# MDIL-SNU/SevenNet

Hardware: AMD Instinct MI355X
Metric: atom-steps/sec (energy+forces), SevenNet-0 100k-atom cell, 1/2/4/8 MI355X (higher is better)
Workload: dtype f32 (storage / accumulate / tensor product; in-kernel W2 products f16x3 = two fp16 terms per operand, three matrix-core products: fp32-rounding class; node linears bf16x6); 1 GPU; sevennet_0 shape (5 interaction layers), 97336-atom periodic diamond-Si cell (a=5.431 A x 23^3, sigma=0.05 A), cutoff 5.0 A, 2725408 directed edges, seeded synthetic weights; atoms=97336, edges=2725408, parallelism=single GPU, fused=auto, terms=4

## Files before the change

include/snet_hip.h:

```cpp
#ifndef SNET_HIP_H
#define SNET_HIP_H

#include <stdint.h>

#ifdef __cplusplus
extern "C" {
#endif

#define SNET_ABI_VERSION 3

int snet_abi_version(void);
const char *snet_last_error(void);
int snet_conv_num_shapes(void);
const char *snet_conv_shape_tag(int i);

typedef struct snet_edge_params {
  float cutoff;
  int32_t n_basis;
  int32_t cutoff_kind;
  int32_t poly_p;
  float cutoff_on;
  int32_t lmax;
  int32_t normalize;
} snet_edge_params;
// ... 54 lines not shown
void snet_fused_plan_destroy(snet_fused_plan *plan);
int snet_edge_tiles(const int32_t *row_ptr, int64_t n_dst, int32_t *tile_ptr, int32_t *tile_node, int64_t tile_capacity,
                    int64_t *n_tiles, void *stream);
int snet_edge_tiles_packed(const int32_t *row_ptr, int64_t node_begin, int64_t node_end, int32_t *tile_e0,
                           int32_t *tile_nodes, int64_t tile_capacity, int64_t *n_tiles, void *stream);
int snet_fused_plan_tile_mode(const snet_fused_plan *plan);
int snet_conv_plan_transposed(const snet_conv_plan *plan, char *tag, float *col_scale, int32_t *dead, int32_t dead_capacity,
                              int32_t *n_dead);
int snet_edges_by_source(const int32_t *row_ptr, int64_t n_dst, const int32_t *eperm, const int32_t *w_row, int64_t n_edges,
                         int32_t *center_t, int32_t *w_row_t, void *stream);
int snet_conv_fwd_fused(const snet_fused_plan *plan, const float *x, const float *sh, const float *h2,
                        const int32_t *w_row, const int32_t *row_ptr, const int32_t *src, int64_t n_dst, float scale,
                        float *out, void *stream);
int snet_conv_bwd_fused(const snet_fused_plan *plan, const float *x, const float *sh, const float *dsh,
                        const float *h2, const int32_t *w_row, const int32_t *row_ptr, const int32_t *src,
                        const int32_t *tile_ptr, const int32_t *tile_node, int64_t n_tiles, float scale,
                        const float *g_out, float *g_xe, float *g_h2, const float *emb, float *g_emb, float *g_vec,
                        const float *x_rowmax, const float *g_rowmax, void *stream);
int snet_conv_bwd_fused_sh(const snet_fused_plan *plan, const float *x, const float *sh, const float *h2, const int32_t *w_row,
                           const int32_t *row_ptr, const int32_t *src, const int32_t *tile_ptr, const int32_t *tile_node,
                           int64_t n_tiles, float scale, const float *g_out, float *g_xe, float *g_h2, const float *emb,
                           float *g_emb, float *g_sh, const float *x_rowmax, const float *g_rowmax, void *stream);
int snet_fused_plan_has_mlp_tail(const snet_fused_plan *plan);
int snet_fused_plan_prefers_tangent(const snet_fused_plan *plan);
int snet_edge_embed_tangent(const snet_edge_params *p_host, const float *coeffs_host, const float *edge_vec,
                            const int32_t *edge_of_row, int64_t n_rows, float *demb, void *stream);
int snet_radial_mlp_hidden_fwd_layers_tangent(const snet_mlp_plan *const *plans, int32_t n_layers, const float *emb, const float *demb,
                                              int64_t n_rows, float *const *h2, float *const *h2d, void *stream);
int snet_conv_bwd_fused_tangent(const snet_fused_plan *plan, const float *x, const float *sh, const float *dsh, const float *h2,
                                const float *h2d, const int32_t *w_row, const int32_t *row_ptr, const int32_t *src,
                                const int32_t *tile_ptr, const int32_t *tile_node, int64_t n_tiles, float scale, const float *g_out,
                                float *g_xe, const float *edge_vec, float *g_vec, const float *x_rowmax, const float *g_rowmax,
                                void *stream);
int snet_fused_plan_gxe_chunks(const snet_fused_plan *plan, int32_t *chunk_pos, int32_t capacity);
int snet_segment_sum_rows_chunked(const float *x, const int32_t *seg_ptr, const int32_t *perm, int64_t n_seg, int32_t dim,
                                  const int32_t *chunk_pos, float *out, void *stream);
int snet_row_absmax(const float *x, int64_t n_rows, int32_t dim, float *out, void *stream);
int snet_row_absmax_multi(const float *const *x, const int64_t *n_rows, const int32_t *dims, float *const *out, int32_t n,
                          void *stream);
int snet_row_norm2(const float *x, int64_t n_rows, int32_t dim, float mult, float *out, void *stream);
int snet_conv_bwd_edge(const snet_conv_plan *plan, const float *x, const float *sh, const float *w,
                       const int32_t *w_row, const int32_t *row_ptr, const int32_t *src, int64_t n_dst, float scale,
                       const float *g_out, float *g_w, float *g_xe, float *g_sh, void *stream);
int snet_conv_bwd_edge_vec(const snet_conv_plan *plan, const float *x, const float *sh, const float *dsh,
                           const float *w, const int32_t *w_row, const int32_t *row_ptr, const int32_t *src,
                           int64_t n_dst, float scale, const float *g_out, float *g_w, float *g_xe, float *g_vec,
                           void *stream);
int snet_conv_bwd_node(const snet_conv_plan *plan, const float *sh, const float *w, const int32_t *w_row,
                       const int32_t *col_ptr,
                       const int32_t *eperm, const int32_t *dst, int64_t n_src, float scale,
                       const float *g_out, float *g_x, void *stream);

int snet_segment_sum_rows(const float *x, const int32_t *seg_ptr, const int32_t *perm, int64_t n_seg, int32_t dim,
                          float *out, void *stream);

typedef struct snet_gate_seg {
  int32_t kind;
  int32_t in_off;
  int32_t out_off;
  int32_t mul;
  int32_t l;
  int32_t gate_off;
  int32_t act;
  float cst;
} snet_gate_seg;
#define SNET_MAX_GATE_SEGS 16
// ... 153 lines not shown
```

sevennet_amd/_lib.py:

```python
from __future__ import annotations

import ctypes as C
import os

_HERE = os.path.dirname(os.path.abspath(__file__))
ABI_VERSION = 3
LIB_PATH = os.environ.get('SNET_HIP_LIB') or os.path.join(_HERE, 'libsnet_hip.so')

c_f32p = C.c_void_p
c_i32p = C.c_void_p
c_f64p = C.c_void_p
c_stream = C.c_void_p


class EdgeParams(C.Structure):
    _fields_ = [('cutoff', C.c_float), ('n_basis', C.c_int32), ('cutoff_kind', C.c_int32),
                ('poly_p', C.c_int32), ('cutoff_on', C.c_float), ('lmax', C.c_int32),
                ('normalize', C.c_int32)]


class GemmDesc(C.Structure):
    _fields_ = [('B', C.c_void_p), ('B_split', C.c_void_p), ('a_off', C.c_int64), ('c_off', C.c_int64), ('d', C.c_int32), ('K', C.c_int32),
                ('N', C.c_int32), ('accumulate', C.c_int32)]

# ... 30 lines not shown
    'snet_act_bwd': (C.c_int, [c_f32p, c_f32p, c_f32p, C.c_int64, C.c_int32, C.c_float, c_stream]),
    'snet_conv_plan_create': (C.c_int, [C.c_char_p, C.POINTER(C.c_void_p)]),
    'snet_conv_plan_destroy': (None, [C.c_void_p]),
    'snet_conv_register_library': (C.c_int, [C.c_char_p]),
    'snet_conv_plan_dims': (C.c_int, [C.c_void_p, C.POINTER(C.c_int32), C.POINTER(C.c_int32),
                                      C.POINTER(C.c_int32), C.POINTER(C.c_int32)]),
    'snet_conv_fwd': (C.c_int, [C.c_void_p, c_f32p, c_f32p, c_f32p, c_i32p, c_i32p, c_i32p, C.c_int64, C.c_float,
                                c_f32p, c_stream]),
    'snet_radial_mlp_hidden_fwd': (C.c_int, [C.c_void_p, c_f32p, C.c_int64, c_f32p, c_stream]),
    'snet_radial_mlp_hidden_fwd_layers': (C.c_int, [C.POINTER(C.c_void_p), C.c_int32, c_f32p, C.c_int64, C.POINTER(C.c_void_p), c_stream]),
    'snet_radial_mlp_hidden_bwd': (C.c_int, [C.c_void_p, c_f32p, c_f32p, C.c_int64, c_f32p, c_stream]),
    'snet_conv_fused_available': (C.c_int, [C.c_void_p]),
    'snet_conv_plan_transposed': (C.c_int, [C.c_void_p, C.c_char_p, c_f32p, c_i32p, C.c_int32, C.POINTER(C.c_int32)]),
    'snet_edges_by_source': (C.c_int, [c_i32p, C.c_int64, c_i32p, c_i32p, C.c_int64, c_i32p, c_i32p, c_stream]),
    'snet_fused_plan_create': (C.c_int, [C.c_void_p, C.c_void_p, C.c_int32, C.POINTER(C.c_void_p)]),
    'snet_fused_plan_destroy': (None, [C.c_void_p]),
    'snet_edge_tiles': (C.c_int, [c_i32p, C.c_int64, c_i32p, c_i32p, C.c_int64, C.POINTER(C.c_int64), c_stream]),
    'snet_conv_fwd_fused': (C.c_int, [C.c_void_p, c_f32p, c_f32p, c_f32p, c_i32p, c_i32p, c_i32p, C.c_int64, C.c_float,
                                      c_f32p, c_stream]),
    'snet_conv_bwd_fused': (C.c_int, [C.c_void_p, c_f32p, c_f32p, c_f32p, c_f32p, c_i32p, c_i32p, c_i32p, c_i32p,
                                      c_i32p, C.c_int64, C.c_float, c_f32p, c_f32p, c_f32p, c_f32p, c_f32p, c_f32p, c_f32p, c_f32p,
                                      c_stream]),
    'snet_conv_bwd_fused_sh': (C.c_int, [C.c_void_p, c_f32p, c_f32p, c_f32p, c_i32p, c_i32p, c_i32p, c_i32p,
                                         c_i32p, C.c_int64, C.c_float, c_f32p, c_f32p, c_f32p, c_f32p, c_f32p, c_f32p, c_f32p, c_f32p,
                                         c_stream]),
    'snet_fused_plan_has_mlp_tail': (C.c_int, [C.c_void_p]),
    'snet_fused_plan_prefers_tangent': (C.c_int, [C.c_void_p]),
    'snet_edge_embed_tangent': (C.c_int, [C.POINTER(EdgeParams), C.POINTER(C.c_float), c_f32p, c_i32p, C.c_int64, c_f32p, c_stream]),
    'snet_radial_mlp_hidden_fwd_layers_tangent': (C.c_int, [C.POINTER(C.c_void_p), C.c_int32, c_f32p, c_f32p, C.c_int64,
                                                            C.POINTER(C.c_void_p), C.POINTER(C.c_void_p), c_stream]),
    'snet_conv_bwd_fused_tangent': (C.c_int, [C.c_void_p, c_f32p, c_f32p, c_f32p, c_f32p, c_f32p, c_i32p, c_i32p, c_i32p, c_i32p,
                                              c_i32p, C.c_int64, C.c_float, c_f32p, c_f32p, c_f32p, c_f32p, c_f32p, c_f32p,
                                              c_stream]),
    'snet_fused_plan_gxe_chunks': (C.c_int, [C.c_void_p, C.POINTER(C.c_int32), C.c_int32]),
    'snet_segment_sum_rows_chunked': (C.c_int, [c_f32p, c_i32p, c_i32p, C.c_int64, C.c_int32, c_i32p, c_f32p, c_stream]),
    'snet_edge_vectors': (C.c_int, [c_f64p, c_i32p, c_i32p, c_f64p, C.c_int64, c_f32p, c_stream]),
    'snet_row_absmax': (C.c_int, [c_f32p, C.c_int64, C.c_int32, c_f32p, c_stream]),
    'snet_row_absmax_multi': (C.c_int, [C.POINTER(C.c_void_p), C.POINTER(C.c_int64), C.POINTER(C.c_int32), C.POINTER(C.c_void_p), C.c_int32, c_stream]),
    'snet_row_norm2': (C.c_int, [c_f32p, C.c_int64, C.c_int32, C.c_float, c_f32p, c_stream]),
    'snet_conv_bwd_edge': (C.c_int, [C.c_void_p, c_f32p, c_f32p, c_f32p, c_i32p, c_i32p, c_i32p, C.c_int64, C.c_float,
                                     c_f32p, c_f32p, c_f32p, c_f32p, c_stream]),
    'snet_segment_sum_rows': (C.c_int, [c_f32p, c_i32p, c_i32p, C.c_int64, C.c_int32, c_f32p, c_stream]),
    'snet_conv_bwd_node': (C.c_int, [C.c_void_p, c_f32p, c_f32p, c_i32p, c_i32p, c_i32p, c_i32p, C.c_int64, C.c_float,
                                     c_f32p, c_f32p, c_stream]),
    'snet_gate_fwd': (C.c_int, [c_f32p, c_f32p, c_f32p, C.c_int64, C.c_int32, C.c_int32, C.POINTER(GateSeg), C.c_int32,
                                c_stream]),
    'snet_gate_bwd': (C.c_int, [c_f32p, c_f32p, c_f32p, C.c_int64, C.c_int32, C.c_int32, C.POINTER(GateSeg),
                                C.c_int32, c_stream]),
    'snet_gate_bwd_norm': (C.c_int, [c_f32p, c_f32p, c_f32p, C.c_int64, C.c_int32, C.c_int32, C.POINTER(GateSeg),
                                     C.c_int32, C.c_float, c_f32p, c_stream]),
    'snet_embed_rows': (C.c_int, [c_f32p, c_i32p, c_f32p, C.c_int64, C.c_int32, c_stream]),
    'snet_add_row_bias': (C.c_int, [c_f32p, c_f32p, C.c_int64, C.c_int32, c_stream]),
    'snet_add_inplace': (C.c_int, [c_f32p, c_f32p, C.c_int64, c_stream]),
    'snet_permute_cols': (C.c_int, [c_f32p, c_i32p, c_f32p, C.c_int64, C.c_int32, c_stream]),
    'snet_rescale_reduce': (C.c_int, [c_f32p, c_i32p, c_f32p, c_f32p, C.c_int32, C.c_int64, c_f32p, c_f64p,
                                      c_stream]),
    'snet_readout_energy': (C.c_int, [c_f32p, C.c_int64, C.c_int32, c_f64p, C.c_double, c_i32p, c_f32p, c_f32p, C.c_int32,
                                      c_f32p, c_f64p, c_stream]),
    'snet_readout_grad': (C.c_int, [c_f64p, C.c_int32, c_i32p, c_f32p, C.c_int32, C.c_int64, c_f32p, c_stream]),
    'snet_edge_force': (C.c_int, [c_f32p, c_f32p, c_i32p, c_i32p, c_i32p, C.c_int64, C.c_int64, c_f32p, c_f32p,
                                  c_f64p, c_stream]),
    'snet_readout_energy_seg': (C.c_int, [c_f32p, C.c_int64, C.c_int32, c_f64p, C.c_double, c_i32p, c_f32p, c_f32p, C.c_int32,
                                          c_i32p, C.c_int32, c_f32p, c_f64p, c_f64p, c_stream]),
    'snet_rescale_reduce_seg': (C.c_int, [c_f32p, c_i32p, c_f32p, c_f32p, C.c_int32, C.c_int64, c_i32p, C.c_int32, c_f32p, c_f64p,
                                          c_f64p, c_stream]),
    'snet_edge_force_seg': (C.c_int, [c_f32p, c_f32p, c_i32p, c_i32p, c_i32p, C.c_int64, C.c_int64, c_i32p, C.c_int32, c_f32p,
# ... 132 lines not shown
```

sevennet_amd/build.py:

```python
from __future__ import annotations

import argparse
import concurrent.futures as cf
import hashlib
import os
import shutil
import subprocess
import sys
from typing import List

from . import codegen, codegen_fused
from .shapes import aot_conv_specs

HERE = os.path.dirname(os.path.abspath(__file__))
CSRC = os.path.join(HERE, 'csrc')
INCLUDE = os.path.join(os.path.dirname(HERE), 'include')
LIB = os.environ.get('SNET_BUILD_LIB') or os.path.join(HERE, 'libsnet_hip.so')
_sfx = ('_' + os.path.basename(LIB).replace('.so', '')) if os.environ.get('SNET_BUILD_LIB') else ''
GEN = os.path.join(CSRC, 'generated' + _sfx)
OBJ = os.path.join(CSRC, 'build' + _sfx)
ARCH = 'gfx950'
STATIC_SOURCES = ['snet_api.cpp', 'snet_model.cpp', 'snet_halo.cpp', 'snet_gemm.hip', 'snet_mlp.hip', 'snet_edge.hip', 'snet_node.hip', 'snet_force.hip', 'snet_neighbor.hip', 'snet_batch.hip', 'snet_relax.hip', 'snet_mdstep.hip', 'snet_md.hip', 'snet_d3.hip', 'snet_d3_ref.cpp']


# ... 90 lines not shown
        ['-o', out, f'-L{os.path.dirname(LIB)}', '-l:' + os.path.basename(LIB), f'-L{rocm}/lib', '-lamdhip64',
         '-Wl,-rpath,$ORIGIN/../../sevennet_amd', f'-Wl,-rpath,{rocm}/lib']
    r = subprocess.run(cmd, capture_output=True, text=True)
    if r.returncode != 0:
        raise RuntimeError(f'g++ failed on the LAMMPS mock harness:\n{r.stderr[-4000:]}')
    if verbose:
        print(f'[sevennet_amd.build] built {out}', flush=True)
    return out


def build(jobs: int = 0, force: bool = False, extra_configs=(), verbose: bool = True) -> str:
    write_d3_blob()
    os.makedirs(GEN, exist_ok=True)
    os.makedirs(OBJ, exist_ok=True)
    os.makedirs(os.path.join(CSRC, 'generated'), exist_ok=True)
    codegen.write_if_changed(os.path.join(CSRC, 'generated', 'sh_generated.h'), codegen.gen_sh_header(3))
    specs = aot_conv_specs(extra_configs)
    sources = [os.path.join(CSRC, s) for s in STATIC_SOURCES]
    keep = set()
    for tag, spec in specs.items():
        path = os.path.join(GEN, f'conv_{tag}.hip')
        codegen.write_if_changed(path, codegen.gen_conv(spec))
        sources.append(path)
        keep.add(os.path.basename(path))
        if codegen_fused.fusable(spec):
            fpath = os.path.join(GEN, f'convf_{tag}.hip')
            codegen.write_if_changed(fpath, codegen_fused.gen_conv_fused(spec))
            sources.append(fpath)
            keep.add(os.path.basename(fpath))
            tpath = os.path.join(GEN, f'convft_{tag}.hip')
            codegen.write_if_changed(tpath, codegen_fused.gen_conv_fused_tangent(spec))
            sources.append(tpath)
            keep.add(os.path.basename(tpath))
    for f in os.listdir(GEN):
        if (f.startswith('conv_') or f.startswith('convf_') or f.startswith('convft_') or f.startswith('_conv')) and f not in keep:
            os.remove(os.path.join(GEN, f))
    jobs = jobs or min(16, os.cpu_count() or 4)
    if verbose:
        print(f'[sevennet_amd.build] {len(sources)} translation units ({len(specs)} conv shapes), -j{jobs}',
              flush=True)
    with cf.ThreadPoolExecutor(jobs) as ex:
        objs = list(ex.map(lambda s: _compile(s, force), sources))
    newest = max(os.path.getmtime(o) for o in objs)
    if force or not os.path.exists(LIB) or os.path.getmtime(LIB) < newest:
        cmd = [_hipcc(), f'--offload-arch={ARCH}', '-shared', '-fPIC', '-o', LIB] + objs
        r = subprocess.run(cmd, capture_output=True, text=True)
        if r.returncode != 0:
            raise RuntimeError(f'link failed:\n{r.stderr[-4000:]}')
    if verbose:
        print(f'[sevennet_amd.build] built {LIB}', flush=True)
    if not os.environ.get('SNET_BUILD_LIB'):
        try:
            build_lammps_harness(verbose)
        except Exception as exc:
            print(f'[sevennet_amd.build] LAMMPS mock harness NOT built: {exc}', file=sys.stderr, flush=True)
    return LIB


def main(argv=None):
    ap = argparse.ArgumentParser()
    ap.add_argument('-j', type=int, default=0)
    ap.add_argument('--force', action='store_true')
    a = ap.parse_args(argv)
    build(a.j, a.force)


if __name__ == '__main__':
    main()
# ... 1 lines not shown
```

sevennet_amd/codegen_fused.py:

```python
from __future__ import annotations

import struct
from typing import Dict, List

from .codegen import OPTS, _Cat, _f, _path_terms, _sum_expr
from .model_spec import ConvSpec


def fusable(spec: ConvSpec) -> bool:
    return all(mul % 16 == 0 for mul, _, _ in spec.irreps_x) and spec.irreps_sh.dim <= 16 and len(spec.paths) > 0


def schedule(spec: ConvSpec):
    cats = []
    for i in range(len(spec.irreps_x)):
        cat = _Cat(spec, i, 0)
        if cat.paths:
            cats.append(cat)
    pairs_of, cols = [], []
    for cat in cats:
        ps = [pi for pi, _ in cat.paths]
        pairs = [(ps[k], ps[k + 1] if k + 1 < len(ps) else None) for k in range(0, len(ps), 2)]
        pairs_of.append(pairs)
        for ct in range(cat.mul // 16):
            for pa, pb in pairs:
                cols.append((spec.paths[pa].w_off + 16 * ct, spec.paths[pb].w_off + 16 * ct if pb is not None else -1))
    return cats, pairs_of, cols


def schedule_bwd(spec: ConvSpec):
    out, cols = [], []
    n_cats = sum(1 for i in range(len(spec.irreps_x)) if _Cat(spec, i, 0).paths)
    for i in range(len(spec.irreps_x)):
        cat = _Cat(spec, i, 0)
        if not cat.paths:
            continue
        ps = [pi for pi, _ in cat.paths]
        nct = cat.mul // 16
        entries = sum(2 * p.l3 + 1 for _, p in cat.paths)
        if len(ps) % 2 == 1 and nct % 2 == 0 and 2 * entries <= 32 and n_cats > 1 and not OPTS.get('nopairct'):
            full = [(ps[k], ps[k + 1]) for k in range(0, len(ps) - 1, 2)]
            steps = [((a, 0), (b, 0)) for a, b in full] + [((a, 1), (b, 1)) for a, b in full] + [((ps[-1], 0), (ps[-1], 1))]
            U = 2
# ... 97 lines not shown
    for a, cl in reverse_plan(p):
        A(f'  {{  // x component {a}')
        A(f'    const f32x2 xl = lo2(xr[{a}]), xh = hi2(xr[{a}]);')
        A('    const f32x2 wxl = wl * xl, wxh = wh * xh;')
        A('    f32x2 Pl, Ph;')
        for k, (c, bl) in enumerate(cl):
            tl = [f'{_f(v)} * ys[{p.sh_off + b}]' for b, v in bl]
            A(f'    {{ const float V = {_sum_expr(tl)};')
            A('      const f32x2 V2 = f32x2{V, V};')
            A(f'      const f32x2 Gl = lo2(G[{c}]), Gh = hi2(G[{c}]);')
            if k == 0:
                A('      Pl = V2 * Gl; Ph = V2 * Gh;')
            else:
                A('      Pl = __builtin_elementwise_fma(V2, Gl, Pl); Ph = __builtin_elementwise_fma(V2, Gh, Ph);')
            A('      const f32x2 s2 = __builtin_elementwise_fma(wxh, Gh, wxl * Gl);')
            for b, v in bl:
                if pkgy:
                    A(f'      gy[{p.sh_off + b}] = __builtin_elementwise_fma(f32x2{{{_f(v)}, {_f(v)}}}, s2, gy[{p.sh_off + b}]);')
                else:
                    A(f'      gy[{p.sh_off + b}] = fmaf({_f(v)}, s2[0] + s2[1], gy[{p.sh_off + b}]);')
            A('    }')
        A('    gwl = __builtin_elementwise_fma(xl, Pl, gwl); gwh = __builtin_elementwise_fma(xh, Ph, gwh);')
        A('    if constexpr (GX) {')
        A(f'      const f32x2 gl_ = __builtin_elementwise_fma(wl, Pl, lo2(gx[{a}])), gh_ = __builtin_elementwise_fma(wh, Ph, hi2(gx[{a}]));')
        A(f'      gx[{a}] = f32x4{{gl_[0], gl_[1], gh_[0], gh_[1]}};')
        A('    }')
        A('  }')
    A('  gw = f32x4{gwl[0], gwl[1], gwh[0], gwh[1]};')
    A('}')


class _Gen:

    def __init__(self, spec: ConvSpec, tangent: bool = False):
        self.spec = spec
        self.TG = bool(tangent)
        tag = self.tag = spec.tag
        self.def_b = (int(OPTS.get('fnwv', 8)), int(OPTS.get('fglds', 0)), int(OPTS.get('focc', 2)))
        self.def_f = (int(OPTS.get('fnwvf', 8)), int(OPTS.get('fgldsf', 0)), int(OPTS.get('foccf', 2)))
        self.exp = OPTS.get('fexp') == tag
        self.DX, self.DOUT, self.NSH, self.WN = spec.irreps_x.dim, spec.irreps_out.dim, spec.irreps_sh.dim, spec.weight_numel
        NSH = self.NSH
        cats, self.pairs_of, self.cols = schedule(spec)
        self.cats = cats
        self.NS = len(self.cols)
        self.offs_x = spec.irreps_x.offsets()
        self.dead_x = [i for i in range(len(spec.irreps_x)) if not any(p.i_x == i for p in spec.paths)]
        self.L: List[str] = []
        self.A = self.L.append
        self.NSHP = NSH + 1 if (4 * NSH) % 32 == 0 else NSH
        self.gxe_std = bool(OPTS.get('gxestd'))
        self.stamped = tag in (OPTS.get('stamp'), OPTS.get('stampl'), OPTS.get('stampf'), OPTS.get('stampfl'))
        self.FROW = bool(int(OPTS.get('frow', 1)))
        self.FRSB = int(OPTS.get('frsb', 0))
        self._reverse_decisions()
        self._forward_decisions()
        if self.TG:
            self.stamped = self.ST = self.STL = False

    def _reverse_decisions(self):
        spec, cats, NSH = self.spec, self.cats, self.NSH
        bsched, cols_b = schedule_bwd(spec)
        self.bsched, self.cols_b = bsched, cols_b
        glists = [[(pi, m3, u) for u in range(bs['U']) for pi, p in bs['cat'].paths for m3 in range(2 * p.l3 + 1)] for bs in bsched]
        self.glists = glists
        NGP = max((len(gl) + 15) // 16 * 16 for gl in glists)
        NK = NGP // 16
        self.NGP, self.NK = NGP, NK
        maxd1 = max(2 * c_.l1 + 1 for c_ in cats)
        maxd3 = max(2 * p_.l3 + 1 for p_ in spec.paths)

        def live_regs(gs):
            return 12 * maxd1 + 32 + NSH + 4 * gs * NK + 16 + 4 * maxd3 + 35
        packed_class = live_regs(2) <= 200 and live_regs(1) > 168 and len(cats) > 1
        XT = self.XT = bool(int(OPTS['xtile'])) if 'xtile' in OPTS else packed_class
        GS = self.GS = 2 if XT else 1
        self.PK = bool(int(OPTS['pk'])) if 'pk' in OPTS else XT
        self.PKGY = self.PK and bool(int(OPTS.get('pkgy', 1)))
        VMORD = self.VMORD = not OPTS.get('novmord')
        self.GRAW = VMORD and not OPTS.get('nograw')
        GUNC = VMORD and not OPTS.get('nogunc')
        live = self.live = live_regs(GS)
        self.three_waves = 2 * 8 * 2 * 1024 + 4 * (2 * NGP * 64 + NSH * 64) <= 53 * 1024 and live <= (160 if XT else 168)
        if self.three_waves:
            GUNC = GUNC and bool(OPTS.get('gunc3'))
        self.GUNC = GUNC
        budget = (168 if self.three_waves else 256) - 24
        xp_regs = max([4 * b_['U'] * (2 * b_['cat'].l1 + 1) for b_ in bsched[1:]] or [0])
        self.XPF = VMORD and len(bsched) > 1 and live + xp_regs + 8 <= budget and not OPTS.get('noxpf')
        self.HOIST = VMORD and live + 16 + 8 <= budget and not OPTS.get('nohoist')
        self.noxn = int(OPTS.get('noxn', 7 if live > 200 else 0))
        self.STL = OPTS.get('stampl') == self.tag
        self.ST = OPTS.get('stamp') == self.tag or self.STL
        self.TGPREF = bool(int(OPTS['tgpref'])) if 'tgpref' in OPTS else live <= 200

    def block_info(self, ci):
        bs = self.bsched[ci]
        d1 = 2 * bs['cat'].l1 + 1
        return bs['cat'], bs['U'], bs['ncb'], d1, (self.noxn > 0 and d1 >= self.noxn)

    def bwd_lds(self, nt, nwv):
        return 2 * 8 * nt * 1024 + nwv * (2 * self.NGP * 64 + (128 if self.XT else 0) + self.NSH * 64)

    def bwd_cfg(self, nt):
        if 'fnwv' in OPTS:
            return self.def_b
        if len(self.cats) == 1 and self.bwd_lds(nt, 8) <= 80 * 1024:
            return (8, 0, 2)
        if self.bwd_lds(nt, 4) <= 53 * 1024 and self.live <= (160 if self.XT else 168):
            return (4, 0, 3)
        if self.bwd_lds(nt, 4) <= 80 * 1024:
            return (4, 0, 2)
        return (2, 0, 2)

    def _forward_decisions(self):
        spec, cats = self.spec, self.cats
        FG = int(OPTS.get('ffg', 3))
        fgroups = []
        for ci, cat in enumerate(cats):
            prs = list(enumerate(self.pairs_of[ci]))
            fgroups.append([prs[i:i + FG] for i in range(0, len(prs), FG)])
        self.fgroups = fgroups
        self.LPB = max(len(grp) for gl in fgroups for grp in gl)
        NOE = max(sum(2 * spec.paths[pi].l3 + 1 for _, pr in grp for pi in pr if pi is not None) for gl in fgroups for grp in gl)
        self.NOEP = (NOE + 15) // 16 * 16
        self.MAXD1 = max(2 * cat.l1 + 1 for cat in cats)
        self.N_OOFF = sum((sum(2 * spec.paths[pi].l3 + 1 for _, pr in grp for pi in pr if pi is not None) + 15) // 16 for gl in fgroups for grp in gl)
        self.OOLDS = self.N_OOFF > 8 if 'oolds' not in OPTS else bool(int(OPTS['oolds']))
        self.STFL = OPTS.get('stampfl') == self.tag
        self.STF = OPTS.get('stampf') == self.tag or self.STFL
        self.olists, self.oo_index = {}, {}

    def fwd_lds(self, nt, nwv):
        return 2 * self.LPB * 4 * nt * 1024 + nwv * (32 * self.NSHP * 4 + self.MAXD1 * 1024 + self.NOEP * 64) + 4 * nwv + (64 * self.N_OOFF if self.OOLDS else 0)

    def fwd_cfg(self, nt):
        if 'fnwvf' in OPTS:
            return self.def_f
        if len(self.cats) == 1 and self.fwd_lds(nt, 8) <= 80 * 1024:
            return (8, 0, 2)
        if nt <= 2 and self.fwd_lds(nt, 12) <= 160 * 1024:
            return (12, 0 if OPTS.get('f12reg') else 1, 3)
        for w in (8, 4, 2, 1):
            if self.fwd_lds(nt, w) <= 160 * 1024:
                return (w, 1, 2)
        raise NotImplementedError(f'conv shape {self.spec.key}: the fused forward kernel does not fit the LDS')

    @staticmethod
    def out_index(p, m3):
        return p.out_off + m3 * p.out_mul + p.out_ch

    def S(self, i, ind='      '):
        if self.ST and (not self.STL or i in (0, 1, 10, 11, 12, 13)):
            self.A(f'{ind}stamp({i});')

    def SF(self, i, ind, light=True):
        if self.STF and (light or not self.STFL):
            self.A(f'{ind}stamp({i});')

    def g_row(self, ci, pi, m3, u):
        return self.glists[ci].index((pi, m3, u))

    def emit_g_loads(self, ind, ci, cb_expr):
        A, glists, bsched, exp, GRAW, GUNC, XT = self.A, self.glists, self.bsched, self.exp, self.GRAW, self.GUNC, self.XT
        gl = glists[ci]
        U_ = bsched[ci]['U']
        for k in range((len(gl) + 15) // 16):
            dg = '(diag & 8) ? f32x4{1.f, 1.f, 1.f, 1.f} : ' if exp else ''
            sc_ = ' * scale' if not GRAW else ''
            pred = '' if GUNC else f'(goff{ci}_{k} < 0) ? f32x4{{0.f, 0.f, 0.f, 0.f}} : '
            A(f'{ind}gpre[{k}] = {dg}{pred}*reinterpret_cast<const f32x4 *>(gnode + goff{ci}_{k} + {16 * U_} * ({cb_expr})){sc_};')
        if XT:
            A(f'{ind}if (two) {{')
            for k in range((len(gl) + 15) // 16):
                A(f'{ind}  gpre_b[{k}] = {dg}{pred}*reinterpret_cast<const f32x4 *>(gnode_b + goff{ci}_{k} + {16 * U_} * ({cb_expr})){sc_};')
            A(f'{ind}}}')

    def emit_g_park(self, ind, ci, buf_expr):
        A, glists, GRAW, XT = self.A, self.glists, self.GRAW, self.XT
        gl = glists[ci]
        for k in range((len(gl) + 15) // 16):
            sc_ = ' * g_park'
            A(f'{ind}*reinterpret_cast<f32x4 *>(&s_g[wave][{"0" if XT else buf_expr}][(16 * {k} + (lane >> 2)) * 16 + 4 * (lane & 3)]) = gpre[{k}]{sc_};')
        if XT:
            A(f'{ind}if (two) {{')
            for k in range((len(gl) + 15) // 16):
                A(f'{ind}  *reinterpret_cast<f32x4 *>(&s_g[wave][1][(16 * {k} + (lane >> 2)) * 16 + 4 * (lane & 3)]) = gpre_b[{k}]{sc_};')
            A(f'{ind}}}')

    def emit_x_loads(self, ind, ci_, ct_expr, tl_):
        A, cats = self.A, self.cats
        cat_ = cats[ci_]
        A(f'{ind}{{ const float *xs_ = x + {cat_.x_off} + 16 * ({ct_expr}) + 4 * (lane & 3) + (size_t)srs[{tl_}] * DX;')
        for m in range(2 * cat_.l1 + 1):
            A(f'{ind}  xq[{m}] = *reinterpret_cast<const f32x4 *>(xs_ + {m * cat_.mul});')
        A(f'{ind}}}')


def _emit_header(cx: _Gen):
    A, spec, tag, cats = cx.A, cx.spec, cx.tag, cx.cats
    DX, DOUT, NSH, NSHP, WN, NS, cols, cols_rev = cx.DX, cx.DOUT, cx.NSH, cx.NSHP, cx.WN, cx.NS, cx.cols, cx.cols_b
    A('// GENERATED by sevennet_amd/codegen_fused.py -- do not edit.')
    A(f'// fused conv shape {tag}: x = {spec.irreps_x}, sh = {spec.irreps_sh}, out = {spec.irreps_out}')
    A(f'// {len(spec.paths)} paths, weight_numel = {WN}, {NS} sub-steps of two 16-column tiles')
    A('#include <cstdio>')
    A('#include <cstdlib>')
    A('#include "snet_common.h"')
    A('#include "snet_split.h"')
    A('namespace {')
    A('using namespace snet;')
    A('__device__ __forceinline__ f32x2 lo2(const f32x4 v) { return __builtin_shufflevector(v, v, 0, 1); }')
    A('__device__ __forceinline__ f32x2 hi2(const f32x4 v) { return __builtin_shufflevector(v, v, 2, 3); }')
    A(f'constexpr int DX = {DX}, DOUT = {DOUT}, NSH = {NSH}, NSHP = {NSHP}, WN = {WN}, NS = {NS};')
    A('const int32_t SUB_COLS[NS * 2] = {' + ', '.join(f'{a}, {b}' for a, b in cols) + '};')
    A(f'const int32_t SUB_COLS_B[{2 * len(cols_rev)}] = {{' + ', '.join(f'{a}, {b}' for a, b in cols_rev) + '};')
    gxe_chunk = list(range(DX // 16))
    for cat in ([] if cx.gxe_std else cats):
        d1c = 2 * cat.l1 + 1
        for ct in range(cat.mul // 16):
            for m in range(d1c):
                gxe_chunk[(cat.x_off + m * cat.mul) // 16 + ct] = cat.x_off // 16 + ct * d1c + m
    assert sorted(gxe_chunk) == list(range(DX // 16))
    A(f'const int32_t GXE_CHUNK[{DX // 16}] = {{' + ', '.join(str(v) for v in gxe_chunk) + '};')
    A('')


def _emit_path_functions(cx: _Gen):
    A, spec, PK, FROW, FRSB = cx.A, cx.spec, cx.PK, cx.FROW, cx.FRSB
    for pi, p in enumerate(spec.paths):
# ... 51 lines not shown
                    A(f'    const float y{b_} = ysl[{r} * NSHP + {p.sh_off + b_}];')
            if w_first:
                for a_ in sorted({a_ for (a_, _) in byab}):
                    A(f'    const float xw{a_} = w[{r}] * xr[{r}][{a_}];')
            for (a_, b_), cl in sorted(byab.items()):
                A(f'    {{ const float xy = ' + (f'xw{a_}' if w_first else f'xr[{r}][{a_}]') + f' * y{b_};')
                for cc, v in cl:
                    A(f'      acc[{cc}] = fmaf({_f(v)}, xy, acc[{cc}]);' if w_first else f'      s{cc} = fmaf({_f(v)}, xy, s{cc});')
                A('    }')
            for i in range(0 if w_first else d3):
                A(f'    acc[{i}] = fmaf(w[{r}], s{i}, acc[{i}]);')
            A('  }')
            if r < 3 and FRSB and len(terms) >= FRSB:
                A('  __builtin_amdgcn_sched_barrier(0);   // one row at a time: the rows\' temporaries are not interleaved (register pressure of the large paths)')
        A('}')
    A('')


def _rev_prologue(cx: _Gen):
    A, spec, tag, cats, exp = cx.A, cx.spec, cx.tag, cx.cats, cx.exp
    NSH, XT, ST, GUNC, HOIST = cx.NSH, cx.XT, cx.ST, cx.GUNC, cx.HOIST
    bsched, glists, NGP, NK, NSB = cx.bsched, cx.glists, cx.NGP, cx.NK, len(cx.cols_b)
    S, emit_g_loads, emit_g_park, out_index = cx.S, cx.emit_g_loads, cx.emit_g_park, cx.out_index
    NPH = 16
    if cx.stamped:
        A('constexpr int SNET_STAMP_TILES = 1 << 18;')
        A('__device__ unsigned snet_stamps[16 * SNET_STAMP_TILES];   // one row per tile: no atomics (2.7 M atomics on 16 hot words stalled the whole chip)')
    TG = cx.TG
    if TG:
        A('// TANGENT MODE of the reverse kernel: the radial gradient dE/d|r_e| = sum_k g_w[e, k] w\'_e[k] with w\'_e = h2\' W2, h2\' = d h2 / d|r| of')
        A('// the edge\'s radial row (tail.h2d).  w\' is a second product on the A fragments of w, its contraction with the fresh g_w tiles one')
        A('// multiply-add per register.  No operand split of g_w, no g_h2 products, no second W2 image in the slab, no hidden-layer tail, no')
        A('// g_emb: the sum goes, along r_e / |r_e|, straight into the g_vec row the kernel writes anyway.')
    A('template <int NT, bool F16, int NWV, bool GLDS, int OCC, bool GX>')
    A(f'__global__ __launch_bounds__(64 * NWV, OCC) void conv_bwdf{"t" if TG else ""}_{tag}(const float *__restrict__ x, const float *__restrict__ sh,')
    A('    const float *__restrict__ dsh, const float *__restrict__ h2, const int32_t *__restrict__ w_row,')
    A('    const int32_t *__restrict__ row_ptr, const int32_t *__restrict__ src, const int32_t *__restrict__ tile_ptr,')
    A('    const int32_t *__restrict__ tile_node, int n_tiles, const u32x4 *__restrict__ slabs, float scale,')
    A('    const float *__restrict__ g_out, float *__restrict__ g_xe, float *__restrict__ g_h2, float *__restrict__ g_vec,')
    A('    const snet::FusedTail tail, int diag) {')
    A('  // diag: always 0 in production (bit 0 also serves as the opaque branch condition around the tensor-product bodies);')
    A('  // kernel-tuning builds: 1 skip the tensor product, 2 skip the g_h2 products, 4 skip the w products, 8 skip the')
    A('  // g_out loads, 16 skip the g_xe stores -- timing decomposition, results are then garbage')
    if TG:
        A('  constexpr int LPS = 8 * NT, LW = 4 * NT, NTH = 64 * NWV, NST = (LW * 64 + NTH - 1) / NTH, GLN = 1;  // 1-KB fragment lines per sub-step in the stream / staged; sub-steps per slab')
        A('  __shared__ u32x4 slab[2][GLN * LW * 64];')
    else:
        A('  constexpr int LPS = 8 * NT, NTH = 64 * NWV, NST = (LPS * 64 + NTH - 1) / NTH, GLN = 1;  // 1-KB fragment lines per sub-step; sub-steps per slab')
        A('  __shared__ u32x4 slab[2][GLN * LPS * 64];')
    A('  const int tid = threadIdx.x, lane = tid & 63, wave = __builtin_amdgcn_readfirstlane(tid >> 6);   // (wave-uniform: scalar address arithmetic)')
    A('  const int j = lane & 15, g = lane >> 4;')
    if ST:
        A(f'  unsigned ph[{NPH}];')
        A('#pragma unroll')
        A(f'  for (int i = 0; i < {NPH}; ++i) ph[i] = 0u;')
        A('  unsigned t_prev;')
        A('  { unsigned long long t0_; asm volatile("s_memtime %0\\n\\ts_waitcnt lgkmcnt(0)" : "=s"(t0_) :: "memory"); t_prev = (unsigned)t0_; }')
        A('  auto stamp = [&](int i) {')
        A('    __builtin_amdgcn_sched_barrier(0);')
        A('    unsigned long long t_; asm volatile("s_memtime %0\\n\\ts_waitcnt lgkmcnt(0)" : "=s"(t_) :: "memory");')
        A('    const unsigned tn = (unsigned)t_;')
        A('    ph[i] += tn - t_prev;')
        A('    t_prev = tn;')
        A('    __builtin_amdgcn_sched_barrier(0);')
        A('  };')
    _emit_staging(A, 'LW' if TG else 'LPS')
    A('  stage_load(0, 0);')
    A('  const int t_raw = snet::xcd_node(blockIdx.x, gridDim.x) * NWV + wave;')
    A('  const bool live = t_raw < n_tiles;')
    A('  const int t = __builtin_amdgcn_readfirstlane(live ? t_raw : n_tiles - 1);  // idle waves shadow the last tile, stores masked')
    if XT:
        A('  const int node = __builtin_amdgcn_readfirstlane(tile_node[2 * t]);       // A: the node of the tile\'s first edge')
        A('  const int node_b = __builtin_amdgcn_readfirstlane(tile_node[2 * t + 1]);  // B: the node of its last edge (= A for most tiles of a long segment)')
        A('  const bool two = node_b != node;')
    else:
        A('  const int node = __builtin_amdgcn_readfirstlane(tile_node[t]);')
    A(f'  constexpr int NGP = {NGP}, NK = {NK}, NSUB = {NSB};   // NSUB: sub-steps of the reverse kernel\'s weight stream')
    if XT:
        A(f'  __shared__ __attribute__((aligned(16))) float s_g[NWV][2][NGP * 16 + {int(OPTS.get("gpad", 16))}];   // (+ 16: the two sets of a (row, group) read on disjoint banks)')
        A('  f32x4 gpre[NK], gpre_b[NK];')
        A('  const float *gnode = g_out + (size_t)node * DOUT + 4 * (lane & 3);')
        A('  const float *gnode_b = g_out + (size_t)node_b * DOUT + 4 * (lane & 3);')
    else:
        A('  __shared__ __attribute__((aligned(16))) float s_g[NWV][2][NGP * 16];')
        A('  f32x4 gpre[NK];')
        A('  const float *gnode = g_out + (size_t)((diag & 256) ? (node & 63) : node) * DOUT + 4 * (lane & 3);')
    for ci, gl in enumerate(glists):
        for k in range((len(gl) + 15) // 16):
            offs = [out_index(spec.paths[gl[q][0]], gl[q][1]) + 16 * gl[q][2] if q < len(gl) else (0 if GUNC else -1) for q in range(16 * k, 16 * k + 16)]
            A(f'  static const int32_t GOFF{ci}_{k}[16] = {{' + ', '.join(str(o) for o in offs) + '};')
            A(f'  const int goff{ci}_{k} = GOFF{ci}_{k}[lane >> 2];')
    emit_g_loads('  ', 0, '0')
    if XT:
        A('  const int e0 = tile_ptr[t];')
        A('  const int cnt = tile_ptr[t + 1] - e0;')
        A('  const int e_b = two ? row_ptr[node + 1] : 0x7fffffff;   // first edge of node B')
    else:
        A('  const int e0 = row_ptr[node] + 16 * (t - tile_ptr[node]);')
        A('  const int cnt = min(16, row_ptr[node + 1] - e0);')
    A('  const bool valid = live && j < cnt;')
    A('  const int e = e0 + min(j, cnt - 1);')
    if XT:
        A('  const int in_b = e >= e_b ? 1 : 0;')
    A('  const int s_src = src[e];')
    A('  const int wr = w_row ? w_row[e] : e;')
    A('  float x_bound = 0.f;')
    A('  if constexpr (F16) x_bound = tail.x_max[s_src] * tail.g_max[' + ('in_b ? node_b : node' if XT else 'node') + '];')
    _c0, _U0 = cats[0], bsched[0]['U']
    _d0 = 2 * _c0.l1 + 1
    A(f'  const float *xs0 = x + (size_t)s_src * DX + {_c0.x_off} + 4 * g;')
    A(f'  f32x4 xr0[{_U0}][{_d0}], xn0[{_U0}][{_d0}];')
    for u in range(_U0):
        for m in range(_d0):
            A(f'  xr0[{u}][{m}] = *reinterpret_cast<const f32x4 *>(xs0 + {16 * u + m * _c0.mul});')

    A('  // the edge\'s spherical harmonics wait in wave-private LDS ([component][edge]: conflict-free, the four channel')
    A('  // groups of an edge read the same word) and are re-read per path: 9 .. 16 fewer live registers per lane')
    A('  __shared__ float s_y[NWV][NSH * 16];')
    A('  if (g == 0) {')
    A('#pragma unroll')
    A('    for (int k = 0; k < NSH; ++k) s_y[wave][k * 16 + j] = sh[(size_t)e * NSH + k];')
    A('  }')
    A('  const float *yl = &s_y[wave][j];')
    A('  SplitN<NT> hb[2];  // h2^T as B operand: column = edge, k slots (g, 0..7) <-> hidden unit 32 q + 8 g + slot')
    A('  float w_unscale = 1.f;  // fp16 terms: h2 is scaled per tile (wave-uniform power of two), W2 per matrix on the host')
    A('  {')
    A('    float hv[2][8];')
    A('#pragma unroll')
    A('    for (int q = 0; q < 2; ++q) {')
    A('      const f32x4 lo4 = *reinterpret_cast<const f32x4 *>(h2 + (size_t)wr * 64 + 32 * q + 8 * g);')
    A('      const f32x4 hi4 = *reinterpret_cast<const f32x4 *>(h2 + (size_t)wr * 64 + 32 * q + 8 * g + 4);')
    A('#pragma unroll')
    A('      for (int i = 0; i < 4; ++i) { hv[q][i] = lo4[i]; hv[q][4 + i] = hi4[i]; }')
    A('    }')
    A('    if constexpr (F16) {')
    A('      const int kh = snet::F16_TOP - snet::bound_exp(snet::wave_max(fmaxf(snet::max8(hv[0]), snet::max8(hv[1]))));')
    A('      const float sc = snet::pow2f(kh);')
    A('#pragma unroll')
    A('      for (int q = 0; q < 2; ++q)')
    A('#pragma unroll')
    A('        for (int i = 0; i < 8; ++i) hv[q][i] *= sc;')
    A('      w_unscale = snet::pow2f(-(kh + tail.w2_exp));')
    A('    }')
    A('    hb[0] = splitn8<NT, F16>(hv[0]);')
    A('    hb[1] = splitn8<NT, F16>(hv[1]);')
    A('  }')
    if TG:
# ... 16 lines not shown
        A('      for (int q = 0; q < 2; ++q)')
        A('#pragma unroll')
        A('        for (int i = 0; i < 8; ++i) hv[q][i] *= sc;')
        A('      hd_unsc = snet::pow2f(-kd);')
        A('    }')
        A('    hdb[0] = splitn8<NT, F16>(hv[0]);')
        A('    hdb[1] = splitn8<NT, F16>(hv[1]);')
        A('  }')
    else:
        A('  f32x4 ga[4];  // g_h2^T[k = 16 m + 4 g + r][edge]')
        A('#pragma unroll')
        A('  for (int m = 0; m < 4; ++m) ga[m] = f32x4{0.f, 0.f, 0.f, 0.f};')
    if cx.PKGY:
        A('  f32x2 gy[NSH];')
        A('#pragma unroll')
        A('  for (int k = 0; k < NSH; ++k) gy[k] = f32x2{0.f, 0.f};')
    else:
        A('  float gy[NSH];')
        A('#pragma unroll')
        A('  for (int k = 0; k < NSH; ++k) gy[k] = 0.f;')
    KC = max(sum(abs(v) for _, _, _, v in _path_terms(p)) for p in spec.paths)
    A('  float g_sc = 1.f, g_unsc = 1.f, gx_fix = 1.f;')
    A('  if constexpr (F16) {')
    A('    float ym = 0.f;')
    A('#pragma unroll')
    A('    for (int k = 0; k < NSH; ++k) ym = fmaxf(ym, fabsf(yl[k * 16]));')
    A(f'    const int kg = min(60, snet::F16_TOP - snet::bound_exp({_f(KC)} * fabsf(scale) * snet::wave_max(x_bound * ym)));')
    A('    g_sc = snet::pow2f(kg);')
    A('    g_unsc = snet::pow2f(-(kg + tail.w2_exp));')
    A('    gx_fix = w_unscale * snet::pow2f(-kg);')
    A('  }')
    A('  const float g_park = ' + ('scale * g_sc' if cx.GRAW else 'g_sc') + ';   // factor of the g_out entries when they are parked in LDS')
    emit_g_park('  ', 0, '0')
    A('  stage_store(0);')
    A('  __syncthreads();')
    if HOIST:
        A('  if (1 < NSUB' + (' && !(diag & 32)' if exp else '') + ') stage_load(1, 1);   // the first block\'s first sub-step does not request its slab itself')
    A('  int sidx = 0, buf = 0, gbuf = 0;')
    S(0, '  ')


def _rev_block_top(cx: _Gen, ci: int):
    A, exp, XT, XPF, bsched = cx.A, cx.exp, cx.XT, cx.XPF, cx.bsched
    S, emit_g_loads = cx.S, cx.emit_g_loads
    bs = bsched[ci]
    cat, U, ncb, d1, NOXN = cx.block_info(ci)
    A(f'  // ---- x block {cat.i_x}: {cat.mul}x l={cat.l1}, {len(cat.paths)} paths, {U} channel tile(s) per block, {len(bs["steps"])} sub-steps per block')
    if ci > 0:
        A(f'  const float *xs{ci} = x + (size_t)s_src * DX + {cat.x_off} + 4 * g;')
        A(f'  f32x4 xr{ci}[{U}][{d1}], xn{ci}[{U}][{d1}];')
        for u in range(U):
            for m in range(d1):
                A(f'  xr{ci}[{u}][{m}] = ' + (f'xp{ci}[{u}][{m}];' if XPF else f'*reinterpret_cast<const f32x4 *>(xs{ci} + {16 * u + m * cat.mul});'))
    if XPF and ci + 1 < len(bsched):
        cat_n, U_n = bsched[ci + 1]['cat'], bsched[ci + 1]['U']
        d1_n = 2 * cat_n.l1 + 1
        A(f'  const float *xs{ci + 1}p = x + (size_t)s_src * DX + {cat_n.x_off} + 4 * g;')
        A(f'  f32x4 xp{ci + 1}[{U_n}][{d1_n}];')
    A(f'  for (int cb = 0; cb < {ncb}; ++cb) {{')
    A(f'    f32x4 (&xr)[{U}][{d1}] = xr{ci};')
    A(f'    f32x4 gx[{U}][{d1}];')
    for u in range(U):
        for m in range(d1):
            A(f'    gx[{u}][{m}] = f32x4{{0.f, 0.f, 0.f, 0.f}};')
    def emit_next_xblock_rows(ind):
        for u in range(U_n):
            for m in range(d1_n):
                A(f'{ind}xp{ci + 1}[{u}][{m}] = *reinterpret_cast<const f32x4 *>(xs{ci + 1}p + {16 * u + m * cat_n.mul});')
    if ncb > 1:
        A(f'    if (cb + 1 < {ncb}' + (' && !(diag & 64)' if exp else '') + ') {')
        for u in range(U):
            for m in range(d1):
                if not NOXN:
                    A(f'      xn{ci}[{u}][{m}] = *reinterpret_cast<const f32x4 *>(xs{ci} + {16 * U} * (cb + 1) + {16 * u + m * cat.mul});')
        if XPF and ci + 1 < len(bsched):
            A('    } else {')
            emit_next_xblock_rows('      ')
        A('    }')
    elif XPF and ci + 1 < len(bsched):
        emit_next_xblock_rows('    ')
    A('    const float *gl_ = &s_g[wave][' + ('in_b' if XT else 'gbuf') + '][4 * g];')
    if ncb > 1:
        A(f'    if (cb + 1 < {ncb}) {{')
        emit_g_loads('      ', ci, 'cb + 1')
        A('    }' + (' else {' if ci + 1 < len(bsched) else ''))
        if ci + 1 < len(bsched):
            emit_g_loads('      ', ci + 1, '0')
            A('    }')
    elif ci + 1 < len(bsched):
        emit_g_loads('    ', ci + 1, '0')
    S(1, '    ')


def _rev_substep(cx: _Gen, ci: int, si_: int, ta, tb):
    A, spec, exp, ST, STL, HOIST = cx.A, cx.spec, cx.exp, cx.ST, cx.STL, cx.HOIST
    S, g_row = cx.S, cx.g_row
    U, TG = cx.bsched[ci]['U'], cx.TG
    A('    {')
    if not (HOIST and si_ == 0):
        A('      if (sidx + 1 < NSUB' + (' && !(diag & 32)' if exp else '') + ') stage_load(sidx + 1, (buf ^ 1));')
    A('      __builtin_amdgcn_sched_barrier(0);')
    S(2)
    A('      const u32x4 *sl = slab[buf];')
    A('      f32x4 gw0 = f32x4{0.f, 0.f, 0.f, 0.f}, gw1 = gw0;')
    for tp, tl_ in enumerate((ta, tb)):
        if tl_ is None:
# ... 322 lines not shown
        A('      gr = gr * g_unsc * hd_unsc;   // g_w carried 2^kg, w\' 2^(kd + w2_exp) (fp16 terms; 1 otherwise)')
        A('      const float *v_ = tail.edge_vec + (size_t)e * 3;')
        A('      const float vx = v_[0], vy = v_[1], vz = v_[2];')
        A('      const float ir = 1.f / sqrtf(vx * vx + vy * vy + vz * vz);')
        A('      float *o = g_vec + (size_t)e * 3;')
        A('      o[0] += gr * vx * ir; o[1] += gr * vy * ir; o[2] += gr * vz * ir;')
        A('    }')
        A('  }')
    if ST:
        S(13, '  ')
        A('  if (lane == 0 && live && t_raw < SNET_STAMP_TILES) {')
        A(f'    for (int i = 0; i < {NPH}; ++i) snet_stamps[t_raw * 16 + i] = ph[i];')
        A('  }')
    A('}')
    A('')


def _emit_reverse_kernel(cx: _Gen):
    _rev_prologue(cx)
    for ci, bs in enumerate(cx.bsched):
        _rev_block_top(cx, ci)
        for si_, (ta, tb) in enumerate(bs['steps']):
            _rev_substep(cx, ci, si_, ta, tb)
        _rev_block_end(cx, ci)
    _rev_tail(cx)
    _rev_epilogue(cx)


def _fwd_prologue(cx: _Gen):
    A, L, spec, tag, NSHP = cx.A, cx.L, cx.spec, cx.tag, cx.NSHP
    fgroups, LPB, NOEP, MAXD1, N_OOFF, OOLDS, STF = cx.fgroups, cx.LPB, cx.NOEP, cx.MAXD1, cx.N_OOFF, cx.OOLDS, cx.STF
    SF, out_index, olists, oo_index = cx.SF, cx.out_index, cx.olists, cx.oo_index
    oo_rows = []
    A('template <int NT, bool F16, int NWV, bool GLDS, int OCC>')
    A(f'__global__ __launch_bounds__(64 * NWV, OCC) void conv_fwdf_{tag}(const float *__restrict__ x, const float *__restrict__ sh,')
    A('    const float *__restrict__ h2, const int32_t *__restrict__ w_row, const int32_t *__restrict__ row_ptr,')
    A('    const int32_t *__restrict__ src, int n_nodes, const u32x4 *__restrict__ slabs, float scale, float *__restrict__ out, int w2_exp, int diag) {')
    A(f'  constexpr int LPS = 8 * NT, LPF = 4 * NT, LPB = {LPB}, NTH = 64 * NWV;  // lines per sub-step (all / w part), sub-steps per block')
    A('  constexpr int NSTB = (LPB * LPF * 64 + NTH - 1) / NTH;')
    A('  __shared__ u32x4 slab[2][LPB * LPF * 64];')
    A('  __shared__ int s_pass[NWV];')
    if OOLDS:
        A(f'  __shared__ int32_t s_ooff[{16 * N_OOFF}];')
    A('  __shared__ __attribute__((aligned(16))) float s_ys[NWV][32 * NSHP];  // spherical harmonics of the pass\'s edges (rows padded: NSHP)')
    A(f'  __shared__ __attribute__((aligned(16))) float s_x[NWV][{MAXD1} * 256];  // source-row slice of one tile: [m][r][g][channel]')
    A(f'  __shared__ __attribute__((aligned(16))) float s_o[NWV][{NOEP} * 16];      // output rows of one block: [entry][channel]')
    A('  const int tid = threadIdx.x, lane = tid & 63, wave = __builtin_amdgcn_readfirstlane(tid >> 6);   // (wave-uniform: scalar address arithmetic)')
    A('  const int c = lane & 15, g = lane >> 4;')
    A('  const int n_raw = snet::xcd_node(blockIdx.x, gridDim.x) * NWV + wave;')
    if STF:
        A('  unsigned ph[16];')
        A('#pragma unroll')
        A('  for (int i = 0; i < 16; ++i) ph[i] = 0u;')
        A('  unsigned t_prev;')
        A('  { unsigned long long t0_; asm volatile("s_memtime %0\\n\\ts_waitcnt lgkmcnt(0)" : "=s"(t0_) :: "memory"); t_prev = (unsigned)t0_; }')
        A('  auto stamp = [&](int i) {')
        A('    __builtin_amdgcn_sched_barrier(0);')
        A('    unsigned long long t_; asm volatile("s_memtime %0\\n\\ts_waitcnt lgkmcnt(0)" : "=s"(t_) :: "memory");')
        A('    const unsigned tn = (unsigned)t_;')
        A('    ph[i] += tn - t_prev;')
        A('    t_prev = tn;')
        A('    __builtin_amdgcn_sched_barrier(0);')
        A('  };')
    A('  const bool live = n_raw < n_nodes;')
    A('  const int node = __builtin_amdgcn_readfirstlane(live ? n_raw : n_nodes - 1);')
    A('  const int e_beg = row_ptr[node], e_end = row_ptr[node + 1];')
    A('  const int my_pass = live ? (e_end - e_beg + 31) >> 5 : 0;')
    oo_fill_at = len(L)
    A('  if (lane == 0) s_pass[wave] = my_pass;')
    A('  __syncthreads();')
    A('  int n_pass = 1;  // every wave of the block walks the weight stream the same number of times')
    A('#pragma unroll')
    A('  for (int i = 0; i < NWV; ++i) n_pass = max(n_pass, s_pass[i]);')
    SF(0, '  ')
    A('  u32x4 st[GLDS ? 1 : NSTB];')
    A('  auto stage_load = [&](int s0, int n, int b) {  // the w parts of sub-steps s0 .. s0 + n - 1 -> slab[b]')
    A('    if constexpr (GLDS) {')
    A('      for (int l = wave; l < n * LPF; l += NWV)')
    A('        __builtin_amdgcn_global_load_lds((const __attribute__((address_space(1))) void *)(slabs + (size_t)(s0 + l / LPF) * (LPS * 64) + (l % LPF) * 64 + lane),')
    A('                                         (__attribute__((address_space(3))) void *)(&slab[b][l * 64]), 16, 0, 0);')
    A('    } else {')
    A('#pragma unroll')
    A('      for (int i = 0; i < NSTB; ++i) {')
    A('        const int f = tid + NTH * i, l = f >> 6;')
    A('        if (l < n * LPF) st[i] = slabs[(size_t)(s0 + l / LPF) * (LPS * 64) + (l % LPF) * 64 + (f & 63)];')
    A('      }')
    A('    }')
    A('  };')
    A('  auto stage_store = [&](int n, int b) {')
    A('    if constexpr (!GLDS) {')
    A('#pragma unroll')
    A('      for (int i = 0; i < NSTB; ++i) if (((tid + NTH * i) >> 6) < n * LPF) slab[b][tid + NTH * i] = st[i];')
    A('    }')
    A('  };')
    A('  float *onode = out + (size_t)node * DOUT + 4 * (lane & 3);')
    A('  const bool has_e = e_end > e_beg;')
    A('  const int e_last = max(e_beg, e_end - 1);  // clamp target for padded rows (their weight is zeroed)')
    for ci, gl in enumerate(fgroups):
        for gi, grp in enumerate(gl):
            ol = [(pi, m3) for _, pr in grp for pi in pr if pi is not None for m3 in range(2 * spec.paths[pi].l3 + 1)]
# ... 16 lines not shown
    A, FROW, fgroups, MAXD1, SF = cx.A, cx.FROW, cx.fgroups, cx.MAXD1, cx.SF
    A('  for (int pass = 0; pass < n_pass; ++pass) {')
    A('    const int eb = e_beg + 32 * pass;')
    A('    const int n_e = live ? max(0, min(32, e_end - eb)) : 0;  // edges of this pass: tile 0 = [0,16), tile 1 = [16,32)')
    A('    const bool two = n_e > 16;')
    if FROW:
        A('    const int m_t[2] = {min(n_e, 16), max(n_e - 16, 0)};')
        A('    const int rows_t[2] = {(m_t[0] + 3) >> 2, (m_t[1] + 3) >> 2};')
        A('    auto edge_of_row = [&](int tl, int row) { return 16 * tl + (row >> 2) * rows_t[tl] + (row & 3); };  // (rows r >= R alias a neighbour\'s edge: never used)')
    else:
        A('    auto edge_of_row = [&](int tl, int row) { return 16 * tl + row; };')
    A('    // per tile: A fragments of h2 (row = edge lane & 15; rows without an edge are zero) and the source row this lane stages (edge lane >> 2)')
    A('    SplitN<NT> ha[2][2];')
    A('    int srs[2];')
    A('    float hv[2][2][8];')
    A('#pragma unroll')
    A('    for (int tl = 0; tl < 2; ++tl) {')
    A('      const int ea = min(eb + edge_of_row(tl, c), e_last);')
    if FROW:
        A('      const bool rv = (c & 3) < rows_t[tl] && (c >> 2) * rows_t[tl] + (c & 3) < m_t[tl];   // this lane\'s A row holds an edge')
    else:
        A('      const bool rv = 16 * tl + c < n_e;')
    A('      const int wra = rv ? (w_row ? w_row[ea] : ea) : 0;')
    A('#pragma unroll')
    A('      for (int q = 0; q < 2; ++q) {')
    A('        f32x4 lo4 = f32x4{0.f, 0.f, 0.f, 0.f}, hi4 = lo4;')
    A('        if (rv) {')
    A('          lo4 = *reinterpret_cast<const f32x4 *>(h2 + (size_t)wra * 64 + 32 * q + 8 * g);')
    A('          hi4 = *reinterpret_cast<const f32x4 *>(h2 + (size_t)wra * 64 + 32 * q + 8 * g + 4);')
    A('        }')
    A('#pragma unroll')
    A('        for (int i = 0; i < 4; ++i) { hv[tl][q][i] = lo4[i]; hv[tl][q][4 + i] = hi4[i]; }')
    A('      }')
    A('      srs[tl] = has_e ? src[min(eb + edge_of_row(tl, lane >> 2), e_last)] : 0;')
    A('    }')
    A('    float o_scale = scale;  // fp16 terms: h2 is scaled per pass (wave-uniform power of two), W2 per matrix on the host; both are undone on the output rows')
    A('    if constexpr (F16) {')
    A('      const int kh = snet::F16_TOP - snet::bound_exp(snet::wave_max(fmaxf(fmaxf(snet::max8(hv[0][0]), snet::max8(hv[0][1])), fmaxf(snet::max8(hv[1][0]), snet::max8(hv[1][1])))));')
    A('      const float sc = snet::pow2f(kh);')
    A('#pragma unroll')
    A('      for (int tl = 0; tl < 2; ++tl)')
    A('#pragma unroll')
    A('        for (int q = 0; q < 2; ++q)')
    A('#pragma unroll')
    A('          for (int i = 0; i < 8; ++i) hv[tl][q][i] *= sc;')
    A('      o_scale = scale * snet::pow2f(-(kh + w2_exp));')
    A('    }')
    A('#pragma unroll')
    A('    for (int tl = 0; tl < 2; ++tl) {')
    A('      ha[tl][0] = splitn8<NT, F16>(hv[tl][0]);')
    A('      ha[tl][1] = splitn8<NT, F16>(hv[tl][1]);')
    A('    }')
    A('    for (int i = lane; i < 32 * NSH; i += 64) {')
    A('      const int el = i / NSH;')
    A('      s_ys[wave][el * NSHP + (i - el * NSH)] = has_e ? sh[(size_t)min(eb + edge_of_row(el >> 4, el & 15), e_last) * NSH + (i - el * NSH)] : 0.f;')
    A('    }')
    first_n = len(fgroups[0][0])
    A(f'    stage_load(0, {first_n}, 0);')
    A(f'    stage_store({first_n}, 0);')
    A('    __syncthreads();  // also orders the wave\'s s_ys stores before its reads')
    SF(1, '    ')
    A('    int sidx = 0, buf = 0;')
    A(f'    f32x4 xq[{MAXD1}];  // the next stage\'s slice, in flight: lane L holds channels 4 (L & 3) .. + 3 of edge L >> 2')
    cx.emit_x_loads('    ', 0, '0', 0)


def _fwd_block(cx: _Gen, ci: int, gi: int):
# ... 110 lines not shown


def _emit_forward_kernel(cx: _Gen):
    A = cx.A
    _fwd_prologue(cx)
    _fwd_pass_top(cx)
    for ci, cat in enumerate(cx.cats):
        A(f'    // ---- x block {cat.i_x}: {cat.mul}x l={cat.l1}, {len(cat.paths)} paths')
        A(f'    for (int ct = 0; ct < {cat.mul // 16}; ++ct) {{')
        for gi in range(len(cx.fgroups[ci])):
            _fwd_block(cx, ci, gi)
        A('    }')
    A('  }')
    if cx.STF:
        A('  if (lane == 0 && live && n_raw < SNET_STAMP_TILES) {')
        A('    for (int i = 0; i < 16; ++i) snet_stamps[n_raw * 16 + i] = ph[i];')
        A('  }')
    A('}')
    A('')


def _variants(exp, default, fwd=False):
    combos = [default]
    if exp:
        cand = ((4, 0, 2), (8, 0, 2), (8, 1, 2), (4, 0, 3), (12, 0, 3), (12, 1, 3)) if fwd else \
            ((4, 0, 2), (8, 0, 2), (8, 1, 2), (4, 0, 3), (4, 1, 3), (12, 0, 3), (12, 1, 3), (8, 1, 4), (8, 0, 4), (8, 0, 3))
        combos += [v for v in cand if v != default]
    return combos


def _emit_launch_bwd(cx: _Gen):
    A, exp, def_b, bwd_cfg = cx.A, cx.exp, cx.def_b, cx.bwd_cfg
    tag = ('t_' if cx.TG else '_') + cx.tag
    A('template <int NT, bool F16, int NWV, bool GLDS, int OCC>')
    A('void launch_bwd_t(const float *x, const float *sh, const float *dsh, const float *h2, const int32_t *w_row,')
    A('                  const int32_t *row_ptr, const int32_t *src, const int32_t *tile_ptr, const int32_t *tile_node, int64_t n_tiles,')
    A('                  const void *slabs, float scale, const float *g_out, float *g_xe, float *g_h2, float *g_vec, snet::FusedTail tail, hipStream_t st) {')
    A('  const unsigned grid = (unsigned)((n_tiles + NWV - 1) / NWV);')
    A('  int diag = 0;')
    if exp:
        A('  if (const char *e = getenv("SNET_FV_DIAG")) diag = atoi(e);')
    A('  // launches without a g_xe output (first layer, last layer with the transposed convolution) take the instantiation that does not form')
    A('  // the source-row gradient: its multiply-adds and its 4 U d1 registers per lane are gone, not just its stores')
    A('  if (g_xe != nullptr)')
    A(f'    conv_bwdf{tag}<NT, F16, NWV, GLDS, OCC, true><<<dim3(grid), dim3(64 * NWV), 0, st>>>(x, sh, dsh, h2, w_row, row_ptr, src, tile_ptr, tile_node,')
    A('        (int)n_tiles, static_cast<const u32x4 *>(slabs), scale, g_out, g_xe, g_h2, g_vec, tail, diag);')
    A('  else')
    A(f'    conv_bwdf{tag}<NT, F16, NWV, GLDS, OCC, false><<<dim3(grid), dim3(64 * NWV), 0, st>>>(x, sh, dsh, h2, w_row, row_ptr, src, tile_ptr, tile_node,')
    A('        (int)n_tiles, static_cast<const u32x4 *>(slabs), scale, g_out, g_xe, g_h2, g_vec, tail, diag);')
    A('}')
    A(f'void launch_bwd{"_tangent" if cx.TG else ""}(int nt, const float *x, const float *sh, const float *dsh, const float *h2, const int32_t *w_row,')
    A('                const int32_t *row_ptr, const int32_t *src, const int32_t *tile_ptr, const int32_t *tile_node, int64_t n_tiles,')
    A('                const void *slabs, float scale, const float *g_out, float *g_xe, float *g_h2, float *g_vec, snet::FusedTail tail, hipStream_t st) {')
    args_b = 'x, sh, dsh, h2, w_row, row_ptr, src, tile_ptr, tile_node, n_tiles, slabs, scale, g_out, g_xe, g_h2, g_vec, tail, st'
    if exp:
        A('  int vw = %d, vg = %d, vo = %d;' % def_b)
        A('  if (const char *e = getenv("SNET_FV_BWD")) sscanf(e, "%d,%d,%d", &vw, &vg, &vo);')
        for (w, gl, oc) in _variants(exp, def_b):
            for nt_ in (3, 2):
                A(f'  if (nt == {nt_} && vw == {w} && vg == {gl} && vo == {oc}) return launch_bwd_t<{nt_}, false, {w}, {"true" if gl else "false"}, {oc}>({args_b});')
            A(f'  if (nt == 4 && vw == {w} && vg == {gl} && vo == {oc}) return launch_bwd_t<2, true, {w}, {"true" if gl else "false"}, {oc}>({args_b});')
    w, gl, oc = bwd_cfg(2)
    A(f'  if (nt == 4) launch_bwd_t<2, true, {w}, {"true" if gl else "false"}, {oc}>({args_b});')
    for nt_, kw in ((3, 'else if'), (2, 'else if'), (1, 'else')):
        w, gl, oc = bwd_cfg(nt_)
        cond = f' (nt == {nt_})' if kw != 'else' else ''
        A(f'  {kw}{cond} launch_bwd_t<{nt_}, false, {w}, {"true" if gl else "false"}, {oc}>({args_b});')
    A('}')


def _emit_launch_fwd(cx: _Gen):
    A, tag, exp, def_f, fwd_cfg = cx.A, cx.tag, cx.exp, cx.def_f, cx.fwd_cfg
    A('template <int NT, bool F16, int NWV, bool GLDS, int OCC>')
    A('void launch_fwd_t(const float *x, const float *sh, const float *h2, const int32_t *w_row, const int32_t *row_ptr,')
    A('                  const int32_t *src, int64_t n_dst, const void *slabs, float scale, float *out, int w2_exp, hipStream_t st) {')
    A('  unsigned grid = (unsigned)((n_dst + NWV - 1) / NWV);')
    A('  int diag = 0;')
    if exp:
        A('  if (const char *e = getenv("SNET_FV_DIAG")) diag = atoi(e);')
    A(f'  conv_fwdf_{tag}<NT, F16, NWV, GLDS, OCC><<<dim3(grid), dim3(64 * NWV), 0, st>>>(x, sh, h2, w_row, row_ptr, src, (int)n_dst,')
    A('      static_cast<const u32x4 *>(slabs), scale, out, w2_exp, diag);')
    A('}')
    A('void launch_fwd(int nt, const float *x, const float *sh, const float *h2, const int32_t *w_row, const int32_t *row_ptr,')
    A('                const int32_t *src, int64_t n_dst, const void *slabs, float scale, float *out, int w2_exp, hipStream_t st) {')
    args_f = 'x, sh, h2, w_row, row_ptr, src, n_dst, slabs, scale, out, w2_exp, st'
    if exp:
        A('  int vw = %d, vg = %d, vo = %d;' % def_f)
        A('  if (const char *e = getenv("SNET_FV_FWD")) sscanf(e, "%d,%d,%d", &vw, &vg, &vo);')
        for (w, gl, oc) in _variants(exp, def_f, True):
            for nt_ in (3, 2):
                if nt_ == 3 and w > 8:
                    continue
                A(f'  if (nt == {nt_} && vw == {w} && vg == {gl} && vo == {oc}) return launch_fwd_t<{nt_}, false, {w}, {"true" if gl else "false"}, {oc}>({args_f});')
            A(f'  if (nt == 4 && vw == {w} && vg == {gl} && vo == {oc}) return launch_fwd_t<2, true, {w}, {"true" if gl else "false"}, {oc}>({args_f});')
    w, gl, oc = fwd_cfg(2)
    A(f'  if (nt == 4) launch_fwd_t<2, true, {w}, {"true" if gl else "false"}, {oc}>({args_f});')
    for nt_, kw in ((3, 'else if'), (2, 'else if'), (1, 'else')):
        w, gl, oc = fwd_cfg(nt_)
        cond = f' (nt == {nt_})' if kw != 'else' else ''
        A(f'  {kw}{cond} launch_fwd_t<{nt_}, false, {w}, {"true" if gl else "false"}, {oc}>({args_f});')
    A('}')


def _emit_registration(cx: _Gen):
    A, tag, XT, cols_rev = cx.A, cx.tag, cx.XT, cx.cols_b
    if cx.TG:
        A(f'const snet::FusedTangentKernels kernels = {{"{tag}", {1 if cx.TGPREF else 0}, launch_bwd_tangent}};')
        A('const snet::FusedTangentRegistrar registrar(&kernels);')
        A('}  // namespace')
        return
    A(f'const snet::FusedKernels kernels = {{"{tag}", DX, DOUT, NSH, WN, NS, SUB_COLS, {len(cols_rev)}, SUB_COLS_B, GXE_CHUNK, launch_bwd, launch_fwd, {1 if XT else 0}}};')
    A('const snet::FusedRegistrar registrar(&kernels);')
    A('}  // namespace')
    if cx.stamped:
        A('// out[0 .. 15] = per-phase cycle sums over the tiles of the LAST launch, out[31] = number of tiles that reported')
        A('extern "C" int snet_debug_stamps(unsigned long long *out, int reset) {')
        A('  static unsigned *host = nullptr;')
        A('  const size_t bytes = sizeof(unsigned) * 16 * SNET_STAMP_TILES;')
        A('  if (!host) host = static_cast<unsigned *>(malloc(bytes));')
        A('  if (out) {')
        A('    if (hipMemcpyFromSymbol(host, HIP_SYMBOL(snet_stamps), bytes) != hipSuccess) return 1;')
        A('    for (int i = 0; i < 32; ++i) out[i] = 0;')
        A('    for (int t = 0; t < SNET_STAMP_TILES; ++t) {')
        A('      unsigned long long tot = 0;')
        A('      for (int i = 0; i < 16; ++i) tot += host[t * 16 + i];')
        A('      if (!tot) continue;')
        A('      for (int i = 0; i < 16; ++i) out[i] += host[t * 16 + i];')
        A('      ++out[31];')
        A('    }')
        A('  }')
        A('  if (reset) { void *dev = nullptr; if (hipGetSymbolAddress(&dev, HIP_SYMBOL(snet_stamps)) != hipSuccess || hipMemset(dev, 0, bytes) != hipSuccess) return 1; }')
        A('  return 0;')
        A('}')


def gen_conv_fused_tangent(spec: ConvSpec) -> str:
    cx = _Gen(spec, tangent=True)
    _emit_header(cx)
    _emit_path_functions(cx)
    _emit_reverse_kernel(cx)
    _emit_launch_bwd(cx)
    _emit_registration(cx)
    return '\n'.join(cx.L) + '\n'


def gen_conv_fused(spec: ConvSpec) -> str:
    cx = _Gen(spec)
    _emit_header(cx)
    _emit_path_functions(cx)
    _emit_reverse_kernel(cx)
    _emit_forward_kernel(cx)
    _emit_launch_bwd(cx)
    _emit_launch_fwd(cx)
    _emit_registration(cx)
    return '\n'.join(cx.L) + '\n'
```

sevennet_amd/csrc/snet_api.cpp:

```cpp
#include <cstdio>
#include <cstring>
#include <map>
#include <vector>

#include <dlfcn.h>

#include "snet_common.h"

namespace snet {

static thread_local std::string g_err;
void set_error(const std::string &msg) { g_err = msg; }

static std::vector<const ConvKernels *> &registry() {
  static std::vector<const ConvKernels *> r;
  return r;
}
void register_conv(const ConvKernels *k) { registry().push_back(k); }

static std::vector<const FusedKernels *> &fused_registry() {
  static std::vector<const FusedKernels *> r;
  return r;
}
void register_fused(const FusedKernels *k) { fused_registry().push_back(k); }
const FusedKernels *find_fused(const char *tag) {
  for (const FusedKernels *k : fused_registry())
    if (std::string(k->tag) == tag) return k;
  return nullptr;
}
static std::vector<const FusedTangentKernels *> &fused_tangent_registry() {
  static std::vector<const FusedTangentKernels *> r;
  return r;
}
void register_fused_tangent(const FusedTangentKernels *k) { fused_tangent_registry().push_back(k); }
const FusedTangentKernels *find_fused_tangent(const char *tag) {
  for (const FusedTangentKernels *k : fused_tangent_registry())
    if (std::string(k->tag) == tag) return k;
  return nullptr;
}

double *reduce_scratch(int64_t n_doubles, hipStream_t st) {
  (void)st;
  static thread_local std::map<int, std::pair<double *, int64_t>> bufs;
  int dev = 0;
  if (hipGetDevice(&dev) != hipSuccess) return nullptr;
  auto &b = bufs[dev];
  if (b.second < n_doubles) {
    if (b.first) (void)hipFree(b.first);
    const int64_t n = n_doubles < 4096 ? 4096 : n_doubles;
    if (hipMalloc(&b.first, sizeof(double) * n) != hipSuccess) {
      b = {nullptr, 0};
      return nullptr;
    }
    b.second = n;
  }
  return b.first;
}

}

struct snet_conv_plan {
  const snet::ConvKernels *k;
};
struct snet_fused_plan {
  const snet::FusedKernels *k;
  const snet::FusedTangentKernels *kt;
  int terms;
  void *slabs;
  void *slabs_b;
  snet::MlpHidden hidden;
  int32_t exps[3];
};

extern "C" {

int snet_abi_version(void) { return SNET_ABI_VERSION; }
const char *snet_last_error(void) { return snet::g_err.c_str(); }
int snet_conv_num_shapes(void) { return (int)snet::registry().size(); }
const char *snet_conv_shape_tag(int i) {
  auto &r = snet::registry();
  return (i >= 0 && i < (int)r.size()) ? r[i]->tag : nullptr;
}

int snet_conv_plan_create(const char *tag, snet_conv_plan **plan) {
  SNET_REQUIRE(tag != nullptr && plan != nullptr, "snet_conv_plan_create: null argument");
  for (const snet::ConvKernels *k : snet::registry()) {
    if (std::string(k->tag) == tag) {
      *plan = new snet_conv_plan{k};
      return 0;
    }
  }
  snet::set_error(std::string("snet_conv_plan_create: tensor-product shape '") + tag +
                  "' is not compiled into libsnet_hip.so (rebuild with the model's config: "
                  "sevennet_amd.build.build(extra_configs=[config]), or register it in sevennet_amd/shapes.py)");
  return 3;
}
void snet_conv_plan_destroy(snet_conv_plan *plan) { delete plan; }
int snet_conv_register_library(const char *path) {
  SNET_REQUIRE(path != nullptr, "snet_conv_register_library: null path");
  const size_t before = snet::registry().size() + snet::fused_registry().size();
  void *h = dlopen(path, RTLD_NOW | RTLD_LOCAL);
  if (h == nullptr) {
    const char *why = dlerror();
    snet::set_error(std::string("snet_conv_register_library: dlopen(") + path + ") failed: " + (why ? why : "?"));
// ... 34 lines not shown
  snprintf(tag, 13, "%s", k->t_tag);
  if (col_scale) memcpy(col_scale, k->t_col_scale, (size_t)k->wn * 4);
  if (dead) memcpy(dead, k->t_dead, (size_t)k->t_ndead * 8);
  if (n_dead) *n_dead = k->t_ndead;
  return 0;
}

int snet_conv_fused_available(const snet_conv_plan *plan) {
  return plan != nullptr && snet::find_fused(plan->k->tag) != nullptr;
}


int snet_fused_plan_create(const snet_conv_plan *plan, const snet_mlp_plan *mlp, int32_t terms, snet_fused_plan **out) {
  SNET_REQUIRE(plan != nullptr && mlp != nullptr && out != nullptr, "snet_fused_plan_create: null argument");
  SNET_REQUIRE(terms >= 1 && terms <= 4,
               "snet_fused_plan_create: terms must be 1 (bf16), 2 (bf16x3), 3 (bf16x6) or 4 (f16x3: two fp16 terms)");
  const snet::FusedKernels *k = snet::find_fused(plan->k->tag);
  SNET_REQUIRE(k != nullptr, "snet_fused_plan_create: this tensor-product shape has no fused kernels (channel "
                             "multiplicities must be multiples of 16)");
  SNET_REQUIRE(snet::mlp_plan_wn(mlp) == k->wn && snet::mlp_plan_w2_host(mlp) != nullptr,
               "snet_fused_plan_create: the radial-MLP plan does not match the shape's weight_numel");
  void *dev = nullptr;
  snet::MlpHidden hid = snet::mlp_plan_hidden(mlp);
  if (hid.w0 != nullptr && !(hid.nb <= 16 && hid.nb % 4 == 0 && (hid.act == 0 || hid.act == 1))) hid.w0 = nullptr;
  int32_t exps[3] = {0, 0, 0}, exps_f[3];
  void *dev_b = nullptr;
  if (snet::pack_fused_slabs(snet::mlp_plan_w2_host(mlp), k->wn, k->n_sub, k->sub_cols, terms, nullptr, &dev, exps_f) != 0 ||
      snet::pack_fused_slabs(snet::mlp_plan_w2_host(mlp), k->wn, k->n_sub_b, k->sub_cols_b, terms,
                             hid.w0 ? &hid : nullptr, &dev_b, exps) != 0) {
    if (dev) (void)hipFree(dev);
    snet::set_error("snet_fused_plan_create: device allocation / upload of the W2 fragment stream failed");
    return 1;
  }
  *out = new snet_fused_plan{k, snet::find_fused_tangent(plan->k->tag), terms, dev, dev_b, hid, {exps[0], exps[1], exps[2]}};
  return 0;
}
int snet_fused_plan_tile_mode(const snet_fused_plan *p) { return p ? p->k->tile_mode : 0; }
void snet_fused_plan_destroy(snet_fused_plan *p) {
  if (!p) return;
  if (p->slabs) (void)hipFree(p->slabs);
  if (p->slabs_b) (void)hipFree(p->slabs_b);
  delete p;
}

int snet_conv_fwd_fused(const snet_fused_plan *fp, const float *x, const float *sh, const float *h2,
                        const int32_t *w_row, const int32_t *row_ptr, const int32_t *src, int64_t n_dst, float scale,
                        float *out, void *stream) {
  SNET_REQUIRE(fp != nullptr, "snet_conv_fwd_fused: null plan");
  SNET_REQUIRE(n_dst < (1ll << 31) / 4, "snet_conv_fwd_fused: too many nodes");
  if (n_dst <= 0) return 0;
  fp->k->fwd(fp->terms, x, sh, h2, w_row, row_ptr, src, n_dst, fp->slabs, scale, out, fp->exps[0],
             static_cast<hipStream_t>(stream));
  SNET_CHECK_LAUNCH("snet_conv_fwd_fused");
  return 0;
}
int snet_fused_plan_gxe_chunks(const snet_fused_plan *fp, int32_t *chunk_pos, int32_t capacity) {
  SNET_REQUIRE(fp != nullptr && chunk_pos != nullptr, "snet_fused_plan_gxe_chunks: null argument");
  const int n = fp->k->dx / 16;
  SNET_REQUIRE(capacity >= n, "snet_fused_plan_gxe_chunks: capacity below dx / 16");
  for (int i = 0; i < n; ++i) chunk_pos[i] = fp->k->gxe_chunk[i];
  return 0;
}
int snet_fused_plan_has_mlp_tail(const snet_fused_plan *fp) { return fp != nullptr && fp->hidden.w0 != nullptr; }

static int conv_bwd_fused_impl(const char *who, const snet_fused_plan *fp, const float *x, const float *sh, const float *dsh,
                               const float *h2, const int32_t *w_row, const int32_t *row_ptr, const int32_t *src,
                               const int32_t *tile_ptr, const int32_t *tile_node, int64_t n_tiles, float scale, const float *g_out,
// ... 21 lines not shown
                        const int32_t *w_row, const int32_t *row_ptr, const int32_t *src, const int32_t *tile_ptr,
                        const int32_t *tile_node, int64_t n_tiles, float scale, const float *g_out, float *g_xe,
                        float *g_h2, const float *emb, float *g_emb, float *g_vec, const float *x_rowmax,
                        const float *g_rowmax, void *stream) {
  return conv_bwd_fused_impl("snet_conv_bwd_fused", fp, x, sh, dsh, h2, w_row, row_ptr, src, tile_ptr, tile_node, n_tiles, scale, g_out,
                             g_xe, g_h2, emb, g_emb, g_vec, nullptr, x_rowmax, g_rowmax, stream);
}
int snet_fused_plan_prefers_tangent(const snet_fused_plan *fp) {
  return fp != nullptr && fp->kt != nullptr && fp->kt->tangent_pref != 0;
}
int snet_conv_bwd_fused_tangent(const snet_fused_plan *fp, const float *x, const float *sh, const float *dsh, const float *h2,
                                const float *h2d, const int32_t *w_row, const int32_t *row_ptr, const int32_t *src,
                                const int32_t *tile_ptr, const int32_t *tile_node, int64_t n_tiles, float scale, const float *g_out,
                                float *g_xe, const float *edge_vec, float *g_vec, const float *x_rowmax, const float *g_rowmax,
                                void *stream) {
  SNET_REQUIRE(fp != nullptr, "snet_conv_bwd_fused_tangent: null plan");
  SNET_REQUIRE(fp->kt != nullptr, "snet_conv_bwd_fused_tangent: this shape's tangent-mode kernel is not compiled in");
  SNET_REQUIRE(fp->terms != 4 || (x_rowmax != nullptr && g_rowmax != nullptr),
               "snet_conv_bwd_fused_tangent: terms = 4 (fp16 operands) needs x_rowmax and g_rowmax (snet_row_absmax of x and g_out)");
  SNET_REQUIRE(n_tiles < (1ll << 31), "snet_conv_bwd_fused_tangent: too many tiles");
  if (n_tiles <= 0) return 0;
  SNET_REQUIRE(tile_ptr != nullptr && tile_node != nullptr, "snet_conv_bwd_fused_tangent: null tile list");
  SNET_REQUIRE(h2d != nullptr && edge_vec != nullptr && dsh != nullptr && g_vec != nullptr,
               "snet_conv_bwd_fused_tangent: h2d, edge_vec, dsh and g_vec are required");
  snet::FusedTail tail{nullptr, nullptr, fp->hidden.nb, fp->hidden.act, fp->hidden.cst, fp->exps[0], fp->exps[1], fp->exps[2],
                       x_rowmax, g_rowmax, nullptr};
  tail.h2d = h2d;
  tail.edge_vec = edge_vec;
  fp->kt->bwd(fp->terms, x, sh, dsh, h2, w_row, row_ptr, src, tile_ptr, tile_node, n_tiles, fp->slabs_b, scale, g_out, g_xe, nullptr,
              g_vec, tail, static_cast<hipStream_t>(stream));
  SNET_CHECK_LAUNCH("snet_conv_bwd_fused_tangent");
  return 0;
}
int snet_conv_bwd_fused_sh(const snet_fused_plan *fp, const float *x, const float *sh, const float *h2, const int32_t *w_row,
                           const int32_t *row_ptr, const int32_t *src, const int32_t *tile_ptr, const int32_t *tile_node,
                           int64_t n_tiles, float scale, const float *g_out, float *g_xe, float *g_h2, const float *emb,
                           float *g_emb, float *g_sh, const float *x_rowmax, const float *g_rowmax, void *stream) {
  SNET_REQUIRE(g_sh != nullptr, "snet_conv_bwd_fused_sh: null g_sh");
  return conv_bwd_fused_impl("snet_conv_bwd_fused_sh", fp, x, sh, nullptr, h2, w_row, row_ptr, src, tile_ptr, tile_node, n_tiles, scale,
                             g_out, g_xe, g_h2, emb, g_emb, nullptr, g_sh, x_rowmax, g_rowmax, stream);
}
int snet_conv_bwd_edge(const snet_conv_plan *plan, const float *x, const float *sh, const float *w,
                       const int32_t *w_row, const int32_t *row_ptr, const int32_t *src, int64_t n_dst, float scale, const float *g_out,
                       float *g_w, float *g_xe, float *g_sh, void *stream) {
  SNET_REQUIRE(plan != nullptr, "snet_conv_bwd_edge: null plan");
  SNET_REQUIRE(n_dst < (1ll << 31), "snet_conv_bwd_edge: too many nodes");
  if (n_dst <= 0) return 0;
  plan->k->bwd_edge(x, sh, w, w_row, row_ptr, src, n_dst, scale, g_out, g_w, g_xe, g_sh, static_cast<hipStream_t>(stream));
  SNET_CHECK_LAUNCH("snet_conv_bwd_edge");
  return 0;
}
int snet_conv_bwd_edge_vec(const snet_conv_plan *plan, const float *x, const float *sh, const float *dsh,
                           const float *w, const int32_t *w_row, const int32_t *row_ptr, const int32_t *src, int64_t n_dst, float scale,
                           const float *g_out, float *g_w, float *g_xe, float *g_vec, void *stream) {
  SNET_REQUIRE(plan != nullptr, "snet_conv_bwd_edge_vec: null plan");
  SNET_REQUIRE(n_dst < (1ll << 31), "snet_conv_bwd_edge_vec: too many nodes");
  if (n_dst <= 0) return 0;
  plan->k->bwd_edge_vec(x, sh, dsh, w, w_row, row_ptr, src, n_dst, scale, g_out, g_w, g_xe, g_vec,
                        static_cast<hipStream_t>(stream));
  SNET_CHECK_LAUNCH("snet_conv_bwd_edge_vec");
  return 0;
}
int snet_conv_bwd_node(const snet_conv_plan *plan, const float *sh, const float *w, const int32_t *w_row,
                       const int32_t *col_ptr,
                       const int32_t *eperm, const int32_t *dst, int64_t n_src, float scale, const float *g_out,
                       float *g_x, void *stream) {
// ... 10 lines not shown
```

sevennet_amd/csrc/snet_common.h:

```cpp
#pragma once
#include <hip/hip_runtime.h>
#include <stdint.h>

#include <string>

#include "snet_hip.h"

namespace snet {

void set_error(const std::string &msg);

#define SNET_CHECK_LAUNCH(what)                                                    \
  do {                                                                             \
    hipError_t _e = hipGetLastError();                                             \
    if (_e != hipSuccess) {                                                        \
      snet::set_error(std::string(what) + ": " + hipGetErrorString(_e));           \
      return 1;                                                                    \
    }                                                                              \
  } while (0)

#define SNET_REQUIRE(cond, msg)                                                    \
  do {                                                                             \
    if (!(cond)) {                                                                 \
      snet::set_error(std::string(msg));                                           \
// ... 38 lines not shown
struct FusedKernels {
  const char *tag;
  int dx, dout, nsh, wn;
  int n_sub;
  const int32_t *sub_cols;
  int n_sub_b;
  const int32_t *sub_cols_b;
  const int32_t *gxe_chunk;
  void (*bwd)(int nt, const float *x, const float *sh, const float *dsh, const float *h2, const int32_t *w_row,
              const int32_t *row_ptr, const int32_t *src, const int32_t *tile_ptr, const int32_t *tile_node,
              int64_t n_tiles, const void *slabs, float scale, const float *g_out, float *g_xe, float *g_h2,
              float *g_vec, FusedTail tail, hipStream_t st);
  void (*fwd)(int nt, const float *x, const float *sh, const float *h2, const int32_t *w_row, const int32_t *row_ptr,
              const int32_t *src, int64_t n_dst, const void *slabs, float scale, float *out, int w2_exp, hipStream_t st);
  int tile_mode;
};
void register_fused(const FusedKernels *k);
const FusedKernels *find_fused(const char *tag);
struct FusedRegistrar {
  explicit FusedRegistrar(const FusedKernels *k) { register_fused(k); }
};
struct FusedTangentKernels {
  const char *tag;
  int tangent_pref;
  void (*bwd)(int nt, const float *x, const float *sh, const float *dsh, const float *h2, const int32_t *w_row,
              const int32_t *row_ptr, const int32_t *src, const int32_t *tile_ptr, const int32_t *tile_node,
              int64_t n_tiles, const void *slabs, float scale, const float *g_out, float *g_xe, float *g_h2,
              float *g_vec, FusedTail tail, hipStream_t st);
};
void register_fused_tangent(const FusedTangentKernels *k);
const FusedTangentKernels *find_fused_tangent(const char *tag);
struct FusedTangentRegistrar {
  explicit FusedTangentRegistrar(const FusedTangentKernels *k) { register_fused_tangent(k); }
};
const float *mlp_plan_w2_host(const snet_mlp_plan *plan);
struct MlpHidden {
  const float *w0, *w1;
  int nb, act;
  float cst;
};
MlpHidden mlp_plan_hidden(const snet_mlp_plan *plan);
constexpr int FUSED_TAIL_FRAGS = 22;
int pack_fused_slabs(const float *w2, int wn, int n_sub, const int32_t *sub_cols, int mode, const MlpHidden *tail,
                     void **dev_out, int32_t (&exps)[3]);

uint16_t f16_rne(float f);
float f16_f(uint16_t h);
int f16_scale_exp(const float *v, size_t n);

struct ConvRegistrar {
  explicit ConvRegistrar(const ConvKernels *k) { register_conv(k); }
};

__device__ __forceinline__ int xcd_node(unsigned b, unsigned n) {
  const unsigned k = b & 7u, j = b >> 3, q = n >> 3, r = n & 7u;
  return (int)(k * q + (k < r ? k : r) + j);
}

__device__ __forceinline__ float wave_sum(float v) {
  v += __shfl_xor(v, 32, 64);
  v += __shfl_xor(v, 16, 64);
  v += __shfl_xor(v, 8, 64);
  v += __shfl_xor(v, 4, 64);
  v += __shfl_xor(v, 2, 64);
  v += __shfl_xor(v, 1, 64);
  return v;
// ... 144 lines not shown
```

sevennet_amd/csrc/snet_model.cpp:

```cpp
#include <algorithm>
#include <cmath>
#include <cstdio>
#include <cstdlib>
#include <cstring>
#include <exception>
#include <map>
#include <string>
#include <vector>

#include "snet_common.h"

namespace {

struct Reader {
  const unsigned char *p, *end;
  bool ok = true;
  void get(void *dst, size_t n) {
    if (!ok || (size_t)(end - p) < n) {
      ok = false;
      return;
    }
    memcpy(dst, p, n);
    p += n;
  }
// ... 162 lines not shown
    if (!r.ok || !dev_upload(b, &L.bias)) return false;
  }
  plan_groups(L, false);
  plan_groups(L, true);
  return r.ok;
}

struct Arena {
  char *base = nullptr;
  size_t cap = 0, off = 0;
  float *f(size_t n) {
    const size_t bytes = ((n * 4 + 255) / 256) * 256;
    float *p = reinterpret_cast<float *>(base + off);
    off += bytes;
    return p;
  }
};

}

struct snet_model {
  int n_species, n_layers, lmax, normalize, n_basis, cutoff_kind, poly_p, act_radial, n_scale, d0;
  float cutoff, cutoff_on, act_cst;
  std::vector<float> coeffs;
  float *embed = nullptr, *scale = nullptr, *shift = nullptr;
  double *ro_v = nullptr, ro_c = 0.0;
  std::vector<int> fcn_dims;
  std::vector<float *> fcn_w, fcn_wt;
  int fcn_act = 0;
  float fcn_cst = 1.f;
  double *one_d = nullptr;
  float *h0_table = nullptr, *sc0_table = nullptr;
  float scale0 = 1.f;
  std::vector<Layer> layers;
  Linear ro1, ro2;
  std::string meta;
  Arena arena;
  snet_halo_fn halo_fwd = nullptr, halo_rev = nullptr;
  void *halo_user = nullptr;
  bool fold_forces = true;
  std::vector<std::vector<int32_t>> species_rows_host;
  int32_t *species_rows = nullptr;
  size_t species_rows_cap = 0;
  std::vector<int64_t> species_off, species_cnt;
  bool topo_cache = false, topo_valid = false;
  struct TopoKey { int64_t NT, N, E; const void *row_ptr, *src, *eperm, *w_row; } topo_key{0, 0, 0, nullptr, nullptr, nullptr, nullptr};
  int32_t *c_tile_ptr = nullptr, *c_tile_node = nullptr, *c_center_t = nullptr, *c_w_row_t = nullptr;
  size_t c_tile_cap = 0, c_edge_cap = 0, c_node_cap = 0;
  int64_t c_n_tiles = 0;
  int64_t n_interior = 0;
  hipStream_t halo_stream = nullptr;
  hipEvent_t ev_h0 = nullptr, ev_h1 = nullptr;
  int32_t *c_tile_ptr_b = nullptr;
  size_t c_tile_ptr_b_cap = 0;
  int64_t c_tile_k = 0;
  bool c_split_valid = false;
  int32_t *c_ptile_e0 = nullptr, *c_ptile_nodes = nullptr;
  size_t c_ptile_cap = 0;
  int64_t c_pn_tiles = 0, c_ptile_k = 0;
  std::vector<int32_t> types_prev;
  int64_t eval_syncs = 0;
  hipStream_t side = nullptr;
  hipEvent_t ev_main = nullptr, ev_bwd[2] = {nullptr, nullptr};
  std::vector<hipEvent_t> ev_w;
  bool overlap = getenv("SNET_NO_OVERLAP") == nullptr;
  int fused_terms = [] {
// ... 105 lines not shown
          for (int c = 0; c < L.wn; ++c) w2t[(size_t)k * L.wn + c] *= cs[c];
        good = snet_radial_mlp_plan_create(L.mlp[0], L.mlp[1], L.mlp[2], L.mlp[3], w0.data(), w1.data(), w2t.data(),
                                           m->act_radial, m->act_cst, 1, &L.tmlp) == 0 &&
               snet_fused_plan_create(L.tconv, L.tmlp, m->fused_terms, &L.tfused) == 0;
        L.t_dead.assign(dead, dead + 2 * nd);
      } else if (L.tconv) {
        snet_conv_plan_destroy(L.tconv);
        L.tconv = nullptr;
      }
    }
    good = good && read_linear(r, L.sc) && read_linear(r, L.si1) && read_linear(r, L.si2);
    if (good) {
      const int ns = r.i32();
      good = r.ok && ns >= 1 && ns <= SNET_MAX_GATE_SEGS;
      for (int i = 0; good && i < ns; ++i) {
        snet_gate_seg s;
        s.kind = r.i32(); s.in_off = r.i32(); s.out_off = r.i32(); s.mul = r.i32(); s.l = r.i32();
        s.gate_off = r.i32(); s.act = r.i32(); s.cst = r.f32();
        L.segs.push_back(s);
      }
      good = good && r.ok;
    }
    m->layers.push_back(L);
  }
  const int ro_kind = good ? r.i32() : 0;
  good = good && r.ok && (ro_kind == 0 || ro_kind == 1);
  if (good && ro_kind == 0) good = read_linear(r, m->ro1) && read_linear(r, m->ro2);
  if (good) {
    const int dx0 = r.i32(), gin0 = r.i32();
    good = r.ok && dx0 == m->layers[0].dx && (gin0 == 0 || gin0 == m->layers[0].gin) && (gin0 != 0) == m->layers[0].sc.present();
    if (good) {
      std::vector<float> h0 = r.farr((size_t)m->n_species * dx0), sc0 = r.farr((size_t)m->n_species * gin0);
      good = r.ok && dev_upload(h0, &m->h0_table) && dev_upload(sc0, &m->sc0_table);
    }
  }
  if (good && ro_kind == 1) {
    const int nl = r.i32();
    good = r.ok && nl >= 1 && nl <= 16;
    for (int i = 0; good && i <= nl; ++i) {
      m->fcn_dims.push_back(r.i32());
      good = r.ok && m->fcn_dims.back() >= 1 && m->fcn_dims.back() <= (1 << 16);
    }
    m->fcn_act = good ? r.i32() : 0;
    m->fcn_cst = good ? r.f32() : 1.f;
    good = good && r.ok && m->fcn_act >= 0 && m->fcn_act < snet::N_ACT && m->fcn_dims.front() == m->layers.back().dout && m->fcn_dims.back() == 1;
    for (int i = 0; good && i < nl; ++i) {
      const int di = m->fcn_dims[i], dn = m->fcn_dims[i + 1];
      std::vector<float> w = r.farr((size_t)di * dn), wt((size_t)di * dn);
      for (int a = 0; a < di && r.ok; ++a)
        for (int b = 0; b < dn; ++b) wt[(size_t)b * di + a] = w[(size_t)a * dn + b];
      float *dw = nullptr, *dwt = nullptr;
      good = r.ok && dev_upload(w, &dw) && dev_upload(wt, &dwt);
      m->fcn_w.push_back(dw);
      m->fcn_wt.push_back(dwt);
    }
    const double one = 1.0;
    good = good && hipMalloc((void **)&m->one_d, 8) == hipSuccess && hipMemcpy(m->one_d, &one, 8, hipMemcpyHostToDevice) == hipSuccess;
    if (good) m->ro1.dim_in = m->fcn_dims.front();
  }
  if (good && ro_kind == 0) {
    const int d_ro = r.i32();
    m->ro_c = r.f64();
    good = r.ok && d_ro == m->ro1.dim_in && d_ro == m->layers.back().dout;
    if (good) {
      std::vector<double> v = r.darr((size_t)d_ro);
      good = r.ok && hipMalloc((void **)&m->ro_v, v.size() * 8) == hipSuccess &&
// ... 186 lines not shown
      m->species_rows_host[types_host[i]].push_back((int32_t)i);
    }
    if (m->species_rows_cap < (size_t)N) {
      if (m->species_rows) (void)hipFree(m->species_rows);
      SNET_REQUIRE(hipMalloc((void **)&m->species_rows, (size_t)(N + 1) * 4) == hipSuccess, "snet_model_eval: alloc");
      m->species_rows_cap = N;
    }
    m->species_off.assign(m->n_species, 0);
    m->species_cnt.assign(m->n_species, 0);
    int64_t o = 0;
    for (int s = 0; s < m->n_species; ++s) {
      auto &v = m->species_rows_host[s];
      m->species_off[s] = o;
      m->species_cnt[s] = (int64_t)v.size();
      if (!v.empty())
        SNET_REQUIRE(hipMemcpyAsync(m->species_rows + o, v.data(), v.size() * 4, hipMemcpyHostToDevice, st) == hipSuccess,
                     "snet_model_eval: upload of species rows failed");
      o += (int64_t)v.size();
    }
    SNET_REQUIRE(hipStreamSynchronize(st) == hipSuccess, "snet_model_eval: sync");
    ++m->eval_syncs;
    m->types_prev.assign(types_host, types_host + N);
    }
  }

  size_t need = 0;
  auto add = [&](size_t n) { need += ((n * 4 + 255) / 256) * 256; };
  size_t dmax = (size_t)m->d0, trans = 0;
  add((size_t)E * nb); add((size_t)E * nsh); add((size_t)E * nsh * 3); add((size_t)E * 3); add((size_t)E * nb);
  add((size_t)WR * nb); add((size_t)WR * nb);
  for (auto &L : m->layers) {
    if (L.fused) add((size_t)WR * 64);
    dmax = dmax > (size_t)L.dout ? dmax : (size_t)L.dout;
    add((size_t)NT * L.dx); add(L.fused ? (size_t)WR * 64 : (size_t)WR * L.wn); add((size_t)N * L.gin);
    add((size_t)NT + 64);
    const size_t t = ((size_t)N * L.gin + 64) * 2 + (size_t)N * L.dmid * 2 + (size_t)E * (L.fused ? 64 : L.wn) + (size_t)E * L.dx +
                     (size_t)NT * L.dx * 2 + (size_t)N * L.dout + (size_t)NT + (size_t)N + 4096;
    trans = trans > t ? trans : t;
  }
  size_t wn_max = 0;
  for (auto &L : m->layers) wn_max = wn_max > (size_t)L.wn ? wn_max : (size_t)L.wn;
  if (ov) { add((size_t)E * wn_max); add((size_t)E * wn_max); }
  if (need_tiles[0]) { add((size_t)N + 64); add((size_t)N + (size_t)E / 16 + 64); }
  if (need_tiles[1]) { add((size_t)N + (size_t)E / 16 + 64); add(2 * ((size_t)N + (size_t)E / 16 + 64)); }
  if (any_transposed) { add((size_t)E + 64); add((size_t)E + 64); add((size_t)E * nsh + 64); }
  add((size_t)NT * dmax * 2 + 256); add((size_t)N * (m->ro1.dim_out + 8) * 2); add(trans + 64 * 1024);
  for (size_t i = 0; i + 1 < m->fcn_dims.size(); ++i) {
    add((size_t)N * m->fcn_dims[i + 1] + 64); add((size_t)N * m->fcn_dims[i + 1] + 64); add((size_t)N * m->fcn_dims[i] + 64);
  }
  need += 1 << 20;
  if (m->arena.cap < need) {
    if (m->arena.base) (void)hipFree(m->arena.base);
    m->arena.base = nullptr;
    m->arena.cap = 0;
    SNET_REQUIRE(hipMalloc((void **)&m->arena.base, need) == hipSuccess, "snet_model_eval: arena allocation failed");
    m->arena.cap = need;
  }
  Arena &A = m->arena;
  A.off = 0;

  snet_edge_params ep{m->cutoff, m->n_basis, m->cutoff_kind, m->poly_p, m->cutoff_on, m->lmax, m->normalize};
  float *emb = A.f((size_t)E * nb), *sh = A.f((size_t)E * nsh), *dsh = A.f((size_t)E * nsh * 3);
  float *g_vec = dE_dr ? dE_dr : A.f((size_t)E * 3), *g_emb = A.f((size_t)E * nb);
  int rc;
  if ((rc = snet_edge_embed_fwd(&ep, m->coeffs.data(), edge_vec, E, emb, sh, dsh, st))) return rc;
  const float *emb_w = emb;
  if (pairs) {
    float *ep = A.f((size_t)WR * nb);
    if ((rc = snet_gather_rows(emb, pair_edge, ep, WR, nb, st))) return rc;
    emb_w = ep;
  }
  float *x = A.f((size_t)NT * dmax), *x2 = A.f((size_t)NT * dmax);

  struct Saved { float *h, *w, *y, *wd; };
  std::vector<Saved> saved(Lc);
  bool all_tangent = true;
  for (int t = 0; t < Lc; ++t) {
    saved[t].h = A.f((size_t)NT * m->layers[t].dx);
    saved[t].w = A.f(m->layers[t].fused ? (size_t)WR * 64 : (size_t)WR * m->layers[t].wn);
    const bool tg = m->layers[t].fused != nullptr && snet_fused_plan_prefers_tangent(m->layers[t].fused) != 0;
    saved[t].wd = tg ? A.f((size_t)WR * 64) : nullptr;
    all_tangent = all_tangent && tg;
    saved[t].y = A.f((size_t)N * m->layers[t].gin);
  }
  const snet_model::TopoKey key{NT, N, E, row_ptr, src, eperm, pairs ? w_row : nullptr};
  const bool topo_hit = m->topo_cache && m->topo_valid && memcmp(&key, &m->topo_key, sizeof key) == 0;
  const bool lib_halo = has_halo && m->halo_fwd == &snet_halo_forward && m->halo_rev == &snet_halo_reverse;
  const int64_t n_int = m->n_interior;
  bool hsplit = lib_halo && n_int > 0 && n_int < N && E > 0 && any_fused && getenv("SNET_NO_HALO_SPLIT") == nullptr;
  if (hsplit && m->halo_stream == nullptr) {
    hsplit = hipStreamCreateWithFlags(&m->halo_stream, hipStreamNonBlocking) == hipSuccess &&
             hipEventCreateWithFlags(&m->ev_h0, hipEventDisableTiming) == hipSuccess &&
             hipEventCreateWithFlags(&m->ev_h1, hipEventDisableTiming) == hipSuccess;
  }
  int32_t *tile_ptr = nullptr, *tile_node = nullptr;
  int64_t n_tiles = 0;
  if (need_tiles[0] && E > 0) {
    if (m->topo_cache) {
      if (m->c_node_cap < (size_t)N + 64 || m->c_tile_cap < (size_t)N + (size_t)E / 16 + 64) {
        if (m->c_tile_ptr) (void)hipFree(m->c_tile_ptr);
        if (m->c_tile_node) (void)hipFree(m->c_tile_node);
        m->c_tile_ptr = m->c_tile_node = nullptr;
        m->c_node_cap = (size_t)N + 64;
        m->c_tile_cap = (size_t)N + (size_t)E / 16 + 64;
        SNET_REQUIRE(hipMalloc((void **)&m->c_tile_ptr, m->c_node_cap * 4) == hipSuccess &&
                         hipMalloc((void **)&m->c_tile_node, m->c_tile_cap * 4) == hipSuccess, "snet_model_eval: alloc");
      }
      tile_ptr = m->c_tile_ptr;
      tile_node = m->c_tile_node;
    } else {
      tile_ptr = reinterpret_cast<int32_t *>(A.f((size_t)N + 64));
// ... 111 lines not shown
  {
    const snet_mlp_plan *hp[8];
    float *ho[8], *hd[8];
    float *demb = nullptr;
    for (int pass = 0; pass < 2; ++pass) {
      int nh = 0;
      for (int t = 0; t <= Lc; ++t) {
        if (t < Lc && m->layers[t].fused && (saved[t].wd != nullptr) == (pass == 0)) {
          hp[nh] = m->layers[t].mlp_plan; ho[nh] = saved[t].w; hd[nh] = saved[t].wd; ++nh;
        }
        if (nh == 8 || (t == Lc && nh > 0)) {
          if (pass == 0 && demb == nullptr) {
            demb = A.f((size_t)WR * nb);
            if ((rc = snet_edge_embed_tangent(&ep, m->coeffs.data(), edge_vec, pairs ? pair_edge : nullptr, WR, demb, st))) return rc;
          }
          if ((rc = pass == 0 ? snet_radial_mlp_hidden_fwd_layers_tangent(hp, nh, emb_w, demb, WR, ho, hd, st)
                              : snet_radial_mlp_hidden_fwd_layers(hp, nh, emb_w, WR, ho, st))) return rc;
          nh = 0;
        }
      }
    }
  }

  for (int t = 0; t < Lc; ++t) {
    Layer &L = m->layers[t];
    A.off = mark;
    float *sc = nullptr;
    float *h = saved[t].h;
    if (t == 0) {
      if (L.sc.present()) {
        sc = saved[t].y;
        if ((rc = snet_embed_rows(m->sc0_table, types, sc, N, L.gin, st))) return rc;
      }
      if ((rc = snet_embed_rows(m->h0_table, types, h, NT, L.dx, st))) return rc;
    } else {
      if (L.sc.present()) {
        sc = saved[t].y;
        if ((rc = run_linear(m, L.sc, x, sc, N, false, false, st))) return rc;
      }
      if ((rc = run_linear(m, L.si1, x, h, N, false, false, st))) return rc;
    }
    const bool fsplit = hsplit && t > 0 && L.fused != nullptr;
    if (t > 0 && has_halo) {
      if (fsplit)
        SNET_REQUIRE(hipEventRecord(m->ev_h0, st) == hipSuccess && hipStreamWaitEvent(m->halo_stream, m->ev_h0, 0) == hipSuccess,
                     "snet_model_eval: stream ordering failed");
      if ((rc = m->halo_fwd(m->halo_user, h, NT, N, L.dx, fsplit ? (void *)m->halo_stream : stream))) {
        snet::set_error("snet_model_eval: forward halo callback failed");
        return rc;
      }
      if (fsplit) SNET_REQUIRE(hipEventRecord(m->ev_h1, m->halo_stream) == hipSuccess, "snet_model_eval: stream ordering failed");
    }
    float *mid = A.f((size_t)N * L.dmid);
    if (E == 0) SNET_REQUIRE(hipMemsetAsync(mid, 0, (size_t)N * L.dmid * 4, st) == hipSuccess, "snet_model_eval: memset");
    else
      for (auto &z : L.si2.zero_in)
        SNET_REQUIRE(hipMemset2DAsync(mid + z.first, (size_t)L.dmid * 4, 0, (size_t)z.second * 4, (size_t)N, st) == hipSuccess,
                     "snet_model_eval: memset");
    if (L.fused) {
      const int64_t na = fsplit ? n_int : 0;
      if (na > 0 && (rc = snet_conv_fwd_fused(L.fused, h, sh, saved[t].w, pairs ? w_row : nullptr, row_ptr, src, na, L.conv_scale, mid, st)))
        return rc;
      if (fsplit) SNET_REQUIRE(hipStreamWaitEvent(st, m->ev_h1, 0) == hipSuccess, "snet_model_eval: stream ordering failed");
      if ((rc = snet_conv_fwd_fused(L.fused, h, sh, saved[t].w, pairs ? w_row : nullptr, row_ptr + na, src, N - na, L.conv_scale,
                                    mid + (size_t)na * L.dmid, st)))
        return rc;
    } else {
      if (ov)
        SNET_REQUIRE(hipStreamWaitEvent(st, m->ev_w[t], 0) == hipSuccess, "snet_model_eval: stream ordering failed");
      else if ((rc = snet_radial_mlp_fwd(L.mlp_plan, emb_w, WR, saved[t].w, st)))
        return rc;
      if ((rc = snet_conv_fwd(L.conv, h, sh, saved[t].w, pairs ? w_row : nullptr, row_ptr, src, N, L.conv_scale, mid, st)))
        return rc;
    }
    float *y = saved[t].y;
    if ((rc = run_linear(m, L.si2, mid, y, N, false, sc != nullptr, st))) return rc;
    if ((rc = snet_gate_fwd(y, nullptr, x2, N, L.gin, L.dout, L.segs.data(), (int)L.segs.size(), st))) return rc;
    std::swap(x, x2);
  }
  A.off = mark;
  float *ea = e_atom ? e_atom : A.f((size_t)N + 64);
  float *g_x = x2, *gx_next = x;
  if (!m->fcn_dims.empty()) {
    const std::vector<int> &d = m->fcn_dims;
    const int nl = (int)d.size() - 1;
    std::vector<float *> zs;
    const float *a = x;
    float *z = nullptr;
    for (int i = 0; i < nl; ++i) {
      z = A.f((size_t)N * d[i + 1] + 64);
      if ((rc = snet_gemm(a, m->fcn_w[i], z, N, 1, d[i], d[i + 1], d[i], 0, d[i + 1], 0, nullptr, 0, st))) return rc;
      if (i + 1 < nl) {
        float *an = A.f((size_t)N * d[i + 1] + 64);
        if ((rc = snet_act_fwd(z, an, N * d[i + 1], m->fcn_act, m->fcn_cst, st))) return rc;
        zs.push_back(z);
        a = an;
      }
    }
    if ((rc = snet_rescale_reduce(z, types, m->scale, m->shift, m->n_scale, N, ea, energy, st))) return rc;
    float *gz = A.f((size_t)N + 64);
    if ((rc = snet_readout_grad(m->one_d, 1, types, m->scale, m->n_scale, N, gz, st))) return rc;
    for (int i = nl - 1; i >= 0; --i) {
      float *ga = i == 0 ? g_x : A.f((size_t)N * d[i] + 64);
      if ((rc = snet_gemm(gz, m->fcn_wt[i], ga, N, 1, d[i + 1], d[i], d[i + 1], 0, d[i], 0, nullptr, 0, st))) return rc;
      if (i > 0 && (rc = snet_act_bwd(zs[i - 1], ga, ga, N * d[i], m->fcn_act, m->fcn_cst, st))) return rc;
      gz = ga;
    }
  } else {
    if ((rc = snet_readout_energy(x, N, m->ro1.dim_in, m->ro_v, m->ro_c, types, m->scale, m->shift, m->n_scale, ea, energy, st)))
      return rc;
    if ((rc = snet_readout_grad(m->ro_v, m->ro1.dim_in, types, m->scale, m->n_scale, N, g_x, st))) return rc;
  }
  SNET_REQUIRE(hipMemsetAsync(g_vec, 0, (size_t)E * 3 * 4, st) == hipSuccess &&
                   (all_tangent || hipMemsetAsync(g_emb, 0, (size_t)E * nb * 4, st) == hipSuccess),
               "snet_model_eval: memset failed");
  std::vector<float *> x_max_of((size_t)Lc, nullptr);
  if (E > 0 && m->fused_terms == 4) {
    const float *xs[8];
    float *outs[8];
    int64_t rows[8];
    int32_t dims[8];
    int nj = 0;
    for (int t = 0; t <= Lc; ++t) {
      if (t < Lc && m->layers[t].fused) {
        x_max_of[t] = A.f((size_t)NT + 64);
        xs[nj] = saved[t].h; outs[nj] = x_max_of[t]; rows[nj] = NT; dims[nj] = m->layers[t].dx; ++nj;
      }
      if (nj == 8 || (t == Lc && nj > 0)) {
        if ((rc = snet_row_absmax_multi(xs, rows, dims, outs, nj, st))) return rc;
        nj = 0;
      }
    }
  }
  const size_t mark2 = A.off;
  for (int t = Lc - 1; t >= 0; --t) {
    Layer &L = m->layers[t];
    A.off = mark2;
    float *g_y = A.f((size_t)N * L.gin);
    float *g_max = (L.fused && E > 0 && m->fused_terms == 4) ? A.f((size_t)N) : nullptr;
    if ((rc = snet_gate_bwd_norm(saved[t].y, g_x, g_y, N, L.gin, L.dout, L.segs.data(), (int)L.segs.size(),
                                 g_max ? L.si2.t_norm : 0.f, g_max, st)))
      return rc;
    float *g_m = A.f((size_t)N * L.dmid);
    if ((rc = run_linear(m, L.si2, g_y, g_m, N, true, false, st))) return rc;
    const bool transposed = t > 0 && L.tfused != nullptr && E > 0;
    float *g_xe = t > 0 && !transposed ? A.f((size_t)E * L.dx) : nullptr;
    if (L.fused) {
      const bool tg = saved[t].wd != nullptr;
      const bool tail = tg || snet_fused_plan_has_mlp_tail(L.fused) != 0;
      float *g_h2 = tail ? nullptr : A.f((size_t)E * 64);
      float *x_max = x_max_of[t];
      auto bwd_tiles = [&](const int32_t *tp, const int32_t *tn, int64_t nt) -> int {
        if (E <= 0 || nt <= 0) return 0;
        if (tg)
          return snet_conv_bwd_fused_tangent(L.fused, saved[t].h, sh, dsh, saved[t].w, saved[t].wd, pairs ? w_row : nullptr, row_ptr, src,
                                             tp, tn, nt, L.conv_scale, g_m, g_xe, edge_vec, g_vec, x_max, g_max, st);
        return snet_conv_bwd_fused(L.fused, saved[t].h, sh, dsh, saved[t].w, pairs ? w_row : nullptr, row_ptr, src, tp, tn, nt,
                                   L.conv_scale, g_m, g_xe, g_h2, tail ? emb : nullptr, tail ? g_emb : nullptr, g_vec, x_max, g_max, st);
      };
      const bool rsplit = hsplit && t > 0;
      const bool packed = L.tile_mode != 0;
      auto bwd_all = [&]() -> int { return packed ? bwd_tiles(ptile_e0, ptile_nodes, pn_tiles) : bwd_tiles(tile_ptr, tile_node, n_tiles); };
      if (!rsplit && (rc = bwd_all())) return rc;
      if (t > 0) {
        float *g_h = A.f((size_t)NT * L.dx);
        auto gh_rows = [&](int64_t a, int64_t b) -> int {
          if (b <= a) return 0;
          if (transposed)
            return snet_conv_fwd_fused(L.tfused, g_m, sh_t, saved[t].w, w_row_t, col_ptr + a, center_t, b - a, L.conv_scale,
                                       g_h + (size_t)a * L.dx, st);
          return snet_segment_sum_rows_chunked(g_xe, col_ptr + a, eperm, b - a, L.dx, L.gxe_chunks, g_h + (size_t)a * L.dx, st);
        };
        if (transposed)
          for (size_t i = 0; i + 1 < L.t_dead.size(); i += 2)
            SNET_REQUIRE(hipMemset2DAsync(g_h + L.t_dead[i], (size_t)L.dx * 4, 0, (size_t)L.t_dead[i + 1] * 4, (size_t)NT, st) ==
                             hipSuccess, "snet_model_eval: memset failed");
        if (rsplit) {
          if (!transposed && (rc = packed ? bwd_tiles(ptile_e0 + ptile_k, ptile_nodes + 2 * ptile_k, pn_tiles - ptile_k)
                                          : bwd_tiles(tile_ptr_b, tile_node + tile_k, n_tiles - tile_k))) return rc;
          if ((rc = gh_rows(N, NT))) return rc;
          SNET_REQUIRE(hipEventRecord(m->ev_h0, st) == hipSuccess && hipStreamWaitEvent(m->halo_stream, m->ev_h0, 0) == hipSuccess,
                       "snet_model_eval: stream ordering failed");
          if ((rc = snet_halo_reverse_exchange(m->halo_user, g_h, NT, N, L.dx, m->halo_stream))) return rc;
          SNET_REQUIRE(hipEventRecord(m->ev_h1, m->halo_stream) == hipSuccess, "snet_model_eval: stream ordering failed");
          if ((rc = transposed ? bwd_all() : packed ? bwd_tiles(ptile_e0, ptile_nodes, ptile_k) : bwd_tiles(tile_ptr, tile_node, tile_k))) return rc;
          if ((rc = gh_rows(0, N))) return rc;
// ... 68 lines not shown
```

sevennet_amd/engine.py:

```python
from __future__ import annotations

import ctypes as C
from dataclasses import dataclass
from typing import Dict, List, Optional

import numpy as np
import torch

from . import _lib
from .model_spec import (ACT_CST, ACT_ID, LinearSpec, ModelSpec, build_model_spec, folded_readout, linear_modal_bias,
                         linear_weight_matrices, species_only_tables, transposed_scalar_conv)


def _ptr(t: Optional[torch.Tensor]):
    return None if t is None else C.c_void_p(t.data_ptr())


def _stream():
    return C.c_void_p(torch.cuda.current_stream().cuda_stream)


@dataclass
class Graph:
    n_total: int
# ... 196 lines not shown
                groups.append([b.species, [desc], {tgt}])
            written.add(key)
        out = []
        for species, descs, _ in groups:
            arr = (_lib.GemmDesc * len(descs))(*descs)
            out.append((species, arr, len(descs)))
        return out


class _Span:

    def __init__(self, eng, name):
        self.eng, self.name = eng, name

    def __enter__(self):
        self.on = self.eng.events is not None and (self.eng.event_filter is None or self.name in self.eng.event_filter)
        if self.on:
            self.a = torch.cuda.Event(enable_timing=True)
            self.b = torch.cuda.Event(enable_timing=True)
            self.a.record()

    def __exit__(self, *exc):
        if self.on:
            self.b.record()
            self.eng.events.append((self.name, self.a, self.b))


class HipForceEngine:
    OVERLAP_MAX_EDGES = 1_000_000

    def __init__(self, config: dict, state_dict: Dict[str, np.ndarray], device='cuda:0', mlp_mode: str = 'bf16x6',
                 linear_mode: str = 'bf16x6', fused='auto', fused_terms='f16x3', modal=None, overlap: bool = True,
                 mlp_tail: bool = True, transposed_conv: bool = True, species_tables: bool = True,
                 fold_readout: bool = True, tangent: bool = True):
        if mlp_mode not in ('bf16x6', 'fp32') or linear_mode not in ('bf16x6', 'fp32'):
            raise ValueError("mlp_mode / linear_mode must be 'bf16x6' or 'fp32'")
        if fused not in ('auto', True, False, 'fwd', 'bwd'):
            raise ValueError("fused must be 'auto', True, False, 'fwd' or 'bwd'")
        self.mlp_mode = mlp_mode
        self.linear_mode = linear_mode
        codes = {'bf16': 1, 'bf16x3': 2, 'bf16x6': 3, 'f16x3': 4}
        if fused_terms not in codes and fused_terms not in codes.values():
            raise ValueError(f"fused_terms must be one of {sorted(codes)} (or the C-ABI code 1..4)")
        self.fused_terms = int(codes.get(fused_terms, fused_terms))
        self.fused_mode = {v: k for k, v in codes.items()}[self.fused_terms]
        self.overlap, self.halo_split = bool(overlap), True
        self._side = None
        self._acc_descs = {}
        self.events = None
        self.event_filter = None
        self.lib = _lib.load()
        if not torch.cuda.is_available():
            raise RuntimeError('HipForceEngine needs a ROCm GPU (no CPU fallback exists)')
        self.dev = torch.device(device)
        self.spec: ModelSpec = build_model_spec(config)
        sp = self.spec
        self.modal_idx = mi = sp.modal_index(modal)
        shapes = sp.param_shapes()
        sd = {}
        for k, shp in shapes.items():
            if k not in state_dict:
                raise KeyError(f'state_dict is missing {k}')
            v = state_dict[k]
            v = v.detach().cpu().numpy() if isinstance(v, torch.Tensor) else np.asarray(v)
            if k.startswith('rescale_atomic_energy.'):
                sd[k] = v.astype(np.float64)
                continue
            if v.size != int(np.prod(shp)):
                raise ValueError(f'{k}: checkpoint tensor has {v.size} entries, the model config implies {shp}')
            sd[k] = v.astype(np.float64).reshape(shp)

        self.edge_params = _lib.EdgeParams(sp.cutoff, sp.n_basis, sp.cutoff_kind, sp.cutoff_p, sp.cutoff_on,
                                           sp.lmax_edge, int(sp.normalize_sph))
# ... 86 lines not shown
                    segs[i] = _lib.GateSeg(s.kind, s.in_off, s.out_off, s.mul, s.l, s.gate_off, s.act,
                                           ACT_CST[inv_act[s.act]])
                L.gate_segs = segs
                self.layers.append(L)
            self.h0_table = self.sc0_table = None
            if species_tables:
                h0, sc0 = species_only_tables(sp, sd, mi)
                self.h0_table = torch.from_numpy(h0).to(self.dev)
                self.sc0_table = None if sc0 is None else torch.from_numpy(sc0).to(self.dev)
            self.ro_v = self.ro_fcn = None
            if sp.readout_fcn_dims:
                d = sp.readout_fcn_dims
                ws = [np.ascontiguousarray(sd[f'readout_FCN.fcn.layer{i}.weight'] / np.sqrt(d[i]), dtype=np.float32) for i in range(len(d) - 1)]
                self.ro_fcn = type('F', (), {})()
                self.ro_fcn.dims = d
                self.ro_fcn.w = [torch.from_numpy(w).to(self.dev) for w in ws]
                self.ro_fcn.wt = [torch.from_numpy(np.ascontiguousarray(w.T)).to(self.dev) for w in ws]
                self.ro_fcn.act, self.ro_fcn.cst = ACT_ID[sp.readout_fcn_act], ACT_CST[sp.readout_fcn_act]
            else:
                if fold_readout:
                    v, self.ro_c = folded_readout(sp, sd, mi)
                    self.ro_v = torch.from_numpy(v).to(self.dev)
                self.ro1 = _Linear(sp.readout1, sd[sp.readout1.name], self.dev, split, mi, sd.get(sp.readout1.bias_name))
                self.ro2 = _Linear(sp.readout2, sd[sp.readout2.name], self.dev, split, mi, sd.get(sp.readout2.bias_name))
            sc_v, sh_v = sp.rescale_vectors(sd, mi)
            self.n_scale = len(sc_v)
            self.scale = torch.tensor(sc_v, dtype=torch.float32, device=self.dev)
            self.shift = torch.tensor(sh_v, dtype=torch.float32, device=self.dev)
            self.scale0 = float(sc_v[0])
        self.act_radial = ACT_ID[sp.act_radial]
        self.act_cst = ACT_CST[sp.act_radial]
        self.needs_species_rows = any(ls.sc is not None and ls.sc.n_species for ls in sp.layers)

    def __del__(self):
        try:
            for L in getattr(self, 'layers', []):
                if getattr(L, 'fplan', None) is not None:
                    self.lib.snet_fused_plan_destroy(L.fplan)
                if getattr(L, 'tplan', None) is not None:
                    self.lib.snet_fused_plan_destroy(L.tplan)
                    self.lib.snet_conv_plan_destroy(L.tconv)
                    self.lib.snet_radial_mlp_plan_destroy(L.tmlp)
                self.lib.snet_conv_plan_destroy(L.plan)
                if getattr(L, 'mlp_plan', None) is not None:
                    self.lib.snet_radial_mlp_plan_destroy(L.mlp_plan)
        except Exception:
            pass

    def kernel_times_ms(self) -> Dict[str, List[float]]:
        out: Dict[str, List[float]] = {}
        for name, a, b in self.events or []:
            out.setdefault(name, []).append(a.elapsed_time(b))
        return out

    def _new(self, *shape):
        return torch.empty(*shape, dtype=torch.float32, device=self.dev)

    def _gemm(self, A, B, Cm, n_nodes, d, K, N, a_stride, a_off, c_stride, c_off, rows=None, acc=False):
        _lib.check(self.lib.snet_gemm(_ptr(A), _ptr(B), _ptr(Cm), n_nodes, d, K, N, a_stride, a_off, c_stride,
                                      c_off, _ptr(rows), int(acc), _stream()), 'snet_gemm')

    def _run_groups(self, groups, A, Cm, n, a_stride, c_stride, g: Graph, force_acc=False):
        for species, arr, cnt in groups:
            rows, m = None, n
            if species >= 0:
                rows = g.species_rows[species]
# ... 140 lines not shown
        h2d_of = {t_: self._new(h2_rows, 64) for t_, L_ in enumerate(self.layers) if L_.tangent}
        with _Span(self, 'radial_mlp_hidden_fwd'):
            demb = None
            if h2d_of:
                demb = self._new(h2_rows, nb)
                _lib.check(lib.snet_edge_embed_tangent(C.byref(self.edge_params), self.coeffs, _ptr(g.edge_vec),
                                                       _ptr(g.pair_edge) if pairs else None, h2_rows, _ptr(demb), st), 'snet_edge_embed_tangent')
            for tg_, ts in ((True, sorted(h2d_of)), (False, sorted(set(h2_of) - set(h2d_of)))):
                for i in range(0, len(ts), 8):
                    grp = ts[i:i + 8]
                    plans = (C.c_void_p * len(grp))(*[self.layers[t_].mlp_plan for t_ in grp])
                    outs = (C.c_void_p * len(grp))(*[h2_of[t_].data_ptr() for t_ in grp])
                    if tg_:
                        outs_d = (C.c_void_p * len(grp))(*[h2d_of[t_].data_ptr() for t_ in grp])
                        _lib.check(lib.snet_radial_mlp_hidden_fwd_layers_tangent(plans, len(grp), _ptr(emb_p if pairs else emb), _ptr(demb),
                                                                                 h2_rows, outs, outs_d, st),
                                   'snet_radial_mlp_hidden_fwd_layers_tangent')
                    else:
                        _lib.check(lib.snet_radial_mlp_hidden_fwd_layers(plans, len(grp), _ptr(emb_p if pairs else emb), h2_rows, outs, st),
                                   'snet_radial_mlp_hidden_fwd_layers')
        return SimpleNamespace(g=g, halo=halo, keep=keep, st=st, N=N, NT=NT, E=E, nb=nb, nsh=nsh, inter=inter, emb=emb, sh=sh, dsh=dsh,
                               pairs=pairs, w_row=w_row, emb_p=emb_p if pairs else None, side=side, w_ready=w_ready,
                               gw_bufs=gw_bufs if side is not None else None, gw_done=gw_done if side is not None else None,
                               x=x, saved=saved, split=split, h2_of=h2_of, h2d_of=h2d_of)

    def _forward_layers(self, c):
        lib, g, halo, keep, st, inter = self.lib, c.g, c.halo, c.keep, c.st, c.inter
        N, NT, E = c.N, c.NT, c.E
        emb, sh, pairs, emb_p, w_row, side, w_ready = c.emb, c.sh, c.pairs, c.emb_p, c.w_row, c.side, c.w_ready
        x, saved, split, h2_of = c.x, c.saved, c.split, c.h2_of
        for t, L in enumerate(self.layers):
            ls = L.spec
            n_in = NT if t == 0 else N
            with _Span(self, 'node_linear_fwd'):
                h = self._new(NT, ls.si1.dim_out)
                if t == 0 and self.h0_table is not None:
                    _lib.check(lib.snet_embed_rows(_ptr(self.h0_table), _ptr(g.types), _ptr(h), NT, ls.si1.dim_out, st),
                               'snet_embed_rows')
                else:
                    self._linear(L.si1, x, n_in, g, out=h)
            pending = None
            if t > 0 and halo is not None:
                with _Span(self, 'halo_fwd'):
                    if hasattr(halo, 'forward_start'):
                        pending = halo.forward_start(h, N)
                    else:
                        halo.forward(h, N)
            with _Span(self, 'node_linear_fwd'):
                if t == 0 and self.h0_table is not None:
                    sc = None
                    if self.sc0_table is not None:
                        sc = self._new(N, ls.gate.irreps_in.dim)
                        _lib.check(lib.snet_embed_rows(_ptr(self.sc0_table), _ptr(g.types), _ptr(sc), N, ls.gate.irreps_in.dim,
                                                       st), 'snet_embed_rows')
                else:
                    sc = self._linear(L.sc, x, N, g) if L.sc is not None else None
            dmid = ls.conv.irreps_out.dim
            m = self._new(N, dmid)
            if E == 0:
                m.zero_()
            else:
                for off, ln in L.si2.zero_in:
                    m[:, off:off + ln].zero_()
            h2 = w = zs = None
            rows_w = g.n_pairs if pairs else E
            h2 = h2_of.pop(t, None)
            if not (L.fused_fwd and L.fused_bwd):
                if side is not None:
                    (w, ev), zs = w_ready.pop(t), None
                    torch.cuda.current_stream().wait_event(ev)
                else:
                    with _Span(self, f'radial_mlp_fwd[wn={ls.conv.weight_numel}]'):
                        w, zs = self._mlp_fwd(L, emb_p, g.n_pairs) if pairs else self._mlp_fwd(L, emb, E)
            def conv_rows(a, b):
                if b <= a:
                    return
                rp, mo = C.c_void_p(g.row_ptr.data_ptr() + 4 * a), C.c_void_p(m.data_ptr() + 4 * a * dmid)
                if L.fused_fwd:
                    with _Span(self, f'conv_fwd_fused[{ls.conv.tag}]'):
                        _lib.check(lib.snet_conv_fwd_fused(L.fplan, _ptr(h), _ptr(sh), _ptr(h2), _ptr(w_row), rp,
                                                           _ptr(g.src), b - a, L.scale, mo, st), 'snet_conv_fwd_fused')
                else:
                    with _Span(self, f'conv_fwd[{ls.conv.tag}]'):
                        _lib.check(lib.snet_conv_fwd(L.plan, _ptr(h), _ptr(sh), _ptr(w), _ptr(w_row), rp,
                                                     _ptr(g.src), b - a, L.scale, mo, st), 'snet_conv_fwd')
            n_int = g.n_interior if (pending is not None and split) else 0
            conv_rows(0, n_int)
            if pending is not None:
                with _Span(self, 'halo_fwd'):
                    halo.forward_finish(pending)
            conv_rows(n_int, N)
            if L.fused_bwd:
                w = None
            with _Span(self, 'node_linear_fwd'):
                y = self._linear(L.si2, m, N, g) if sc is None else self._linear(L.si2, m, N, g, out=sc, accumulate=True)
            xo = self._new(N, ls.gate.irreps_out.dim)
            with _Span(self, 'gate_fwd'):
                _lib.check(lib.snet_gate_fwd(_ptr(y), None, _ptr(xo), N, ls.gate.irreps_in.dim,
                                             ls.gate.irreps_out.dim, L.gate_segs, len(ls.gate.segs), st), 'snet_gate_fwd')
            saved.append((h, w, zs, y, h2))
            if keep:
                inter[f'{t}_si1'], inter[f'{t}_conv'], inter[f'{t}_gate_in'], inter[f'{t}_x'] = h[:N], m, y, xo
            x = xo
        return x

    def _readout(self, c, x):
        lib, sp, g, st, N = self.lib, self.spec, c.g, c.st, c.N
        e_atom = self._new(N)
        energy = torch.empty(1, dtype=torch.float64, device=self.dev)
        c.e_sys = None if g.seg_ptr is None else torch.empty(len(g.seg_ptr_host) - 1, dtype=torch.float64, device=self.dev)
        d_ro = sp.readout1.dim_in
# ... 37 lines not shown
            e_sc = self._linear(self.ro2, h1, N, g)
            self._rescale_reduce(c, e_sc, e_atom, energy)
            g_e = self._new(N, 1)
            if self.n_scale > 1:
                _lib.check(lib.snet_embed_rows(_ptr(self.scale), _ptr(g.types), _ptr(g_e), N, 1, st), 'snet_embed_rows')
            else:
                g_e.fill_(self.scale0)
            g_h1 = self._linear_T(self.ro2, g_e, N, g)
            g_x = self._linear_T(self.ro1, g_h1, N, g)
        return e_atom, energy, g_x

    def _rescale_reduce(self, c, e_sc, e_atom, energy):
        lib, g, st, N = self.lib, c.g, c.st, c.N
        if c.e_sys is None:
            _lib.check(lib.snet_rescale_reduce(_ptr(e_sc), _ptr(g.types), _ptr(self.scale), _ptr(self.shift),
                                               self.n_scale, N, _ptr(e_atom), _ptr(energy), st), 'snet_rescale_reduce')
        else:
            _lib.check(lib.snet_rescale_reduce_seg(_ptr(e_sc), _ptr(g.types), _ptr(self.scale), _ptr(self.shift), self.n_scale, N,
                                                   _ptr(g.seg_ptr), c.e_sys.numel(), _ptr(e_atom), _ptr(c.e_sys), _ptr(energy), st),
                       'snet_rescale_reduce_seg')

    def _reverse_layers(self, c, g_x):
        lib, g, halo, st = self.lib, c.g, c.halo, c.st
        N, NT, E, nb, nsh = c.N, c.NT, c.E, c.nb, c.nsh
        emb, sh, dsh, w_row, side, gw_bufs, gw_done = c.emb, c.sh, c.dsh, c.w_row, c.side, c.gw_bufs, c.gw_done
        saved, split = c.saved, c.split
        sh_T = None
        g_vec = torch.zeros(E, 3, dtype=torch.float32, device=self.dev)
        need_g_emb = any(not L_.tangent for L_ in self.layers)
        g_emb = torch.zeros(E, nb, dtype=torch.float32, device=self.dev) if need_g_emb else None
        x_max_of = {}
        if self.fused_terms == 4 and E > 0:
            ts = [t_ for t_, L_ in enumerate(self.layers) if L_.fused_bwd]
            for t_ in ts:
                x_max_of[t_] = self._new(NT)
            with _Span(self, 'row_bounds'):
                for i in range(0, len(ts), 8):
                    grp = ts[i:i + 8]
                    k = len(grp)
                    _lib.check(lib.snet_row_absmax_multi((C.c_void_p * k)(*[saved[t_][0].data_ptr() for t_ in grp]), (C.c_int64 * k)(*[NT] * k),
                                                         (C.c_int32 * k)(*[self.layers[t_].spec.si1.dim_out for t_ in grp]),
                                                         (C.c_void_p * k)(*[x_max_of[t_].data_ptr() for t_ in grp]), k, st),
                               'snet_row_absmax_multi')
        for t in range(len(self.layers) - 1, -1, -1):
            L = self.layers[t]
            ls = L.spec
            h, w, zs, y, h2 = saved[t]
            g_y = self._new(N, ls.gate.irreps_in.dim)
            g_max = self._new(N) if (L.fused_bwd and self.fused_terms == 4 and E > 0) else None
            with _Span(self, 'gate_bwd'):
                _lib.check(lib.snet_gate_bwd_norm(_ptr(y), _ptr(g_x), _ptr(g_y), N, ls.gate.irreps_in.dim, ls.gate.irreps_out.dim,
                                                  L.gate_segs, len(ls.gate.segs), L.si2.t_norm if g_max is not None else 0.0,
                                                  _ptr(g_max), st), 'snet_gate_bwd_norm')
            with _Span(self, 'node_linear_bwd'):
                g_m = self._linear_T(L.si2, g_y, N, g)
            use_t = t > 0 and getattr(L, 'tplan', None) is not None and E > 0
            g_xe = self._new(E, ls.si1.dim_out) if (t > 0 and not use_t) else None
            g_w = g_h2 = None
            rsplit = split and t > 0 and L.fused_bwd
            pending = None
            g_h = self._new(NT, ls.si1.dim_out) if t > 0 else None
            if use_t:
                src_t, w_row_t = g.by_source(lib, st)
                if L.t_dead:
                    g_h.zero_()
                if sh_T is None:
                    sh_T = self._new(E, nsh)
                    _lib.check(lib.snet_gather_rows(_ptr(sh), _ptr(g.eperm), _ptr(sh_T), E, nsh, st), 'snet_gather_rows')

            def gh_rows(a, b):
                if b <= a:
                    return
                cp, go = C.c_void_p(g.col_ptr.data_ptr() + 4 * a), C.c_void_p(g_h.data_ptr() + 4 * a * ls.si1.dim_out)
                if use_t:
                    with _Span(self, f'conv_bwd_node[transposed {ls.conv.tag}]'):
                        _lib.check(lib.snet_conv_fwd_fused(L.tplan, _ptr(g_m), _ptr(sh_T), _ptr(h2), _ptr(w_row_t), cp, _ptr(src_t),
                                                           b - a, L.scale, go, st), 'snet_conv_fwd_fused')
                    return
                with _Span(self, 'conv_bwd_node[segment_sum]'):
                    if L.fused_bwd:
                        _lib.check(lib.snet_segment_sum_rows_chunked(_ptr(g_xe), cp, _ptr(g.eperm), b - a, ls.si1.dim_out,
                                                                     _ptr(L.gxe_chunks), go, st), 'snet_segment_sum_rows_chunked')
                    else:
                        _lib.check(lib.snet_segment_sum_rows(_ptr(g_xe), cp, _ptr(g.eperm), b - a, ls.si1.dim_out, go, st),
                                   'snet_segment_sum_rows')

            if L.fused_bwd:
                tangent = L.tangent
                g_h2 = None if (L.mlp_tail or tangent) else self._new(E, 64)
                x_max = x_max_of.pop(t, None)
                h2d = c.h2d_of.pop(t, None)

                def bwd_tiles(tp_, tn_, nt_):
                    if nt_ <= 0:
                        return
                    with _Span(self, f'conv_bwd_fused[{ls.conv.tag}]'):
                        if tangent:
                            _lib.check(lib.snet_conv_bwd_fused_tangent(L.fplan, _ptr(h), _ptr(sh), _ptr(dsh), _ptr(h2), _ptr(h2d), _ptr(w_row),
                                                                       _ptr(g.row_ptr), _ptr(g.src), _ptr(tp_), _ptr(tn_), nt_, L.scale,
                                                                       _ptr(g_m), _ptr(g_xe), _ptr(g.edge_vec), _ptr(g_vec), _ptr(x_max),
                                                                       _ptr(g_max), st), 'snet_conv_bwd_fused_tangent')
                            return
                        _lib.check(lib.snet_conv_bwd_fused(L.fplan, _ptr(h), _ptr(sh), _ptr(dsh), _ptr(h2), _ptr(w_row),
                                                           _ptr(g.row_ptr), _ptr(g.src), _ptr(tp_), _ptr(tn_), nt_, L.scale,
                                                           _ptr(g_m), _ptr(g_xe), _ptr(g_h2),
                                                           _ptr(emb) if L.mlp_tail else None, _ptr(g_emb) if L.mlp_tail else None,
                                                           _ptr(g_vec), _ptr(x_max), _ptr(g_max), st),
                                   'snet_conv_bwd_fused')
                if rsplit:
                    (tpi, tni, nti), (tpb, tnb, ntb) = g.tiles_split(L.tile_mode)
                    if use_t:
                        gh_rows(N, NT)
                    else:
                        bwd_tiles(tpb, tnb, ntb)
                        gh_rows(N, NT)
                    with _Span(self, 'halo_rev'):
                        pending = halo.reverse_start(g_h, N)
                    if use_t:
                        bwd_tiles(*g.tiles(L.tile_mode))
                    else:
                        bwd_tiles(tpi, tni, nti)
                    gh_rows(0, N)
                elif E > 0:
                    bwd_tiles(*g.tiles(L.tile_mode))
            else:
                if side is not None:
                    if gw_done[t & 1] is not None:
                        torch.cuda.current_stream().wait_event(gw_done[t & 1])
                    g_w = gw_bufs[t & 1][:E * ls.conv.weight_numel].view(E, ls.conv.weight_numel)
# ... 86 lines not shown
```

sevennet_amd/jit.py:

```python
from __future__ import annotations

import hashlib
import os
import subprocess
import sys
import tempfile
import threading

from . import _lib, codegen, codegen_fused
from .build import ARCH, CSRC, INCLUDE, LIB, _flags, _hipcc
from .model_spec import ConvSpec

_lock = threading.Lock()


def cache_dir() -> str:
    d = os.environ.get('SNET_JIT_CACHE') or os.path.join(os.path.expanduser('~'), '.cache', 'sevennet_amd', 'jit')
    os.makedirs(d, exist_ok=True)
    return d


def shape_sources(spec: ConvSpec):
    srcs = [(f'conv_{spec.tag}.hip', codegen.gen_conv(spec))]
    if codegen_fused.fusable(spec):
        srcs.append((f'convf_{spec.tag}.hip', codegen_fused.gen_conv_fused(spec)))
        srcs.append((f'convft_{spec.tag}.hip', codegen_fused.gen_conv_fused_tangent(spec)))
    return srcs


def compile_shape(spec: ConvSpec, out_dir: str = None, verbose: bool = False) -> str:
    out_dir = out_dir or cache_dir()
    srcs = shape_sources(spec)
    h = hashlib.sha1()
    for _, text in srcs:
        h.update(text.encode())
    for hdr in ('snet_common.h', 'snet_split.h'):
        with open(os.path.join(CSRC, hdr), 'rb') as f:
            h.update(f.read())
    h.update(' '.join(_flags()).encode())
    path = os.path.join(out_dir, f'{spec.tag}_{h.hexdigest()[:12]}.so')
    if os.path.exists(path):
        return path
    os.makedirs(os.path.join(CSRC, 'generated'), exist_ok=True)
    codegen.write_if_changed(os.path.join(CSRC, 'generated', 'sh_generated.h'), codegen.gen_sh_header(3))
    with tempfile.TemporaryDirectory(dir=out_dir) as tmp:
        files = []
        for name, text in srcs:
            p = os.path.join(tmp, name)
            with open(p, 'w') as f:
                f.write(text)
            files.append(p)
        lib_dir = os.path.dirname(os.path.abspath(LIB))
        cmd = [_hipcc()] + _flags() + ['-shared', '-x', 'hip'] + files + \
              ['-x', 'none', f'-L{lib_dir}', f'-l:{os.path.basename(LIB)}', f'-Wl,-rpath,{lib_dir}', '-o', os.path.join(tmp, 'shape.so')]
        if verbose:
            print('[sevennet_amd.jit]', ' '.join(cmd), file=sys.stderr, flush=True)
        r = subprocess.run(cmd, capture_output=True, text=True)
        if r.returncode != 0:
            raise RuntimeError(f'hipcc failed on tensor-product shape {spec.tag} ({spec.key}):\n{r.stderr[-4000:]}')
# ... 50 lines not shown
```

Before: 2.712 million atom-steps/s.

## Read layer-0 conv source rows from a species table staged in LDS

For layer 0, whose input is a pure scalar embedding of the atom species, the fused forward and backward convolution kernels now gather source features from a small per-species table, indexed by types[src], instead of from a per-atom materialised x. Small tables are staged in LDS once per workgroup with padded rows to avoid bank conflicts. The per-atom h tensor is then not materialised for layer 0, and row bounds are computed over the table rows. This removes the embed_rows pass and the per-edge global row gathers, at the cost of extra LDS per workgroup (which may lower occupancy) and extra generated kernel variants.

```diff
diff --git a/include/snet_hip.h b/include/snet_hip.h
--- a/include/snet_hip.h
+++ b/include/snet_hip.h
@@ -110,6 +110,21 @@
                                 const int32_t *tile_ptr, const int32_t *tile_node, int64_t n_tiles, float scale, const float *g_out,
                                 float *g_xe, const float *edge_vec, float *g_vec, const float *x_rowmax, const float *g_rowmax,
                                 void *stream);
+int snet_fused_plan_has_table_source(const snet_fused_plan *plan);
+int snet_conv_tag_has_table_source(const char *tag);
+int snet_conv_fwd_fused_table(const snet_fused_plan *plan, const float *table, int32_t n_species, const int32_t *types, const float *sh,
+                              const float *h2, const int32_t *w_row, const int32_t *row_ptr, const int32_t *src, int64_t n_dst,
+                              float scale, float *out, void *stream);
+int snet_conv_bwd_fused_table(const snet_fused_plan *plan, const float *table, int32_t n_species, const int32_t *types, const float *sh,
+                              const float *dsh, const float *h2, const int32_t *w_row, const int32_t *row_ptr, const int32_t *src,
+                              const int32_t *tile_ptr, const int32_t *tile_node, int64_t n_tiles, float scale, const float *g_out,
+                              float *g_xe, float *g_h2, const float *emb, float *g_emb, float *g_vec, const float *table_rowmax,
+                              const float *g_rowmax, void *stream);
+int snet_conv_bwd_fused_tangent_table(const snet_fused_plan *plan, const float *table, int32_t n_species, const int32_t *types,
+                                      const float *sh, const float *dsh, const float *h2, const float *h2d, const int32_t *w_row,
+                                      const int32_t *row_ptr, const int32_t *src, const int32_t *tile_ptr, const int32_t *tile_node,
+                                      int64_t n_tiles, float scale, const float *g_out, float *g_xe, const float *edge_vec, float *g_vec,
+                                      const float *table_rowmax, const float *g_rowmax, void *stream);
 int snet_fused_plan_gxe_chunks(const snet_fused_plan *plan, int32_t *chunk_pos, int32_t capacity);
 int snet_segment_sum_rows_chunked(const float *x, const int32_t *seg_ptr, const int32_t *perm, int64_t n_seg, int32_t dim,
                                   const int32_t *chunk_pos, float *out, void *stream);
diff --git a/sevennet_amd/_lib.py b/sevennet_amd/_lib.py
--- a/sevennet_amd/_lib.py
+++ b/sevennet_amd/_lib.py
@@ -86,6 +86,16 @@
     'snet_conv_bwd_fused_tangent': (C.c_int, [C.c_void_p, c_f32p, c_f32p, c_f32p, c_f32p, c_f32p, c_i32p, c_i32p, c_i32p, c_i32p,
                                               c_i32p, C.c_int64, C.c_float, c_f32p, c_f32p, c_f32p, c_f32p, c_f32p, c_f32p,
                                               c_stream]),
+    'snet_fused_plan_has_table_source': (C.c_int, [C.c_void_p]),
+    'snet_conv_tag_has_table_source': (C.c_int, [C.c_char_p]),
+    'snet_conv_fwd_fused_table': (C.c_int, [C.c_void_p, c_f32p, C.c_int32, c_i32p, c_f32p, c_f32p, c_i32p, c_i32p, c_i32p, C.c_int64,
+                                            C.c_float, c_f32p, c_stream]),
+    'snet_conv_bwd_fused_table': (C.c_int, [C.c_void_p, c_f32p, C.c_int32, c_i32p, c_f32p, c_f32p, c_f32p, c_i32p, c_i32p, c_i32p,
+                                            c_i32p, c_i32p, C.c_int64, C.c_float, c_f32p, c_f32p, c_f32p, c_f32p, c_f32p, c_f32p,
+                                            c_f32p, c_f32p, c_stream]),
+    'snet_conv_bwd_fused_tangent_table': (C.c_int, [C.c_void_p, c_f32p, C.c_int32, c_i32p, c_f32p, c_f32p, c_f32p, c_f32p, c_i32p,
+                                                    c_i32p, c_i32p, c_i32p, c_i32p, C.c_int64, C.c_float, c_f32p, c_f32p, c_f32p,
+                                                    c_f32p, c_f32p, c_f32p, c_stream]),
     'snet_fused_plan_gxe_chunks': (C.c_int, [C.c_void_p, C.POINTER(C.c_int32), C.c_int32]),
     'snet_segment_sum_rows_chunked': (C.c_int, [c_f32p, c_i32p, c_i32p, C.c_int64, C.c_int32, c_i32p, c_f32p, c_stream]),
     'snet_edge_vectors': (C.c_int, [c_f64p, c_i32p, c_i32p, c_f64p, C.c_int64, c_f32p, c_stream]),
diff --git a/sevennet_amd/build.py b/sevennet_amd/build.py
--- a/sevennet_amd/build.py
+++ b/sevennet_amd/build.py
@@ -146,8 +146,14 @@
             codegen.write_if_changed(tpath, codegen_fused.gen_conv_fused_tangent(spec))
             sources.append(tpath)
             keep.add(os.path.basename(tpath))
+        if codegen_fused.table_source_ok(spec):
+            for kern in codegen_fused.TABLE_KERNELS:
+                spath = os.path.join(GEN, f'convfs{kern[0] if kern != "bwdt" else "t"}_{tag}.hip')
+                codegen.write_if_changed(spath, codegen_fused.gen_conv_fused_table(spec, kern))
+                sources.append(spath)
+                keep.add(os.path.basename(spath))
     for f in os.listdir(GEN):
-        if (f.startswith('conv_') or f.startswith('convf_') or f.startswith('convft_') or f.startswith('_conv')) and f not in keep:
+        if (f.startswith('conv_') or f.startswith('convf_') or f.startswith('convft_') or f.startswith('convfs') or f.startswith('_conv')) and f not in keep:
             os.remove(os.path.join(GEN, f))
     jobs = jobs or min(16, os.cpu_count() or 4)
     if verbose:
diff --git a/sevennet_amd/codegen_fused.py b/sevennet_amd/codegen_fused.py
--- a/sevennet_amd/codegen_fused.py
+++ b/sevennet_amd/codegen_fused.py
@@ -9,6 +9,13 @@
 
 def fusable(spec: ConvSpec) -> bool:
     return all(mul % 16 == 0 for mul, _, _ in spec.irreps_x) and spec.irreps_sh.dim <= 16 and len(spec.paths) > 0
+
+
+TAB_LDS_BYTES = 8192
+
+
+def table_source_ok(spec: ConvSpec) -> bool:
+    return fusable(spec) and len(spec.irreps_x) == 1 and all(l == 0 for _, l, _ in spec.irreps_x)
 
 
 def schedule(spec: ConvSpec):
@@ -172,8 +179,11 @@
 
 class _Gen:
 
-    def __init__(self, spec: ConvSpec, tangent: bool = False):
+    def __init__(self, spec: ConvSpec, tangent: bool = False, table: str = None):
         self.spec = spec
+        self.TS = table
+        assert table in (None, 'fwd', 'bwd', 'bwdt') and (table is None or table_source_ok(spec))
+        tangent = tangent or table == 'bwdt'
         self.TG = bool(tangent)
         tag = self.tag = spec.tag
         self.def_b = (int(OPTS.get('fnwv', 8)), int(OPTS.get('fglds', 0)), int(OPTS.get('focc', 2)))
@@ -239,8 +249,11 @@
         d1 = 2 * bs['cat'].l1 + 1
         return bs['cat'], bs['U'], bs['ncb'], d1, (self.noxn > 0 and d1 >= self.noxn)
 
+    def tab_lds(self):
+        return TAB_LDS_BYTES // (4 * self.DX) * (self.DX + 4) * 4 if self.TS else 0
+
     def bwd_lds(self, nt, nwv):
-        return 2 * 8 * nt * 1024 + nwv * (2 * self.NGP * 64 + (128 if self.XT else 0) + self.NSH * 64)
+        return 2 * 8 * nt * 1024 + nwv * (2 * self.NGP * 64 + (128 if self.XT else 0) + self.NSH * 64) + self.tab_lds()
 
     def bwd_cfg(self, nt):
         if 'fnwv' in OPTS:
@@ -272,7 +285,8 @@
         self.olists, self.oo_index = {}, {}
 
     def fwd_lds(self, nt, nwv):
-        return 2 * self.LPB * 4 * nt * 1024 + nwv * (32 * self.NSHP * 4 + self.MAXD1 * 1024 + self.NOEP * 64) + 4 * nwv + (64 * self.N_OOFF if self.OOLDS else 0)
+        return 2 * self.LPB * 4 * nt * 1024 + nwv * (32 * self.NSHP * 4 + self.MAXD1 * 1024 + self.NOEP * 64) + 4 * nwv + (64 * self.N_OOFF if self.OOLDS else 0) + \
+            self.tab_lds()
 
     def fwd_cfg(self, nt):
         if 'fnwvf' in OPTS:
@@ -331,10 +345,46 @@
     def emit_x_loads(self, ind, ci_, ct_expr, tl_):
         A, cats = self.A, self.cats
         cat_ = cats[ci_]
+        if self.TS:
+            A(f'{ind}{{ const int xo_ = {cat_.x_off} + 16 * ({ct_expr}) + 4 * (lane & 3);')
+            for m in range(2 * cat_.l1 + 1):
+                A(f'{ind}  xq[{m}] = tab_row(srs[{tl_}], xo_ + {m * cat_.mul});')
+            A(f'{ind}}}')
+            return
         A(f'{ind}{{ const float *xs_ = x + {cat_.x_off} + 16 * ({ct_expr}) + 4 * (lane & 3) + (size_t)srs[{tl_}] * DX;')
         for m in range(2 * cat_.l1 + 1):
             A(f'{ind}  xq[{m}] = *reinterpret_cast<const f32x4 *>(xs_ + {m * cat_.mul});')
         A(f'{ind}}}')
+
+
+def _emit_table_decl(cx: _Gen):
+    A = cx.A
+    A('  // Source rows are rows of a species table: x[src(e)] = xtab[types[src(e)]].  A small table is staged in LDS once per workgroup')
+    A('  // (rows padded by four floats: lanes that read the same columns of different species fall on different banks); a large one')
+    A('  // is read from global memory.  Same floats into the same multiplies as the row-gather kernel: bit-identical results.')
+    A(f'  constexpr int TROW = DX + 4, TMAX = {TAB_LDS_BYTES // 4} / DX, NTAB = (TMAX * (DX / 4) + NTH - 1) / NTH;')
+    A('  __shared__ __attribute__((aligned(16))) float s_tab[TLDS ? TMAX * TROW : 4];')
+    A('  f32x4 tabst[TLDS ? NTAB : 1];')
+    A('  if constexpr (TLDS) {')
+    A('#pragma unroll')
+    A('    for (int i = 0; i < NTAB; ++i)')
+    A('      if (tid + NTH * i < n_species * (DX / 4)) tabst[i] = *reinterpret_cast<const f32x4 *>(xtab + (size_t)(tid + NTH * i) * 4);')
+    A('  }')
+    A('  auto tab_row = [&](int sp, int off) -> f32x4 {')
+    A('    if constexpr (TLDS) return *reinterpret_cast<const f32x4 *>(&s_tab[sp * TROW + off]);')
+    A('    else return *reinterpret_cast<const f32x4 *>(xtab + (size_t)sp * DX + off);')
+    A('  };')
+    A('  auto species_of = [&](int atom) { return min(max(types[atom], 0), n_species - 1); };   // (clamped: no read outside the table)')
+
+
+def _emit_table_park(cx: _Gen):
+    A = cx.A
+    A('  if constexpr (TLDS) {   // (ordered before the first tab_row by the workgroup barrier below)')
+    A('#pragma unroll')
+    A('    for (int i = 0; i < NTAB; ++i)')
+    A('      if (const int q = tid + NTH * i; q < n_species * (DX / 4))')
+    A('        *reinterpret_cast<f32x4 *>(&s_tab[(q / (DX / 4)) * TROW + 4 * (q % (DX / 4))]) = tabst[i];')
+    A('  }')
 
 
 def _emit_header(cx: _Gen):
@@ -452,8 +502,15 @@
         A('// the edge\'s radial row (tail.h2d).  w\' is a second product on the A fragments of w, its contraction with the fresh g_w tiles one')
         A('// multiply-add per register.  No operand split of g_w, no g_h2 products, no second W2 image in the slab, no hidden-layer tail, no')
         A('// g_emb: the sum goes, along r_e / |r_e|, straight into the g_vec row the kernel writes anyway.')
-    A('template <int NT, bool F16, int NWV, bool GLDS, int OCC, bool GX>')
-    A(f'__global__ __launch_bounds__(64 * NWV, OCC) void conv_bwdf{"t" if TG else ""}_{tag}(const float *__restrict__ x, const float *__restrict__ sh,')
+    TS = cx.TS
+    if TS:
+        A('// TABLE-SOURCE form: the source rows come from a species table (xtab[n_species, DX], types[n_total]) instead of x[n_total, DX].')
+        A('template <int NT, bool F16, int NWV, bool GLDS, int OCC, bool GX, bool TLDS>')
+        A(f'__global__ __launch_bounds__(64 * NWV, OCC) void conv_bwdf{"t" if TG else ""}s_{tag}(const float *__restrict__ xtab, const int32_t *__restrict__ types,')
+        A('    int n_species, const float *__restrict__ sh,')
+    else:
+        A('template <int NT, bool F16, int NWV, bool GLDS, int OCC, bool GX>')
+        A(f'__global__ __launch_bounds__(64 * NWV, OCC) void conv_bwdf{"t" if TG else ""}_{tag}(const float *__restrict__ x, const float *__restrict__ sh,')
     A('    const float *__restrict__ dsh, const float *__restrict__ h2, const int32_t *__restrict__ w_row,')
     A('    const int32_t *__restrict__ row_ptr, const int32_t *__restrict__ src, const int32_t *__restrict__ tile_ptr,')
     A('    const int32_t *__restrict__ tile_node, int n_tiles, const u32x4 *__restrict__ slabs, float scale,')
@@ -470,6 +527,8 @@
         A('  __shared__ u32x4 slab[2][GLN * LPS * 64];')
     A('  const int tid = threadIdx.x, lane = tid & 63, wave = __builtin_amdgcn_readfirstlane(tid >> 6);   // (wave-uniform: scalar address arithmetic)')
     A('  const int j = lane & 15, g = lane >> 4;')
+    if TS:
+        _emit_table_decl(cx)
     if ST:
         A(f'  unsigned ph[{NPH}];')
         A('#pragma unroll')
@@ -524,15 +583,28 @@
         A('  const int in_b = e >= e_b ? 1 : 0;')
     A('  const int s_src = src[e];')
     A('  const int wr = w_row ? w_row[e] : e;')
+    if TS:
+        A('  const int t_src = species_of(s_src);')
     A('  float x_bound = 0.f;')
-    A('  if constexpr (F16) x_bound = tail.x_max[s_src] * tail.g_max[' + ('in_b ? node_b : node' if XT else 'node') + '];')
+    A(f'  if constexpr (F16) x_bound = tail.x_max[{"t_src" if TS else "s_src"}] * tail.g_max[' + ('in_b ? node_b : node' if XT else 'node') + '];')
     _c0, _U0 = cats[0], bsched[0]['U']
     _d0 = 2 * _c0.l1 + 1
-    A(f'  const float *xs0 = x + (size_t)s_src * DX + {_c0.x_off} + 4 * g;')
+    if TS:
+        A(f'  const int xo0 = {_c0.x_off} + 4 * g;')
+    else:
+        A(f'  const float *xs0 = x + (size_t)s_src * DX + {_c0.x_off} + 4 * g;')
     A(f'  f32x4 xr0[{_U0}][{_d0}], xn0[{_U0}][{_d0}];')
-    for u in range(_U0):
-        for m in range(_d0):
-            A(f'  xr0[{u}][{m}] = *reinterpret_cast<const f32x4 *>(xs0 + {16 * u + m * _c0.mul});')
+
+    def first_rows(ind):
+        for u in range(_U0):
+            for m in range(_d0):
+                A(f'{ind}xr0[{u}][{m}] = ' + (f'tab_row(t_src, xo0 + {16 * u + m * _c0.mul});' if TS else f'*reinterpret_cast<const f32x4 *>(xs0 + {16 * u + m * _c0.mul});'))
+    if TS:
+        A('  if constexpr (!TLDS) {')
+        first_rows('    ')
+        A('  }')
+    else:
+        first_rows('  ')
 
     A('  // the edge\'s spherical harmonics wait in wave-private LDS ([component][edge]: conflict-free, the four channel')
     A('  // groups of an edge read the same word) and are re-read per path: 9 .. 16 fewer live registers per lane')
@@ -615,8 +687,14 @@
     A('  }')
     A('  const float g_park = ' + ('scale * g_sc' if cx.GRAW else 'g_sc') + ';   // factor of the g_out entries when they are parked in LDS')
     emit_g_park('  ', 0, '0')
+    if TS:
+        _emit_table_park(cx)
     A('  stage_store(0);')
     A('  __syncthreads();')
+    if TS:
+        A('  if constexpr (TLDS) {')
+        first_rows('    ')
+        A('  }')
     if HOIST:
         A('  if (1 < NSUB' + (' && !(diag & 32)' if exp else '') + ') stage_load(1, 1);   // the first block\'s first sub-step does not request its slab itself')
     A('  int sidx = 0, buf = 0, gbuf = 0;')
@@ -654,7 +732,9 @@
         A(f'    if (cb + 1 < {ncb}' + (' && !(diag & 64)' if exp else '') + ') {')
         for u in range(U):
             for m in range(d1):
-                if not NOXN:
+                if not NOXN and cx.TS:
+                    A(f'      xn{ci}[{u}][{m}] = tab_row(t_src, xo{ci} + {16 * U} * (cb + 1) + {16 * u + m * cat.mul});')
+                elif not NOXN:
                     A(f'      xn{ci}[{u}][{m}] = *reinterpret_cast<const f32x4 *>(xs{ci} + {16 * U} * (cb + 1) + {16 * u + m * cat.mul});')
         if XPF and ci + 1 < len(bsched):
             A('    } else {')
@@ -1043,8 +1123,14 @@
     fgroups, LPB, NOEP, MAXD1, N_OOFF, OOLDS, STF = cx.fgroups, cx.LPB, cx.NOEP, cx.MAXD1, cx.N_OOFF, cx.OOLDS, cx.STF
     SF, out_index, olists, oo_index = cx.SF, cx.out_index, cx.olists, cx.oo_index
     oo_rows = []
-    A('template <int NT, bool F16, int NWV, bool GLDS, int OCC>')
-    A(f'__global__ __launch_bounds__(64 * NWV, OCC) void conv_fwdf_{tag}(const float *__restrict__ x, const float *__restrict__ sh,')
+    if cx.TS:
+        A('// TABLE-SOURCE form: the source rows come from a species table (xtab[n_species, DX], types[n_total]) instead of x[n_total, DX].')
+        A('template <int NT, bool F16, int NWV, bool GLDS, int OCC, bool TLDS>')
+        A(f'__global__ __launch_bounds__(64 * NWV, OCC) void conv_fwdfs_{tag}(const float *__restrict__ xtab, const int32_t *__restrict__ types,')
+        A('    int n_species, const float *__restrict__ sh,')
+    else:
+        A('template <int NT, bool F16, int NWV, bool GLDS, int OCC>')
+        A(f'__global__ __launch_bounds__(64 * NWV, OCC) void conv_fwdf_{tag}(const float *__restrict__ x, const float *__restrict__ sh,')
     A('    const float *__restrict__ h2, const int32_t *__restrict__ w_row, const int32_t *__restrict__ row_ptr,')
     A('    const int32_t *__restrict__ src, int n_nodes, const u32x4 *__restrict__ slabs, float scale, float *__restrict__ out, int w2_exp, int diag) {')
     A(f'  constexpr int LPS = 8 * NT, LPF = 4 * NT, LPB = {LPB}, NTH = 64 * NWV;  // lines per sub-step (all / w part), sub-steps per block')
@@ -1059,6 +1145,8 @@
     A('  const int tid = threadIdx.x, lane = tid & 63, wave = __builtin_amdgcn_readfirstlane(tid >> 6);   // (wave-uniform: scalar address arithmetic)')
     A('  const int c = lane & 15, g = lane >> 4;')
     A('  const int n_raw = snet::xcd_node(blockIdx.x, gridDim.x) * NWV + wave;')
+    if cx.TS:
+        _emit_table_decl(cx)
     if STF:
         A('  unsigned ph[16];')
         A('#pragma unroll')
@@ -1077,6 +1165,8 @@
     A('  const int node = __builtin_amdgcn_readfirstlane(live ? n_raw : n_nodes - 1);')
     A('  const int e_beg = row_ptr[node], e_end = row_ptr[node + 1];')
     A('  const int my_pass = live ? (e_end - e_beg + 31) >> 5 : 0;')
+    if cx.TS:
+        _emit_table_park(cx)
     oo_fill_at = len(L)
     A('  if (lane == 0) s_pass[wave] = my_pass;')
     A('  __syncthreads();')
@@ -1159,7 +1249,10 @@
     A('#pragma unroll')
     A('        for (int i = 0; i < 4; ++i) { hv[tl][q][i] = lo4[i]; hv[tl][q][4 + i] = hi4[i]; }')
     A('      }')
-    A('      srs[tl] = has_e ? src[min(eb + edge_of_row(tl, lane >> 2), e_last)] : 0;')
+    if cx.TS:
+        A('      srs[tl] = has_e ? species_of(src[min(eb + edge_of_row(tl, lane >> 2), e_last)]) : 0;   // the staged row = the source\'s SPECIES row')
+    else:
+        A('      srs[tl] = has_e ? src[min(eb + edge_of_row(tl, lane >> 2), e_last)] : 0;')
     A('    }')
     A('    float o_scale = scale;  // fp16 terms: h2 is scaled per pass (wave-uniform power of two), W2 per matrix on the host; both are undone on the output rows')
     A('    if constexpr (F16) {')
@@ -1336,6 +1429,8 @@
 def _emit_launch_bwd(cx: _Gen):
     A, exp, def_b, bwd_cfg = cx.A, cx.exp, cx.def_b, cx.bwd_cfg
     tag = ('t_' if cx.TG else '_') + cx.tag
+    if cx.TS:
+        return _emit_launch_bwd_table(cx)
     A('template <int NT, bool F16, int NWV, bool GLDS, int OCC>')
     A('void launch_bwd_t(const float *x, const float *sh, const float *dsh, const float *h2, const int32_t *w_row,')
     A('                  const int32_t *row_ptr, const int32_t *src, const int32_t *tile_ptr, const int32_t *tile_node, int64_t n_tiles,')
@@ -1373,6 +1468,67 @@
     A('}')
 
 
+def _emit_launch_bwd_table(cx: _Gen):
+    A, bwd_cfg = cx.A, cx.bwd_cfg
+    kern = f'conv_bwdf{"t" if cx.TG else ""}s_{cx.tag}'
+    A('template <int NT, bool F16, int NWV, bool GLDS, int OCC, bool TOK>   // TOK: the LDS image costs this configuration no workgroup per CU')
+    A('void launch_bwd_t(const float *xtab, const int32_t *types, int n_species, const float *sh, const float *dsh, const float *h2, const int32_t *w_row,')
+    A('                  const int32_t *row_ptr, const int32_t *src, const int32_t *tile_ptr, const int32_t *tile_node, int64_t n_tiles,')
+    A('                  const void *slabs, float scale, const float *g_out, float *g_xe, float *g_h2, float *g_vec, snet::FusedTail tail, hipStream_t st) {')
+    A('  const unsigned grid = (unsigned)((n_tiles + NWV - 1) / NWV);')
+    A(f'  const bool tlds = TOK && (size_t)n_species * DX * 4 <= {TAB_LDS_BYTES};   // the table fits its LDS image')
+    for gx in ('true', 'false'):
+        for tl in ('true', 'false'):
+            A(f'  {"if" if (gx, tl) == ("true", "true") else "else if"} ((g_xe != nullptr) == {gx} && tlds == {tl})')
+            A(f'    {kern}<NT, F16, NWV, GLDS, OCC, {gx}, {tl}><<<dim3(grid), dim3(64 * NWV), 0, st>>>(xtab, types, n_species, sh, dsh, h2, w_row, row_ptr, src,')
+            A('        tile_ptr, tile_node, (int)n_tiles, static_cast<const u32x4 *>(slabs), scale, g_out, g_xe, g_h2, g_vec, tail, 0);')
+    A('}')
+    A('void launch_bwd_table(int nt, const float *xtab, const int32_t *types, int n_species, const float *sh, const float *dsh, const float *h2,')
+    A('                const int32_t *w_row, const int32_t *row_ptr, const int32_t *src, const int32_t *tile_ptr, const int32_t *tile_node, int64_t n_tiles,')
+    A('                const void *slabs, float scale, const float *g_out, float *g_xe, float *g_h2, float *g_vec, snet::FusedTail tail, hipStream_t st) {')
+    args_b = 'xtab, types, n_species, sh, dsh, h2, w_row, row_ptr, src, tile_ptr, tile_node, n_tiles, slabs, scale, g_out, g_xe, g_h2, g_vec, tail, st'
+    def tok(nt_, w):
+        return 'true' if _wgs_per_cu(cx.bwd_lds(nt_, w)) == _wgs_per_cu(cx.bwd_lds(nt_, w) - cx.tab_lds()) else 'false'
+    w, gl, oc = bwd_cfg(2)
+    A(f'  if (nt == 4) launch_bwd_t<2, true, {w}, {"true" if gl else "false"}, {oc}, {tok(2, w)}>({args_b});')
+    for nt_, kw in ((3, 'else if'), (2, 'else if'), (1, 'else')):
+        w, gl, oc = bwd_cfg(nt_)
+        cond = f' (nt == {nt_})' if kw != 'else' else ''
+        A(f'  {kw}{cond} launch_bwd_t<{nt_}, false, {w}, {"true" if gl else "false"}, {oc}, {tok(nt_, w)}>({args_b});')
+    A('}')
+
+
+def _wgs_per_cu(lds_bytes: int) -> int:
+    return (160 * 1024) // max(lds_bytes, 1)
+
+
+def _emit_launch_fwd_table(cx: _Gen):
+    A, fwd_cfg = cx.A, cx.fwd_cfg
+    A('template <int NT, bool F16, int NWV, bool GLDS, int OCC, bool TOK>   // TOK: the LDS image costs this configuration no workgroup per CU')
+    A('void launch_fwd_t(const float *xtab, const int32_t *types, int n_species, const float *sh, const float *h2, const int32_t *w_row,')
+    A('                  const int32_t *row_ptr, const int32_t *src, int64_t n_dst, const void *slabs, float scale, float *out, int w2_exp, hipStream_t st) {')
+    A('  unsigned grid = (unsigned)((n_dst + NWV - 1) / NWV);')
+    A(f'  if (TOK && (size_t)n_species * DX * 4 <= {TAB_LDS_BYTES})   // the table fits its LDS image')
+    A(f'    conv_fwdfs_{cx.tag}<NT, F16, NWV, GLDS, OCC, true><<<dim3(grid), dim3(64 * NWV), 0, st>>>(xtab, types, n_species, sh, h2, w_row, row_ptr, src,')
+    A('        (int)n_dst, static_cast<const u32x4 *>(slabs), scale, out, w2_exp, 0);')
+    A('  else')
+    A(f'    conv_fwdfs_{cx.tag}<NT, F16, NWV, GLDS, OCC, false><<<dim3(grid), dim3(64 * NWV), 0, st>>>(xtab, types, n_species, sh, h2, w_row, row_ptr, src,')
+    A('        (int)n_dst, static_cast<const u32x4 *>(slabs), scale, out, w2_exp, 0);')
+    A('}')
+    A('void launch_fwd_table(int nt, const float *xtab, const int32_t *types, int n_species, const float *sh, const float *h2, const int32_t *w_row,')
+    A('                const int32_t *row_ptr, const int32_t *src, int64_t n_dst, const void *slabs, float scale, float *out, int w2_exp, hipStream_t st) {')
+    args_f = 'xtab, types, n_species, sh, h2, w_row, row_ptr, src, n_dst, slabs, scale, out, w2_exp, st'
+    def tok(nt_, w):
+        return 'true' if _wgs_per_cu(cx.fwd_lds(nt_, w)) == _wgs_per_cu(cx.fwd_lds(nt_, w) - cx.tab_lds()) else 'false'
+    w, gl, oc = fwd_cfg(2)
+    A(f'  if (nt == 4) launch_fwd_t<2, true, {w}, {"true" if gl else "false"}, {oc}, {tok(2, w)}>({args_f});')
+    for nt_, kw in ((3, 'else if'), (2, 'else if'), (1, 'else')):
+        w, gl, oc = fwd_cfg(nt_)
+        cond = f' (nt == {nt_})' if kw != 'else' else ''
+        A(f'  {kw}{cond} launch_fwd_t<{nt_}, false, {w}, {"true" if gl else "false"}, {oc}, {tok(nt_, w)}>({args_f});')
+    A('}')
+
+
 def _emit_launch_fwd(cx: _Gen):
     A, tag, exp, def_f, fwd_cfg = cx.A, cx.tag, cx.exp, cx.def_f, cx.fwd_cfg
     A('template <int NT, bool F16, int NWV, bool GLDS, int OCC>')
@@ -1408,6 +1564,12 @@
 
 def _emit_registration(cx: _Gen):
     A, tag, XT, cols_rev = cx.A, cx.tag, cx.XT, cx.cols_b
+    if cx.TS:
+        fn = {'fwd': 'launch_fwd_table, nullptr, nullptr', 'bwd': 'nullptr, launch_bwd_table, nullptr', 'bwdt': 'nullptr, nullptr, launch_bwd_table'}[cx.TS]
+        A(f'const snet::FusedTableKernels kernels = {{"{tag}", {fn}}};')
+        A('const snet::FusedTableRegistrar registrar(&kernels);')
+        A('}  // namespace')
+        return
     if cx.TG:
         A(f'const snet::FusedTangentKernels kernels = {{"{tag}", {1 if cx.TGPREF else 0}, launch_bwd_tangent}};')
         A('const snet::FusedTangentRegistrar registrar(&kernels);')
@@ -1448,6 +1610,23 @@
     return '\n'.join(cx.L) + '\n'
 
 
+TABLE_KERNELS = ('fwd', 'bwd', 'bwdt')
+
+
+def gen_conv_fused_table(spec: ConvSpec, kernel: str) -> str:
+    cx = _Gen(spec, table=kernel)
+    _emit_header(cx)
+    _emit_path_functions(cx)
+    if kernel == 'fwd':
+        _emit_forward_kernel(cx)
+        _emit_launch_fwd_table(cx)
+    else:
+        _emit_reverse_kernel(cx)
+        _emit_launch_bwd(cx)
+    _emit_registration(cx)
+    return '\n'.join(cx.L) + '\n'
+
+
 def gen_conv_fused(spec: ConvSpec) -> str:
     cx = _Gen(spec)
     _emit_header(cx)
diff --git a/sevennet_amd/csrc/snet_api.cpp b/sevennet_amd/csrc/snet_api.cpp
--- a/sevennet_amd/csrc/snet_api.cpp
+++ b/sevennet_amd/csrc/snet_api.cpp
@@ -1,5 +1,6 @@
 #include <cstdio>
 #include <cstring>
+#include <list>
 #include <map>
 #include <vector>
 
@@ -36,6 +37,25 @@
 const FusedTangentKernels *find_fused_tangent(const char *tag) {
   for (const FusedTangentKernels *k : fused_tangent_registry())
     if (std::string(k->tag) == tag) return k;
+  return nullptr;
+}
+static std::list<FusedTableKernels> &fused_table_registry() {
+  static std::list<FusedTableKernels> r;
+  return r;
+}
+void register_fused_table(const FusedTableKernels *k) {
+  for (FusedTableKernels &e : fused_table_registry())
+    if (std::string(e.tag) == k->tag) {
+      if (k->fwd) e.fwd = k->fwd;
+      if (k->bwd) e.bwd = k->bwd;
+      if (k->bwd_tangent) e.bwd_tangent = k->bwd_tangent;
+      return;
+    }
+  fused_table_registry().push_back(*k);
+}
+const FusedTableKernels *find_fused_table(const char *tag) {
+  for (const FusedTableKernels &e : fused_table_registry())
+    if (std::string(e.tag) == tag) return &e;
   return nullptr;
 }
 
@@ -70,6 +90,7 @@
   void *slabs_b;
   snet::MlpHidden hidden;
   int32_t exps[3];
+  const char *tag;
 };
 
 extern "C" {
@@ -170,7 +191,7 @@
     snet::set_error("snet_fused_plan_create: device allocation / upload of the W2 fragment stream failed");
     return 1;
   }
-  *out = new snet_fused_plan{k, snet::find_fused_tangent(plan->k->tag), terms, dev, dev_b, hid, {exps[0], exps[1], exps[2]}};
+  *out = new snet_fused_plan{k, snet::find_fused_tangent(plan->k->tag), terms, dev, dev_b, hid, {exps[0], exps[1], exps[2]}, k->tag};
   return 0;
 }
 int snet_fused_plan_tile_mode(const snet_fused_plan *p) { return p ? p->k->tile_mode : 0; }
@@ -258,6 +279,81 @@
   SNET_CHECK_LAUNCH("snet_conv_bwd_fused_tangent");
   return 0;
 }
+static const snet::FusedTableKernels *table_kernels(const snet_fused_plan *fp) {
+  const snet::FusedTableKernels *ks = fp ? snet::find_fused_table(fp->tag) : nullptr;
+  return (ks && ks->fwd && ks->bwd && ks->bwd_tangent) ? ks : nullptr;
+}
+int snet_fused_plan_has_table_source(const snet_fused_plan *fp) { return table_kernels(fp) != nullptr; }
+int snet_conv_tag_has_table_source(const char *tag) {
+  const snet::FusedTableKernels *ks = tag ? snet::find_fused_table(tag) : nullptr;
+  return ks && ks->fwd && ks->bwd && ks->bwd_tangent;
+}
+int snet_conv_fwd_fused_table(const snet_fused_plan *fp, const float *table, int32_t n_species, const int32_t *types, const float *sh,
+                              const float *h2, const int32_t *w_row, const int32_t *row_ptr, const int32_t *src, int64_t n_dst,
+                              float scale, float *out, void *stream) {
+  SNET_REQUIRE(fp != nullptr, "snet_conv_fwd_fused_table: null plan");
+  const snet::FusedTableKernels *ks = table_kernels(fp);
+  SNET_REQUIRE(ks != nullptr, "snet_conv_fwd_fused_table: this shape has no table-source kernels (snet_fused_plan_has_table_source)");
+  SNET_REQUIRE(n_dst < (1ll << 31) / 4, "snet_conv_fwd_fused_table: too many nodes");
+  if (n_dst <= 0) return 0;
+  SNET_REQUIRE(table != nullptr && types != nullptr && n_species > 0, "snet_conv_fwd_fused_table: table, types and n_species > 0 are required");
+  ks->fwd(fp->terms, table, types, n_species, sh, h2, w_row, row_ptr, src, n_dst, fp->slabs, scale, out, fp->exps[0],
+          static_cast<hipStream_t>(stream));
+  SNET_CHECK_LAUNCH("snet_conv_fwd_fused_table");
+  return 0;
+}
+int snet_conv_bwd_fused_table(const snet_fused_plan *fp, const float *table, int32_t n_species, const int32_t *types, const float *sh,
+                              const float *dsh, const float *h2, const int32_t *w_row, const int32_t *row_ptr, const int32_t *src,
+                              const int32_t *tile_ptr, const int32_t *tile_node, int64_t n_tiles, float scale, const float *g_out,
+                              float *g_xe, float *g_h2, const float *emb, float *g_emb, float *g_vec, const float *table_rowmax,
+                              const float *g_rowmax, void *stream) {
+  const char *who = "snet_conv_bwd_fused_table";
+  SNET_REQUIRE(fp != nullptr, std::string(who) + ": null plan");
+  const snet::FusedTableKernels *ks = table_kernels(fp);
+  SNET_REQUIRE(ks != nullptr, std::string(who) + ": this shape has no table-source kernels (snet_fused_plan_has_table_source)");
+  SNET_REQUIRE(fp->terms != 4 || (table_rowmax != nullptr && g_rowmax != nullptr),
+               std::string(who) + ": terms = 4 (fp16 operands) needs table_rowmax and g_rowmax (snet_row_absmax of the table and g_out)");
+  SNET_REQUIRE(n_tiles < (1ll << 31), std::string(who) + ": too many tiles");
+  if (n_tiles <= 0) return 0;
+  SNET_REQUIRE(table != nullptr && types != nullptr && n_species > 0, std::string(who) + ": table, types and n_species > 0 are required");
+  SNET_REQUIRE(tile_ptr != nullptr && tile_node != nullptr, std::string(who) + ": null tile list");
+  SNET_REQUIRE((g_h2 != nullptr) != (g_emb != nullptr), std::string(who) + ": exactly one of g_h2 / g_emb is the output");
+  SNET_REQUIRE(g_emb == nullptr || (fp->hidden.w0 != nullptr && emb != nullptr),
+               std::string(who) + ": g_emb needs emb and a plan with the hidden-layer tail (snet_fused_plan_has_mlp_tail)");
+  SNET_REQUIRE(dsh != nullptr && g_vec != nullptr, std::string(who) + ": dsh and g_vec are required");
+  const snet::FusedTail tail{emb, g_emb, fp->hidden.nb, fp->hidden.act, fp->hidden.cst, fp->exps[0], fp->exps[1], fp->exps[2],
+                             table_rowmax, g_rowmax, nullptr, nullptr, nullptr};
+  ks->bwd(fp->terms, table, types, n_species, sh, dsh, h2, w_row, row_ptr, src, tile_ptr, tile_node, n_tiles, fp->slabs_b, scale, g_out,
+          g_xe, g_h2, g_vec, tail, static_cast<hipStream_t>(stream));
+  SNET_CHECK_LAUNCH(who);
+  return 0;
+}
+int snet_conv_bwd_fused_tangent_table(const snet_fused_plan *fp, const float *table, int32_t n_species, const int32_t *types,
+                                      const float *sh, const float *dsh, const float *h2, const float *h2d, const int32_t *w_row,
+                                      const int32_t *row_ptr, const int32_t *src, const int32_t *tile_ptr, const int32_t *tile_node,
+                                      int64_t n_tiles, float scale, const float *g_out, float *g_xe, const float *edge_vec, float *g_vec,
+                                      const float *table_rowmax, const float *g_rowmax, void *stream) {
+  const char *who = "snet_conv_bwd_fused_tangent_table";
+  SNET_REQUIRE(fp != nullptr, std::string(who) + ": null plan");
+  const snet::FusedTableKernels *ks = table_kernels(fp);
+  SNET_REQUIRE(ks != nullptr, std::string(who) + ": this shape has no table-source kernels (snet_fused_plan_has_table_source)");
+  SNET_REQUIRE(fp->terms != 4 || (table_rowmax != nullptr && g_rowmax != nullptr),
+               std::string(who) + ": terms = 4 (fp16 operands) needs table_rowmax and g_rowmax (snet_row_absmax of the table and g_out)");
+  SNET_REQUIRE(n_tiles < (1ll << 31), std::string(who) + ": too many tiles");
+  if (n_tiles <= 0) return 0;
+  SNET_REQUIRE(table != nullptr && types != nullptr && n_species > 0, std::string(who) + ": table, types and n_species > 0 are required");
+  SNET_REQUIRE(tile_ptr != nullptr && tile_node != nullptr, std::string(who) + ": null tile list");
+  SNET_REQUIRE(h2d != nullptr && edge_vec != nullptr && dsh != nullptr && g_vec != nullptr,
+               std::string(who) + ": h2d, edge_vec, dsh and g_vec are required");
+  snet::FusedTail tail{nullptr, nullptr, fp->hidden.nb, fp->hidden.act, fp->hidden.cst, fp->exps[0], fp->exps[1], fp->exps[2],
+                       table_rowmax, g_rowmax, nullptr};
+  tail.h2d = h2d;
+  tail.edge_vec = edge_vec;
+  ks->bwd_tangent(fp->terms, table, types, n_species, sh, dsh, h2, w_row, row_ptr, src, tile_ptr, tile_node, n_tiles, fp->slabs_b, scale,
+                  g_out, g_xe, nullptr, g_vec, tail, static_cast<hipStream_t>(stream));
+  SNET_CHECK_LAUNCH(who);
+  return 0;
+}
 int snet_conv_bwd_fused_sh(const snet_fused_plan *fp, const float *x, const float *sh, const float *h2, const int32_t *w_row,
                            const int32_t *row_ptr, const int32_t *src, const int32_t *tile_ptr, const int32_t *tile_node,
                            int64_t n_tiles, float scale, const float *g_out, float *g_xe, float *g_h2, const float *emb,
diff --git a/sevennet_amd/csrc/snet_common.h b/sevennet_amd/csrc/snet_common.h
--- a/sevennet_amd/csrc/snet_common.h
+++ b/sevennet_amd/csrc/snet_common.h
@@ -94,6 +94,22 @@
 const FusedTangentKernels *find_fused_tangent(const char *tag);
 struct FusedTangentRegistrar {
   explicit FusedTangentRegistrar(const FusedTangentKernels *k) { register_fused_tangent(k); }
+};
+struct FusedTableKernels {
+  const char *tag;
+  void (*fwd)(int nt, const float *xtab, const int32_t *types, int n_species, const float *sh, const float *h2, const int32_t *w_row,
+              const int32_t *row_ptr, const int32_t *src, int64_t n_dst, const void *slabs, float scale, float *out, int w2_exp,
+              hipStream_t st);
+  void (*bwd)(int nt, const float *xtab, const int32_t *types, int n_species, const float *sh, const float *dsh, const float *h2,
+              const int32_t *w_row, const int32_t *row_ptr, const int32_t *src, const int32_t *tile_ptr, const int32_t *tile_node,
+              int64_t n_tiles, const void *slabs, float scale, const float *g_out, float *g_xe, float *g_h2, float *g_vec, FusedTail tail,
+              hipStream_t st);
+  decltype(bwd) bwd_tangent;
+};
+void register_fused_table(const FusedTableKernels *k);
+const FusedTableKernels *find_fused_table(const char *tag);
+struct FusedTableRegistrar {
+  explicit FusedTableRegistrar(const FusedTableKernels *k) { register_fused_table(k); }
 };
 const float *mlp_plan_w2_host(const snet_mlp_plan *plan);
 struct MlpHidden {
diff --git a/sevennet_amd/csrc/snet_model.cpp b/sevennet_amd/csrc/snet_model.cpp
--- a/sevennet_amd/csrc/snet_model.cpp
+++ b/sevennet_amd/csrc/snet_model.cpp
@@ -218,6 +218,7 @@
   double *one_d = nullptr;
   float *h0_table = nullptr, *sc0_table = nullptr;
   float scale0 = 1.f;
+  bool l0_table = false;
   std::vector<Layer> layers;
   Linear ro1, ro2;
   std::string meta;
@@ -389,6 +390,8 @@
     if (good) {
       std::vector<float> h0 = r.farr((size_t)m->n_species * dx0), sc0 = r.farr((size_t)m->n_species * gin0);
       good = r.ok && dev_upload(h0, &m->h0_table) && dev_upload(sc0, &m->sc0_table);
+      m->l0_table = good && m->layers[0].fused != nullptr && snet_fused_plan_has_table_source(m->layers[0].fused) != 0 &&
+                    getenv("SNET_NO_LAYER0_TABLE") == nullptr;
     }
   }
   if (good && ro_kind == 1) {
@@ -641,8 +644,9 @@
   for (auto &L : m->layers) {
     if (L.fused) add((size_t)WR * 64);
     dmax = dmax > (size_t)L.dout ? dmax : (size_t)L.dout;
-    add((size_t)NT * L.dx); add(L.fused ? (size_t)WR * 64 : (size_t)WR * L.wn); add((size_t)N * L.gin);
-    add((size_t)NT + 64);
+    const bool no_h = m->l0_table && &L == &m->layers[0];
+    add(no_h ? 64 : (size_t)NT * L.dx); add(L.fused ? (size_t)WR * 64 : (size_t)WR * L.wn); add((size_t)N * L.gin);
+    add((size_t)(no_h && m->n_species > NT ? m->n_species : NT) + 64);
     const size_t t = ((size_t)N * L.gin + 64) * 2 + (size_t)N * L.dmid * 2 + (size_t)E * (L.fused ? 64 : L.wn) + (size_t)E * L.dx +
                      (size_t)NT * L.dx * 2 + (size_t)N * L.dout + (size_t)NT + (size_t)N + 4096;
     trans = trans > t ? trans : t;
@@ -685,7 +689,7 @@
   std::vector<Saved> saved(Lc);
   bool all_tangent = true;
   for (int t = 0; t < Lc; ++t) {
-    saved[t].h = A.f((size_t)NT * m->layers[t].dx);
+    saved[t].h = (t == 0 && m->l0_table) ? nullptr : A.f((size_t)NT * m->layers[t].dx);
     saved[t].w = A.f(m->layers[t].fused ? (size_t)WR * 64 : (size_t)WR * m->layers[t].wn);
     const bool tg = m->layers[t].fused != nullptr && snet_fused_plan_prefers_tangent(m->layers[t].fused) != 0;
     saved[t].wd = tg ? A.f((size_t)WR * 64) : nullptr;
@@ -863,7 +867,7 @@
         sc = saved[t].y;
         if ((rc = snet_embed_rows(m->sc0_table, types, sc, N, L.gin, st))) return rc;
       }
-      if ((rc = snet_embed_rows(m->h0_table, types, h, NT, L.dx, st))) return rc;
+      if (!m->l0_table && (rc = snet_embed_rows(m->h0_table, types, h, NT, L.dx, st))) return rc;
     } else {
       if (L.sc.present()) {
         sc = saved[t].y;
@@ -888,7 +892,11 @@
       for (auto &z : L.si2.zero_in)
         SNET_REQUIRE(hipMemset2DAsync(mid + z.first, (size_t)L.dmid * 4, 0, (size_t)z.second * 4, (size_t)N, st) == hipSuccess,
                      "snet_model_eval: memset");
-    if (L.fused) {
+    if (L.fused && t == 0 && m->l0_table) {
+      if ((rc = snet_conv_fwd_fused_table(L.fused, m->h0_table, m->n_species, types, sh, saved[t].w, pairs ? w_row : nullptr, row_ptr, src, N,
+                                          L.conv_scale, mid, st)))
+        return rc;
+    } else if (L.fused) {
       const int64_t na = fsplit ? n_int : 0;
       if (na > 0 && (rc = snet_conv_fwd_fused(L.fused, h, sh, saved[t].w, pairs ? w_row : nullptr, row_ptr, src, na, L.conv_scale, mid, st)))
         return rc;
@@ -954,8 +962,9 @@
     int nj = 0;
     for (int t = 0; t <= Lc; ++t) {
       if (t < Lc && m->layers[t].fused) {
-        x_max_of[t] = A.f((size_t)NT + 64);
-        xs[nj] = saved[t].h; outs[nj] = x_max_of[t]; rows[nj] = NT; dims[nj] = m->layers[t].dx; ++nj;
+        const bool tab = t == 0 && m->l0_table;
+        x_max_of[t] = A.f((size_t)(tab ? m->n_species : NT) + 64);
+        xs[nj] = tab ? m->h0_table : saved[t].h; outs[nj] = x_max_of[t]; rows[nj] = tab ? m->n_species : NT; dims[nj] = m->layers[t].dx; ++nj;
       }
       if (nj == 8 || (t == Lc && nj > 0)) {
         if ((rc = snet_row_absmax_multi(xs, rows, dims, outs, nj, st))) return rc;
@@ -983,6 +992,13 @@
       float *x_max = x_max_of[t];
       auto bwd_tiles = [&](const int32_t *tp, const int32_t *tn, int64_t nt) -> int {
         if (E <= 0 || nt <= 0) return 0;
+        if (t == 0 && m->l0_table)
+          return tg ? snet_conv_bwd_fused_tangent_table(L.fused, m->h0_table, m->n_species, types, sh, dsh, saved[t].w, saved[t].wd,
+                                                        pairs ? w_row : nullptr, row_ptr, src, tp, tn, nt, L.conv_scale, g_m, g_xe, edge_vec,
+                                                        g_vec, x_max, g_max, st)
+                    : snet_conv_bwd_fused_table(L.fused, m->h0_table, m->n_species, types, sh, dsh, saved[t].w, pairs ? w_row : nullptr,
+                                                row_ptr, src, tp, tn, nt, L.conv_scale, g_m, g_xe, g_h2, tail ? emb : nullptr,
+                                                tail ? g_emb : nullptr, g_vec, x_max, g_max, st);
         if (tg)
           return snet_conv_bwd_fused_tangent(L.fused, saved[t].h, sh, dsh, saved[t].w, saved[t].wd, pairs ? w_row : nullptr, row_ptr, src,
                                              tp, tn, nt, L.conv_scale, g_m, g_xe, edge_vec, g_vec, x_max, g_max, st);
diff --git a/sevennet_amd/engine.py b/sevennet_amd/engine.py
--- a/sevennet_amd/engine.py
+++ b/sevennet_amd/engine.py
@@ -252,13 +252,12 @@
     def __init__(self, config: dict, state_dict: Dict[str, np.ndarray], device='cuda:0', mlp_mode: str = 'bf16x6',
                  linear_mode: str = 'bf16x6', fused='auto', fused_terms='f16x3', modal=None, overlap: bool = True,
                  mlp_tail: bool = True, transposed_conv: bool = True, species_tables: bool = True,
-                 fold_readout: bool = True, tangent: bool = True):
+                 fold_readout: bool = True, tangent: bool = True, layer0_table: bool = True):
         if mlp_mode not in ('bf16x6', 'fp32') or linear_mode not in ('bf16x6', 'fp32'):
             raise ValueError("mlp_mode / linear_mode must be 'bf16x6' or 'fp32'")
         if fused not in ('auto', True, False, 'fwd', 'bwd'):
             raise ValueError("fused must be 'auto', True, False, 'fwd' or 'bwd'")
-        self.mlp_mode = mlp_mode
-        self.linear_mode = linear_mode
+        self.mlp_mode, self.linear_mode, self.layer0_table = mlp_mode, linear_mode, bool(layer0_table)
         codes = {'bf16': 1, 'bf16x3': 2, 'bf16x6': 3, 'f16x3': 4}
         if fused_terms not in codes and fused_terms not in codes.values():
             raise ValueError(f"fused_terms must be one of {sorted(codes)} (or the C-ABI code 1..4)")
@@ -411,6 +410,12 @@
         self.act_cst = ACT_CST[sp.act_radial]
         self.needs_species_rows = any(ls.sc is not None and ls.sc.n_species for ls in sp.layers)
 
+    @property
+    def l0_table(self) -> bool:
+        L0 = self.layers[0]
+        return bool(self.layer0_table and self.h0_table is not None and L0.fused_fwd and L0.fused_bwd
+                    and self.lib.snet_fused_plan_has_table_source(L0.fplan))
+
     def __del__(self):
         try:
             for L in getattr(self, 'layers', []):
@@ -617,9 +622,12 @@
         for t, L in enumerate(self.layers):
             ls = L.spec
             n_in = NT if t == 0 else N
+            tab = t == 0 and self.l0_table
             with _Span(self, 'node_linear_fwd'):
-                h = self._new(NT, ls.si1.dim_out)
-                if t == 0 and self.h0_table is not None:
+                h = self._new(NT, ls.si1.dim_out) if (keep or not tab) else None
+                if h is None:
+                    pass
+                elif t == 0 and self.h0_table is not None:
                     _lib.check(lib.snet_embed_rows(_ptr(self.h0_table), _ptr(g.types), _ptr(h), NT, ls.si1.dim_out, st),
                                'snet_embed_rows')
                 else:
@@ -661,7 +669,12 @@
                 if b <= a:
                     return
                 rp, mo = C.c_void_p(g.row_ptr.data_ptr() + 4 * a), C.c_void_p(m.data_ptr() + 4 * a * dmid)
-                if L.fused_fwd:
+                if tab:
+                    with _Span(self, f'conv_fwd_fused[{ls.conv.tag}]'):
+                        _lib.check(lib.snet_conv_fwd_fused_table(L.fplan, _ptr(self.h0_table), self.h0_table.shape[0], _ptr(g.types), _ptr(sh),
+                                                                 _ptr(h2), _ptr(w_row), rp, _ptr(g.src), b - a, L.scale, mo, st),
+                                   'snet_conv_fwd_fused_table')
+                elif L.fused_fwd:
                     with _Span(self, f'conv_fwd_fused[{ls.conv.tag}]'):
                         _lib.check(lib.snet_conv_fwd_fused(L.fplan, _ptr(h), _ptr(sh), _ptr(h2), _ptr(w_row), rp,
                                                            _ptr(g.src), b - a, L.scale, mo, st), 'snet_conv_fwd_fused')
@@ -765,13 +778,14 @@
         x_max_of = {}
         if self.fused_terms == 4 and E > 0:
             ts = [t_ for t_, L_ in enumerate(self.layers) if L_.fused_bwd]
+            xs = {t_: self.h0_table if (t_ == 0 and self.l0_table) else saved[t_][0] for t_ in ts}
             for t_ in ts:
-                x_max_of[t_] = self._new(NT)
+                x_max_of[t_] = self._new(xs[t_].shape[0])
             with _Span(self, 'row_bounds'):
                 for i in range(0, len(ts), 8):
                     grp = ts[i:i + 8]
                     k = len(grp)
-                    _lib.check(lib.snet_row_absmax_multi((C.c_void_p * k)(*[saved[t_][0].data_ptr() for t_ in grp]), (C.c_int64 * k)(*[NT] * k),
+                    _lib.check(lib.snet_row_absmax_multi((C.c_void_p * k)(*[xs[t_].data_ptr() for t_ in grp]), (C.c_int64 * k)(*[xs[t_].shape[0] for t_ in grp]),
                                                          (C.c_int32 * k)(*[self.layers[t_].spec.si1.dim_out for t_ in grp]),
                                                          (C.c_void_p * k)(*[x_max_of[t_].data_ptr() for t_ in grp]), k, st),
                                'snet_row_absmax_multi')
@@ -828,6 +842,17 @@
                     if nt_ <= 0:
                         return
                     with _Span(self, f'conv_bwd_fused[{ls.conv.tag}]'):
+                        if t == 0 and self.l0_table:
+                            tb = (L.fplan, _ptr(self.h0_table), self.h0_table.shape[0], _ptr(g.types), _ptr(sh), _ptr(dsh), _ptr(h2))
+                            ti = (_ptr(w_row), _ptr(g.row_ptr), _ptr(g.src), _ptr(tp_), _ptr(tn_), nt_, L.scale, _ptr(g_m), _ptr(g_xe))
+                            if tangent:
+                                _lib.check(lib.snet_conv_bwd_fused_tangent_table(*tb, _ptr(h2d), *ti, _ptr(g.edge_vec), _ptr(g_vec),
+                                                                                 _ptr(x_max), _ptr(g_max), st), 'snet_conv_bwd_fused_tangent_table')
+                            else:
+                                _lib.check(lib.snet_conv_bwd_fused_table(*tb, *ti, _ptr(g_h2), _ptr(emb) if L.mlp_tail else None,
+                                                                         _ptr(g_emb) if L.mlp_tail else None, _ptr(g_vec), _ptr(x_max),
+                                                                         _ptr(g_max), st), 'snet_conv_bwd_fused_table')
+                            return
                         if tangent:
                             _lib.check(lib.snet_conv_bwd_fused_tangent(L.fplan, _ptr(h), _ptr(sh), _ptr(dsh), _ptr(h2), _ptr(h2d), _ptr(w_row),
                                                                        _ptr(g.row_ptr), _ptr(g.src), _ptr(tp_), _ptr(tn_), nt_, L.scale,
diff --git a/sevennet_amd/jit.py b/sevennet_amd/jit.py
--- a/sevennet_amd/jit.py
+++ b/sevennet_amd/jit.py
@@ -25,6 +25,9 @@
     if codegen_fused.fusable(spec):
         srcs.append((f'convf_{spec.tag}.hip', codegen_fused.gen_conv_fused(spec)))
         srcs.append((f'convft_{spec.tag}.hip', codegen_fused.gen_conv_fused_tangent(spec)))
+    if codegen_fused.table_source_ok(spec):
+        for kern in codegen_fused.TABLE_KERNELS:
+            srcs.append((f'convfs{kern[0] if kern != "bwdt" else "t"}_{spec.tag}.hip', codegen_fused.gen_conv_fused_table(spec, kern)))
     return srcs
 
 
```

Result: no change. 2.719 million atom-steps/s, median of 3 (+0.2%).
